# Aatrick/LightDiffusion

Measured on AMD Instinct MI355X. Metric: UNet denoise steps/sec at 512x512, higher is better.
Workload: dtype f16 (fp32 accumulate); 1 GPU; SD1.5 512x512 UNet CFG step, euler_ancestral / normal-30, batch 8/GPU (UNet batch 16), latent 64x64; global_batch=8, parallelism=dp1 (replicas, RCCL cond broadcast), hip_graph=True, setup_before_warmup=hipGraph capture + one untimed schedule pass per workload

## Files before the change

### lightdiffusion_amd/csrc/gemm.h

```cpp
#pragma once
#include "common.h"

struct GemmParams {
    const half_t* A = nullptr;
    const half_t* A2 = nullptr;
    int lda = 0;
    int conv = 0;
    int ksize = 3;
    int pad = -1;
    int Hs = 0, Ws = 0;
    int Hv = 0, Wv = 0;
    int Ho = 0, Wo = 0, stride = 1;
    int C1 = 0, C2 = 0;
    const half_t* S1 = nullptr;
    const half_t* S2 = nullptr;
    int SC1 = 0, SC2 = 0;
    const half_t* W = nullptr;
    int ldw = 0;
    int M = 0, N = 0, K = 0;
    int n_valid = 0;
    int batch = 1;
    long long sA = 0, sW = 0, sC = 0, sR = 0;
    float alpha = 1.0f;
    const half_t* bias_n = nullptr;
    const half_t* bias_m = nullptr;
    const half_t* rowvec = nullptr;
    int rows_per_vec = 1, ldrv = 0;
    const half_t* R = nullptr;
    int ldr = 0;
    int act = 0;
    half_t* C = nullptr;
    int ldc = 0;
    int bm = 0, bn = 0;
    int splitk = 0;
    int m_fastest = -1;
    int xcd_gm = 0;
    float* partial = nullptr;
    size_t partial_bytes = 0;
    float* stat_out = nullptr;
    int* stat_parts_out = nullptr;
    const float* ln_stat = nullptr;
    int ln_parts = 0;
    int ln_rows = 0;
    int ln_zrows = 0;
    float ln_inv_c = 0.f, ln_eps = 0.f;
    const float* ln_wsum = nullptr;
    int ln_swapped = 0;
    const float* gn_scale = nullptr;
    const float* gn_shift = nullptr;
    int gn_silu = 0;
    float* gn_part = nullptr;
    int gn_P = 0, gn_ppb = 0, gn_HW = 0;
    int* gn_part_done = nullptr;
    const half_t* W8 = nullptr;
    int* sync = nullptr;
    int c8_S = 0;
    int dbg = 0;
};

bool conv8_plan(const GemmParams& p, int* S_out);
int conv8_gn_chunks(const GemmParams& p);
int conv8_launch(const GemmParams& p, hipStream_t stream);
bool conv8_weight_eligible(int N, int Cin);
size_t conv8_weight_bytes(int N, int Cin);
int conv8_repack_launch(const half_t* w_okki, int N, int Cin, half_t* dst, hipStream_t stream);
#define LD_SYNC_INTS 1024

bool gemm_ln_fold_available();
const char* gemm_last_kernel_name();

static inline int gemm_pick_bn(int N) { return (N % 160 == 0) ? 160 : 128; }

int gemm_launch(const GemmParams& p, hipStream_t stream);
bool gemm_conv_fuses_groupnorm(const GemmParams& p);
bool gemm_conv_takes_skip_segment(const GemmParams& p);
bool gemm_conv_takes_halo_tile(const GemmParams& p);
```

### lightdiffusion_amd/csrc/gemm.hip

```cpp
#include <cstdlib>
#include <mutex>
#include <set>
#include <string>
#include <type_traits>

#include "gemm.h"

namespace {

constexpr int BK = 64;
constexpr int NT = 256;

__device__ __forceinline__ void epilogue_store8(const GemmParams& p, int z, int m, int n_out, int n_bias, float (&v)[8]) {
    const bool hb = p.bias_n != nullptr && p.act != 2, hv = p.rowvec != nullptr, hr = p.R != nullptr;
    const uint4 rb = hb ? ld16(p.bias_n + n_bias) : zero16();
    const uint4 rv = hv ? ld16(p.rowvec + (long long)(m / p.rows_per_vec) * p.ldrv + n_out) : zero16();
    const uint4 rr = hr ? ld16(p.R + (long long)z * p.sR + (long long)m * p.ldr + n_out) : zero16();
    const float bm = p.bias_m != nullptr ? (float)p.bias_m[m] : 0.f;
    float b[8], e[8], r[8];
    unpack8(rb, b);
    unpack8(rv, e);
    unpack8(rr, r);
#pragma unroll
    for (int j = 0; j < 8; ++j) v[j] = v[j] + b[j] + bm + e[j];
    if (p.act == 1) {
#pragma unroll
        for (int j = 0; j < 8; ++j) v[j] = silu_f(v[j]);
    } else if (p.act == 3) {
#pragma unroll
        for (int j = 0; j < 8; ++j) v[j] = quick_gelu_f(v[j]);
    }
#pragma unroll
    for (int j = 0; j < 8; ++j) v[j] += r[j];
    st16(p.C + (long long)z * p.sC + (long long)m * p.ldc + n_out, pack8(v));
}

template <int BM, int BN>
struct EpiPre {
    static constexpr int CPR = BN / 8, EIT = (BM * CPR + NT - 1) / NT, GRP = EIT > 5 ? (EIT + 1) / 2 : EIT;
    uint4 r[GRP];
    bool fast;
    bool bias_done;
};
template <int BM, int BN>
__device__ __forceinline__ EpiPre<BM, BN> epi_prefetch_residual(const GemmParams& p, int z, int m0, int n0, int tid, bool bias_done) {
    EpiPre<BM, BN> e;
    e.bias_done = bias_done;
    constexpr int CPR = EpiPre<BM, BN>::CPR, GRP = EpiPre<BM, BN>::GRP;
    e.fast = (BM * CPR) % NT == 0 && m0 + BM <= p.M && n0 + BN <= p.N && p.act == 0 && p.bias_m == nullptr && bias_done;
#pragma unroll
    for (int k = 0; k < GRP; ++k) e.r[k] = zero16();
    if (e.fast && p.R != nullptr) {
        const half_t* Rb = p.R + (long long)z * p.sR + (long long)m0 * p.ldr + n0;
#pragma unroll
        for (int k = 0; k < GRP; ++k) {
            const int q = tid + k * NT;
            const int row = q / CPR, cc = q - row * CPR;
            e.r[k] = ld16(Rb + (long long)row * p.ldr + cc * 8);
        }
    }
    return e;
}

template <int BM, int BN>
__device__ __forceinline__ void epilogue_tile(const GemmParams& p, const half_t* Cs, int z, int m0, int n0, int tid, float* lds_scratch, const half_t* bias_s,
                                              const EpiPre<BM, BN>& pre) {
    constexpr int CLD = BN + 8;
    if (p.act == 2) {
        constexpr int CPR = BN / 16;
        constexpr int EIT = (BM * CPR + NT - 1) / NT;
        if ((BM * CPR) % NT == 0 && m0 + BM <= p.M && n0 + BN <= p.N && pre.bias_done) {
            half_t* Cb = p.C + (long long)z * p.sC + (long long)m0 * p.ldc + n0 / 2;
            const bool hr = p.R != nullptr;
            const half_t* Rb = hr ? p.R + (long long)z * p.sR + (long long)m0 * p.ldr + n0 / 2 : nullptr;
            uint4 rres[EIT], ca[EIT], cg[EIT];
#pragma unroll
            for (int it = 0; it < EIT; ++it) {
                const int q = tid + it * NT;
                const int row = q / CPR, cc = q - row * CPR;
                rres[it] = hr ? ld16(Rb + (long long)row * p.ldr + cc * 8) : zero16();
                ca[it] = ld16(Cs + row * CLD + cc * 8);
                cg[it] = ld16(Cs + row * CLD + BN / 2 + cc * 8);
            }
#pragma unroll
            for (int it = 0; it < EIT; ++it) {
                const int q = tid + it * NT;
                const int row = q / CPR, cc = q - row * CPR;
                float g[8];
                unpack8(cg[it], g);
                const unsigned aw[4] = {ca[it].x, ca[it].y, ca[it].z, ca[it].w};
                const f32x2 gp[4] = {{g[0], g[1]}, {g[2], g[3]}, {g[4], g[5]}, {g[6], g[7]}};
                unsigned ow[4];
                geglu8_staged(aw, gp, ow);
                uint4 packed = make_uint4(ow[0], ow[1], ow[2], ow[3]);
                if (hr) packed = add8h(packed, rres[it]);
                st16(Cb + (long long)row * p.ldc + cc * 8, packed);
            }
            return;
        }
        uint4 rba[EIT], rbg[EIT], rres[EIT];
#pragma unroll
        for (int it = 0; it < EIT; ++it) {
            const int q = tid + it * NT;
            const int row = q / CPR, cc = q - row * CPR;
            const int m = m0 + row, nv = n0 + cc * 8, ng = nv + BN / 2;
            const bool ok = q < BM * CPR && m < p.M && ng < p.N;
            rba[it] = (ok && !pre.bias_done) ? ld16(p.bias_n + nv) : zero16();
            rbg[it] = (ok && !pre.bias_done) ? ld16(p.bias_n + ng) : zero16();
            rres[it] = (ok && p.R != nullptr) ? ld16(p.R + (long long)z * p.sR + (long long)m * p.ldr + n0 / 2 + cc * 8) : zero16();
        }
#pragma unroll
        for (int it = 0; it < EIT; ++it) {
            const int q = tid + it * NT;
            const int row = q / CPR, cc = q - row * CPR;
            const int m = m0 + row, ng = n0 + cc * 8 + BN / 2;
            if (q < BM * CPR && m < p.M && ng < p.N) {
                float a[8], g[8], ba[8], bg[8], r[8];
                unpack8(ld16(Cs + row * CLD + cc * 8), a);
                unpack8(ld16(Cs + row * CLD + BN / 2 + cc * 8), g);
                unpack8(rba[it], ba);
                unpack8(rbg[it], bg);
                unpack8(rres[it], r);
#pragma unroll
                for (int j = 0; j < 8; ++j) a[j] = (a[j] + ba[j]) * gelu_f(g[j] + bg[j]) + r[j];
                st16(p.C + (long long)z * p.sC + (long long)m * p.ldc + n0 / 2 + cc * 8, pack8(a));
            }
        }
    } else {
        constexpr int CPR = BN / 8;
        constexpr int EIT = (BM * CPR + NT - 1) / NT;
        constexpr int GRP = EIT > 5 ? (EIT + 1) / 2 : EIT;
        const bool hb = p.bias_n != nullptr && !pre.bias_done, hv = p.rowvec != nullptr, hr = p.R != nullptr;
        if (pre.fast) {
            static_assert(GRP == EpiPre<BM, BN>::GRP, "group size");
            half_t* Cb = p.C + (long long)z * p.sC + (long long)m0 * p.ldc + n0;
            const half_t* Rb = hr ? p.R + (long long)z * p.sR + (long long)m0 * p.ldr + n0 : nullptr;
            uint4 rnext[GRP];
#pragma unroll
            for (int k = 0; k < GRP; ++k) rnext[k] = pre.r[k];
#pragma unroll
            for (int g0 = 0; g0 < EIT; g0 += GRP) {
                uint4 rv[GRP], rres[GRP], cv[GRP];
#pragma unroll
                for (int k = 0; k < GRP; ++k) rres[k] = rnext[k];
#pragma unroll
                for (int k = 0; k < GRP; ++k) {
                    if (g0 + GRP + k >= EIT) continue;
                    const int q = tid + (g0 + GRP + k) * NT;
                    const int row = q / CPR, cc = q - row * CPR;
                    rnext[k] = hr ? ld16(Rb + (long long)row * p.ldr + cc * 8) : zero16();
                }
#pragma unroll
                for (int k = 0; k < GRP; ++k) {
                    if (g0 + k >= EIT) continue;
                    const int q = tid + (g0 + k) * NT;
                    const int row = q / CPR, cc = q - row * CPR;
                    rv[k] = hv ? ld16(p.rowvec + (long long)((m0 + row) / p.rows_per_vec) * p.ldrv + n0 + cc * 8) : zero16();
                    cv[k] = ld16(Cs + row * CLD + cc * 8);
                }
#pragma unroll
                for (int k = 0; k < GRP; ++k) {
                    if (g0 + k >= EIT) continue;
                    const int q = tid + (g0 + k) * NT;
                    const int row = q / CPR, cc = q - row * CPR;
                    uint4 packed = cv[k];
                    if (hv) packed = add8h(packed, rv[k]);
                    if (hr) packed = add8h(packed, rres[k]);
                    st16(Cb + (long long)row * p.ldc + cc * 8, packed);
                    if (lds_scratch != nullptr) {
                        const half2v one2 = {(half_t)1.f, (half_t)1.f};
                        const half2v h0 = __builtin_bit_cast(half2v, packed.x), h1 = __builtin_bit_cast(half2v, packed.y);
                        const half2v h2 = __builtin_bit_cast(half2v, packed.z), h3 = __builtin_bit_cast(half2v, packed.w);
                        float s1 = __builtin_amdgcn_fdot2(h1, one2, __builtin_amdgcn_fdot2(h0, one2, 0.f, false), false);
                        float s2 = __builtin_amdgcn_fdot2(h1, h1, __builtin_amdgcn_fdot2(h0, h0, 0.f, false), false);
                        s1 = __builtin_amdgcn_fdot2(h3, one2, __builtin_amdgcn_fdot2(h2, one2, s1, false), false);
                        s2 = __builtin_amdgcn_fdot2(h3, h3, __builtin_amdgcn_fdot2(h2, h2, s2, false), false);
                        *reinterpret_cast<float2*>(lds_scratch + q * 2) = make_float2(s1, s2);
                    }
                }
            }
            if (lds_scratch != nullptr) {
                __syncthreads();
                if (tid < BM) {
                    float s1 = 0.f, s2 = 0.f;
#pragma unroll 4
                    for (int c = 0; c < CPR; ++c) {
                        const float2 t = *reinterpret_cast<const float2*>(lds_scratch + (tid * CPR + c) * 2);
                        s1 += t.x;
                        s2 += t.y;
                    }
                    *reinterpret_cast<float2*>(p.stat_out + ((long long)(n0 / BN) * p.M + m0 + tid) * 2) = make_float2(s1, s2);
                }
            }
            return;
        }
#pragma unroll
        for (int g0 = 0; g0 < EIT; g0 += GRP) {
            uint4 rb[GRP], rv[GRP], rres[GRP];
#pragma unroll
            for (int k = 0; k < GRP; ++k) {
                const int q = tid + (g0 + k) * NT;
                const int row = q / CPR, cc = q - row * CPR;
                const int m = m0 + row, n = n0 + cc * 8;
                const bool ok = (g0 + k) < EIT && q < BM * CPR && m < p.M && n < p.N;
                rb[k] = (ok && hb) ? ld16(p.bias_n + n) : zero16();
                rv[k] = (ok && hv) ? ld16(p.rowvec + (long long)(m / p.rows_per_vec) * p.ldrv + n) : zero16();
                rres[k] = (ok && hr) ? ld16(p.R + (long long)z * p.sR + (long long)m * p.ldr + n) : zero16();
            }
#pragma unroll
            for (int k = 0; k < GRP; ++k) {
                const int q = tid + (g0 + k) * NT;
                const int row = q / CPR, cc = q - row * CPR;
                const int m = m0 + row, n = n0 + cc * 8;
                if ((g0 + k) < EIT && q < BM * CPR && m < p.M && n < p.N) {
                    float v[8], b[8], e[8], r[8];
                    unpack8(ld16(Cs + row * CLD + cc * 8), v);
                    unpack8(rb[k], b);
                    unpack8(rv[k], e);
                    unpack8(rres[k], r);
                    const float bm = p.bias_m != nullptr ? (float)p.bias_m[m] : 0.f;
#pragma unroll
                    for (int j = 0; j < 8; ++j) {
                        float t = v[j] + b[j] + bm + e[j];
                        if (p.act == 1) t = silu_f(t);
                        else if (p.act == 3) t = quick_gelu_f(t);
                        v[j] = t + r[j];
                    }
                    const uint4 packed = pack8(v);
                    st16(p.C + (long long)z * p.sC + (long long)m * p.ldc + n, packed);
                    if (lds_scratch != nullptr) {
                        float f[8];
                        unpack8(packed, f);
                        float s1 = 0.f, s2 = 0.f;
#pragma unroll
                        for (int j = 0; j < 8; ++j) {
                            s1 += f[j];
                            s2 += f[j] * f[j];
                        }
                        lds_scratch[q * 2] = s1;
                        lds_scratch[q * 2 + 1] = s2;
                    }
                } else if (lds_scratch != nullptr && (g0 + k) < EIT && q < BM * CPR) {
                    lds_scratch[q * 2] = 0.f;
                    lds_scratch[q * 2 + 1] = 0.f;
                }
            }
        }
        if (lds_scratch != nullptr) {
            __syncthreads();
            if (tid < BM && m0 + tid < p.M) {
                float s1 = 0.f, s2 = 0.f;
                for (int c = 0; c < CPR; ++c) {
                    s1 += lds_scratch[(tid * CPR + c) * 2];
                    s2 += lds_scratch[(tid * CPR + c) * 2 + 1];
                }
                float* o = p.stat_out + ((long long)(n0 / BN) * p.M + m0 + tid) * 2;
                o[0] = s1;
                o[1] = s2;
            }
        }
    }
}

__device__ __forceinline__ void ln_sum_parts(const float* q, long long stride, int parts, float& s1, float& s2) {
    int t = 0;
    for (; t + 4 <= parts; t += 4) {
        float2 v[4];
#pragma unroll
        for (int u = 0; u < 4; ++u) v[u] = *reinterpret_cast<const float2*>(q + (t + u) * stride);
#pragma unroll
        for (int u = 0; u < 4; ++u) {
            s1 += v[u].x;
            s2 += v[u].y;
        }
    }
    for (; t < parts; ++t) {
        const float2 v = *reinterpret_cast<const float2*>(q + t * stride);
        s1 += v.x;
        s2 += v.y;
    }
}

template <int BM, int BN>
__device__ __forceinline__ void ln_prepare(const GemmParams& p, float* ln_mu, float* ln_rs, int z, int m0, int n0, int tid) {
    const int cnt = p.ln_swapped ? BN : BM;
    if (tid >= cnt) return;
    const bool ok = p.ln_swapped ? (n0 + tid < p.n_valid) : (m0 + tid < p.M);
    const long long row = p.ln_swapped ? (long long)z * p.ln_zrows + n0 + tid : (long long)m0 + tid;
    float s1 = 0.f, s2 = 0.f;
    if (ok) ln_sum_parts(p.ln_stat + row * 2, (long long)p.ln_rows * 2, p.ln_parts, s1, s2);
    const float mu = s1 * p.ln_inv_c;
    ln_mu[tid] = mu;
    ln_rs[tid] = ok ? rsqrtf(fmaxf(s2 * p.ln_inv_c - mu * mu, 0.f) + p.ln_eps) : 0.f;
}

template <int TM, int TN>
__device__ __forceinline__ void ln_apply(const GemmParams& p, f32x4 (&acc)[TM][TN], const float* ln_mu, const float* ln_rs, int m0, int n0, int wm0,
                                         int wn0, int fr, int fq, const float* wsum_s, const half_t* bias_s, bool add_bias) {
    if (!p.ln_swapped) {
        f32x4 ws[TN], bj[TN];
        const float inv_alpha = 1.0f / p.alpha;
#pragma unroll
        for (int j = 0; j < TN; ++j) {
            ws[j] = *reinterpret_cast<const f32x4*>(wsum_s + wn0 + j * 16 + fq * 4);
            const half4 bh = *reinterpret_cast<const half4*>(bias_s + wn0 + j * 16 + fq * 4);
#pragma unroll
            for (int r = 0; r < 4; ++r) bj[j][r] = add_bias ? (float)bh[r] * inv_alpha : 0.f;
        }
#pragma unroll
        for (int i = 0; i < TM; ++i) {
            const float mu = ln_mu[wm0 + i * 16 + fr], rs = ln_rs[wm0 + i * 16 + fr];
#pragma unroll
            for (int j = 0; j < TN; ++j) acc[i][j] = (acc[i][j] - mu * ws[j]) * rs + bj[j];
        }
    } else {
#pragma unroll
        for (int i = 0; i < TM; ++i) {
            const int m = m0 + wm0 + i * 16 + fr;
            const float wsm = m < p.M ? p.ln_wsum[m] : 0.f;
#pragma unroll
            for (int j = 0; j < TN; ++j) {
                const f32x4 mu4 = *reinterpret_cast<const f32x4*>(ln_mu + wn0 + j * 16 + fq * 4);
                const f32x4 rs4 = *reinterpret_cast<const f32x4*>(ln_rs + wn0 + j * 16 + fq * 4);
                acc[i][j] = (acc[i][j] - mu4 * wsm) * rs4;
            }
        }
    }
}

__device__ uint4 g_zero_row[4096];

template <int BN>
__device__ __forceinline__ void epi_stage_load(const GemmParams& p, int n0, int t, f32x4& b, f32x4& w) {
    const char* zp = reinterpret_cast<const char*>(g_zero_row);
    const char* bp = (t < BN / 8 && p.bias_n != nullptr && n0 + t * 8 < p.N) ? reinterpret_cast<const char*>(p.bias_n + n0 + t * 8) : zp;
    const char* wp = (t < BN / 4 && p.ln_wsum != nullptr && !p.ln_swapped && n0 + t * 4 < p.N) ? reinterpret_cast<const char*>(p.ln_wsum + n0 + t * 4) : zp;
    asm volatile("global_load_dwordx4 %0, %1, off" : "=&v"(b) : "v"(bp) : "memory");
    asm volatile("global_load_dwordx4 %0, %1, off" : "=&v"(w) : "v"(wp) : "memory");
}
#define EPI_STAGE_WAIT(KEEP, b, w) asm volatile("s_waitcnt vmcnt(%2)" : "+v"(b), "+v"(w) : "n"(KEEP) : "memory")
template <int BN>
__device__ __forceinline__ void epi_stage_store(const f32x4& b, const f32x4& w, half_t* bias_s, float* wsum_s, int t) {
    if (t < BN / 8) *reinterpret_cast<f32x4*>(bias_s + t * 8) = b;
    if (t < BN / 4) *reinterpret_cast<f32x4*>(wsum_s + t * 4) = w;
}


__device__ __forceinline__ void glds16s(unsigned voff, const half_t* sbase, unsigned lds_base) {
    asm volatile(
        "s_mov_b32 m0, %2\n\t"
        "s_nop 0\n\t"
        "global_load_lds_dwordx4 %0, %1"
        :
        : "v"(voff), "s"(sbase), "s"(lds_base)
        : "memory");
}

template <int BM, int BN, bool CONV, int NST>
__global__ __launch_bounds__(NT, NST == 2 ? 2 : 1) void gemm3_kernel(const GemmParams p) {
    constexpr int BK3 = 64, PF = NST - 1;
    static_assert(NST == 2 || NST == 4, "ring depth");
    constexpr int WTM = BM / 2, WTN = BN / 2;
    constexpr int TM = WTM / 16, TN = WTN / 16;
    constexpr int A_CH = BM * 8, B_CH = BN * 8;
    constexpr int A_IT = A_CH / NT;
    constexpr int B_IT = B_CH / NT;
    static_assert(B_CH % NT == 0 && A_CH % NT == 0, "whole instructions per wave");
    constexpr int STAGE = (BM + BN) * BK3;
    constexpr int CLD = BN + 8;
    static_assert(BM * CLD <= NST * STAGE, "epilogue tile must fit in the ring");
    static_assert((BM * CLD * 2 + 15) / 16 * 16 + BM * (BN / 8) * 8 <= NST * STAGE * 2, "LN-fold row statistics must fit behind the epilogue tile");
    __shared__ __attribute__((aligned(16))) half_t smem[NST * STAGE];
    __shared__ __attribute__((aligned(16))) float ln_mu[BM > BN ? BM : BN], ln_rs[BM > BN ? BM : BN];
    __shared__ __attribute__((aligned(16))) half_t bias_s[BN];
    __shared__ __attribute__((aligned(16))) float wsum_s[BN];

    const int tid = threadIdx.x, lane = tid & 63;
    const int wid = __builtin_amdgcn_readfirstlane(tid >> 6);
    const int wm0 = (wid >> 1) * WTM, wn0 = (wid & 1) * WTN;
    const int z = blockIdx.z;
    const int tiles_m = (p.M + BM - 1) / BM, tiles_n = (p.N + BN - 1) / BN;
    const int tiles = tiles_m * tiles_n;
    const int splitk = p.splitk > 1 ? p.splitk : 1;
    int bid = xcd_remap(blockIdx.x, tiles * splitk);
    const int ks = bid / tiles;
    bid -= ks * tiles;
    const int tn_i = p.m_fastest ? bid / tiles_m : bid % tiles_n;
    const int tm_i = p.m_fastest ? bid % tiles_m : bid / tiles_n;
    const int m0 = tm_i * BM, n0 = tn_i * BN;
    const int KT = (p.K + BK3 - 1) / BK3;
    const int kt_begin = (int)((long long)ks * KT / splitk), kt_end = (int)((long long)(ks + 1) * KT / splitk);

    const half_t* Ab = p.A + (long long)z * p.sA;
    const half_t* Wb = p.W + (long long)z * p.sW;
    const half_t* zp = reinterpret_cast<const half_t*>(g_zero_row);
    const int Cin = p.C1 + p.C2;

    int a_lc[A_IT];
    bool a_ok[A_IT];
    int a_img[A_IT], a_iy0[A_IT], a_ix0[A_IT];
    const half_t* a_ptr[A_IT];
    unsigned a_off[A_IT];
#pragma unroll
    for (int i = 0; i < A_IT; ++i) {
        const int q = tid + i * NT;
        const int row = q >> 3;
        a_lc[i] = (q & 7) ^ (row & 7);
        const int m = m0 + row;
        a_ok[i] = m < p.M;
        a_img[i] = a_iy0[i] = a_ix0[i] = 0;
        a_ptr[i] = zp;
        a_off[i] = 0;
        if (CONV) {
            const int hw = p.Ho * p.Wo;
            const int mm = a_ok[i] ? m : 0;
            const int img = mm / hw, rem = mm - img * hw;
            const int oy = rem / p.Wo, ox = rem - oy * p.Wo;
            a_img[i] = img;
            a_iy0[i] = oy * p.stride - p.pad;
            a_ix0[i] = ox * p.stride - p.pad;
        } else {
            a_off[i] = (unsigned)(((long long)(a_ok[i] ? m : p.M - 1) * p.lda + a_lc[i] * 8) * 2);
        }
    }
    const half_t* a_base = Ab + (long long)kt_begin * BK3;
    int seg_left = 0;
    auto conv_seek = [&](int k0) {
        const int K9 = p.ksize * p.ksize * Cin;
        const bool skp = k0 >= K9 && p.SC1 > 0;
        const int tap = skp ? 0 : k0 / Cin;
        const int c0 = skp ? k0 - K9 : k0 - tap * Cin;
        const int ky = skp ? p.pad : tap / p.ksize, kx = skp ? p.pad : tap - (tap / p.ksize) * p.ksize;
        const int Ca = skp ? p.SC1 : p.C1, Cb = skp ? p.SC2 : p.C2;
        const bool second = c0 >= Ca;
        const half_t* src = skp ? (second ? p.S2 : p.S1) : (second ? p.A2 : Ab);
        const int Cs = second ? Cb : Ca;
        const int cl = second ? c0 - Ca : c0;
        seg_left = ((second ? Ca + Cb : Ca) - c0) / BK3;
#pragma unroll
        for (int i = 0; i < A_IT; ++i) {
            const int iy = a_iy0[i] + ky, ix = a_ix0[i] + kx;
            const bool ok = a_ok[i] && (unsigned)iy < (unsigned)p.Hv && (unsigned)ix < (unsigned)p.Wv && tap < p.ksize * p.ksize && c0 < Ca + Cb;
            int sy = iy, sx = ix;
            if (p.Hv == 2 * p.Hs && p.Wv == 2 * p.Ws) {
                sy = iy >> 1;
                sx = ix >> 1;
            } else if (p.Hv != p.Hs || p.Wv != p.Ws) {
                sy = (int)((long long)iy * p.Hs / p.Hv);
                sx = (int)((long long)ix * p.Ws / p.Wv);
            }
            a_ptr[i] = ok ? src + (((long long)a_img[i] * p.Hs + sy) * p.Ws + sx) * Cs + cl + a_lc[i] * 8 : zp + a_lc[i] * 8;
        }
    };
    unsigned b_off[B_IT];
    int b_lc[B_IT];
#pragma unroll
    for (int i = 0; i < B_IT; ++i) {
        const int q = tid + i * NT;
        const int row = q >> 3;
        b_lc[i] = (q & 7) ^ (row & 7);
        const int n = n0 + row < p.n_valid ? n0 + row : p.n_valid - 1;
        b_off[i] = (unsigned)(((long long)n * p.ldw + b_lc[i] * 8) * 2);
    }
    const half_t* b_base = Wb + (long long)kt_begin * BK3;

    const unsigned smem_base = __builtin_amdgcn_readfirstlane(lds_addr(smem));
    auto issue = [&](int kt, int st) {
        if (kt >= kt_end) return;
        const unsigned As = smem_base + (unsigned)(st * STAGE) * 2u + (unsigned)(wid * 64) * 16u;
        const unsigned Bs = As + (unsigned)(BM * BK3) * 2u;
        const int k0 = kt * BK3;
        if (k0 + BK3 <= p.K) {
#pragma unroll
            for (int i = 0; i < A_IT; ++i) {
                if (CONV) glds16(a_ptr[i], As + (unsigned)(i * NT) * 16u);
                else glds16s(a_off[i], a_base, As + (unsigned)(i * NT) * 16u);
            }
#pragma unroll
            for (int i = 0; i < B_IT; ++i) glds16s(b_off[i], b_base, Bs + (unsigned)(i * NT) * 16u);
        } else {
#pragma unroll
            for (int i = 0; i < A_IT; ++i) {
                const half_t* src = CONV ? a_ptr[i] : reinterpret_cast<const half_t*>(reinterpret_cast<const char*>(a_base) + a_off[i]);
                glds16(k0 + a_lc[i] * 8 < p.K ? src : zp, As + (unsigned)(i * NT) * 16u);
            }
#pragma unroll
            for (int i = 0; i < B_IT; ++i) {
                const half_t* src = reinterpret_cast<const half_t*>(reinterpret_cast<const char*>(b_base) + b_off[i]);
                glds16(k0 + b_lc[i] * 8 < p.K ? src : zp, Bs + (unsigned)(i * NT) * 16u);
            }
        }
        if (CONV) {
            if (--seg_left <= 0) {
                conv_seek(k0 + BK3);
            } else {
#pragma unroll
                for (int i = 0; i < A_IT; ++i) a_ptr[i] += BK3;
            }
        } else {
            a_base += BK3;
        }
        b_base += BK3;
    };
    if (CONV) conv_seek(kt_begin * BK3);

    const int fr = lane & 15, fq = lane >> 4;
    const half_t* rd0 = smem + (wm0 + fr) * BK3 + ((fq ^ (fr & 7)) << 3);
    const half_t* rd1 = smem + (wm0 + fr) * BK3 + (((4 + fq) ^ (fr & 7)) << 3);
    const int b_rel = (BM + wn0 - wm0) * BK3;

    f32x4 acc[TM][TN];
#pragma unroll
    for (int i = 0; i < TM; ++i)
#pragma unroll
        for (int j = 0; j < TN; ++j) acc[i][j] = (f32x4){0.f, 0.f, 0.f, 0.f};

    half8 fa0[TM], fb0[TN], fa1[TM], fb1[TN];
    auto read_frags = [&](const half_t* rd, half8 (&fa)[TM], half8 (&fb)[TN]) {
#pragma unroll
        for (int j = 0; j < TN; ++j) fb[j] = as_half8(ld16(rd + b_rel + j * 16 * BK3));
#pragma unroll
        for (int i = 0; i < TM; ++i) fa[i] = as_half8(ld16(rd + i * 16 * BK3));
    };
    auto mma = [&](const half8 (&fa)[TM], const half8 (&fb)[TN]) {
#pragma unroll
        for (int i = 0; i < TM; ++i)
#pragma unroll
            for (int j = 0; j < TN; ++j) acc[i][j] = __builtin_amdgcn_mfma_f32_16x16x32_f16(fb[j], fa[i], acc[i][j], 0, 0, 0);
    };

    constexpr int LPT = A_IT + B_IT;
    auto wait_slab = [&](int kt) {
        if (PF == 1) {
            wait_vmcnt<0>();
        } else {
            const int ahead = kt_end - 1 - kt;
            if (ahead >= PF - 1) wait_vmcnt<LPT*(PF - 1)>();
            else if (ahead == 1) wait_vmcnt<LPT>();
            else wait_vmcnt<0>();
        }
    };
    f32x4 est_b, est_w;
    epi_stage_load<BN>(p, n0, tid, est_b, est_w);
#pragma unroll
    for (int t = 0; t < PF; ++t) issue(kt_begin + t, t);
    if (p.ln_stat != nullptr) ln_prepare<BM, BN>(p, ln_mu, ln_rs, z, m0, n0, tid);
    if (kt_end - kt_begin >= PF) EPI_STAGE_WAIT(PF * (A_IT + B_IT), est_b, est_w);
    else EPI_STAGE_WAIT(0, est_b, est_w);
    epi_stage_store<BN>(est_b, est_w, bias_s, wsum_s, tid);
    wait_slab(kt_begin);
    __builtin_amdgcn_s_barrier();
    issue(kt_begin + PF, PF);
    const bool bias_acc = splitk == 1 && p.ln_stat == nullptr && (p.act == 0 || p.act == 2);
    const bool bias_done = bias_acc || (splitk == 1 && p.ln_stat != nullptr && !p.ln_swapped && (p.act == 0 || p.act == 2));
    if (bias_acc) {
        const float inv_alpha = 1.0f / p.alpha;
#pragma unroll
        for (int j = 0; j < TN; ++j) {
            const half4 bh = *reinterpret_cast<const half4*>(bias_s + wn0 + j * 16 + fq * 4);
            f32x4 bf;
#pragma unroll
            for (int r = 0; r < 4; ++r) bf[r] = (float)bh[r] * inv_alpha;
#pragma unroll
            for (int i = 0; i < TM; ++i) acc[i][j] = bf;
        }
    }
    read_frags(rd0, fa0, fb0);
    asm volatile("s_waitcnt lgkmcnt(0)" ::: "memory");
    int st = 0;
    for (int kt = kt_begin; kt < kt_end; ++kt) {
        read_frags(rd1, fa1, fb1);
        __builtin_amdgcn_sched_barrier(0);
        mma(fa0, fb0);
        __builtin_amdgcn_sched_barrier(0);
        asm volatile("s_waitcnt lgkmcnt(0)" ::: "memory");
        wait_slab(kt + 1);
        __builtin_amdgcn_s_barrier();
        issue(kt + NST, st);
        const int flip = (st == NST - 1) ? -(NST - 1) * STAGE : STAGE;
        rd0 += flip;
        rd1 += flip;
        st = (st + 1) & (NST - 1);
        read_frags(rd0, fa0, fb0);
        __builtin_amdgcn_sched_barrier(0);
        mma(fa1, fb1);
        __builtin_amdgcn_sched_barrier(0);
        asm volatile("s_waitcnt lgkmcnt(0)" ::: "memory");
    }
    wait_vmcnt<0>();
    __builtin_amdgcn_s_barrier();

    if (splitk > 1) {
        float* part = p.partial + (long long)ks * p.M * p.N;
#pragma unroll
        for (int i = 0; i < TM; ++i) {
            const int m = m0 + wm0 + i * 16 + fr;
#pragma unroll
            for (int j = 0; j < TN; ++j) {
                const int n = n0 + wn0 + j * 16 + fq * 4;
                if (m < p.M && n < p.N) {
                    f32x4 v = acc[i][j];
                    v *= p.alpha;
                    *reinterpret_cast<f32x4*>(part + (long long)m * p.N + n) = v;
                }
            }
        }
        return;
    }
    half_t* Cs = smem;
    const EpiPre<BM, BN> pre = epi_prefetch_residual<BM, BN>(p, z, m0, n0, tid, bias_done);
    if (p.ln_stat != nullptr) ln_apply<TM, TN>(p, acc, ln_mu, ln_rs, m0, n0, wm0, wn0, fr, fq, wsum_s, bias_s, bias_done);
#pragma unroll
    for (int i = 0; i < TM; ++i) {
        const int ml = wm0 + i * 16 + fr;
#pragma unroll
        for (int j = 0; j < TN; ++j) {
            const int nl = wn0 + j * 16 + fq * 4;
            const f32x4 v = acc[i][j] * p.alpha;
            *reinterpret_cast<uint2*>(Cs + ml * CLD + nl) = make_uint2(pk2h(v[0], v[1]), pk2h(v[2], v[3]));
        }
    }
    __syncthreads();
    float* scratch = p.stat_out != nullptr ? reinterpret_cast<float*>(reinterpret_cast<char*>(smem) + (BM * CLD * 2 + 15) / 16 * 16) : nullptr;
    epilogue_tile<BM, BN>(p, Cs, z, m0, n0, tid, scratch, bias_s, pre);
}

template <int LPT, int MAXA>
__device__ __forceinline__ void wait_slabs_ahead(int ahead) {
    if constexpr (MAXA == 0) {
        wait_vmcnt<0>();
    } else {
        if (ahead >= MAXA) wait_vmcnt<MAXA * LPT>();
        else wait_slabs_ahead<LPT, MAXA - 1>(ahead);
    }
}

template <int BM, int BN, bool CONV, int NST = 4, int WPS = 2>
__global__ __launch_bounds__(2 * NT, WPS) void gemm4_kernel(const GemmParams p) {
    constexpr int BK3 = 64;
    static_assert((NST & (NST - 1)) == 0 && NST >= 4, "ring depth");
    constexpr int WTM = BM / 2, WTN = BN / 2;
    constexpr int TM = WTM / 16, TN = WTN / 16;
    constexpr int A_IT = BM * 8 / NT, B_IT = BN * 8 / NT;
    static_assert((BM * 8) % NT == 0 && (BN * 8) % NT == 0, "whole instructions per wave");
    constexpr int LPT = A_IT + B_IT;
    constexpr int STAGE = (BM + BN) * BK3;
    constexpr int CLD = BN + 8;
    static_assert(BM * CLD <= NST * STAGE, "epilogue tile must fit in the ring");
    __shared__ __attribute__((aligned(16))) half_t smem[NST * STAGE];
    __shared__ __attribute__((aligned(16))) float ln_mu[BM > BN ? BM : BN], ln_rs[BM > BN ? BM : BN];
    __shared__ __attribute__((aligned(16))) half_t bias_s[BN];
    __shared__ __attribute__((aligned(16))) float wsum_s[BN];

    const int lane = threadIdx.x & 63;
    const int wid8 = __builtin_amdgcn_readfirstlane(threadIdx.x >> 6);
    const bool producer = wid8 >= 4;
    const int wid = wid8 & 3;
    const int tid = wid * 64 + lane;
    const int z = blockIdx.z;
    const int tiles_m = (p.M + BM - 1) / BM, tiles_n = (p.N + BN - 1) / BN;
    const int tiles = tiles_m * tiles_n;
    const int splitk = p.splitk > 1 ? p.splitk : 1;
    int bid = xcd_remap(blockIdx.x, tiles * splitk);
    const int ks = bid / tiles;
    bid -= ks * tiles;
    const int tn_i = p.m_fastest ? bid / tiles_m : bid % tiles_n;
    const int tm_i = p.m_fastest ? bid % tiles_m : bid / tiles_n;
    const int m0 = tm_i * BM, n0 = tn_i * BN;
    const int KT = (p.K + BK3 - 1) / BK3;
    const int kt_begin = (int)((long long)ks * KT / splitk), kt_end = (int)((long long)(ks + 1) * KT / splitk);

    if (producer) {
        const half_t* Ab = p.A + (long long)z * p.sA;
        const half_t* Wb = p.W + (long long)z * p.sW;
        const half_t* zp = reinterpret_cast<const half_t*>(g_zero_row);
        const int Cin = p.C1 + p.C2;
        int a_lc[A_IT];
        bool a_ok[A_IT];
        int a_img[A_IT], a_iy0[A_IT], a_ix0[A_IT];
        const half_t* a_ptr[A_IT];
        unsigned a_off[A_IT];
#pragma unroll
        for (int i = 0; i < A_IT; ++i) {
            const int q = tid + i * NT;
            const int row = q >> 3;
            a_lc[i] = (q & 7) ^ (row & 7);
            const int m = m0 + row;
            a_ok[i] = m < p.M;
            a_img[i] = a_iy0[i] = a_ix0[i] = 0;
            a_ptr[i] = zp;
            a_off[i] = 0;
            if (CONV) {
                const int hw = p.Ho * p.Wo;
                const int mm = a_ok[i] ? m : 0;
                const int img = mm / hw, rem = mm - img * hw;
                const int oy = rem / p.Wo, ox = rem - oy * p.Wo;
                a_img[i] = img;
                a_iy0[i] = oy * p.stride - p.pad;
                a_ix0[i] = ox * p.stride - p.pad;
            } else {
                a_off[i] = (unsigned)(((long long)(a_ok[i] ? m : p.M - 1) * p.lda + a_lc[i] * 8) * 2);
            }
        }
        const half_t* a_base = Ab + (long long)kt_begin * BK3;
        int seg_left = 0;
        auto conv_seek = [&](int k0) {
            const int K9 = p.ksize * p.ksize * Cin;
            const bool skp = k0 >= K9 && p.SC1 > 0;
            const int tap = skp ? 0 : k0 / Cin;
            const int c0 = skp ? k0 - K9 : k0 - tap * Cin;
            const int ky = skp ? p.pad : tap / p.ksize, kx = skp ? p.pad : tap - (tap / p.ksize) * p.ksize;
            const int Ca = skp ? p.SC1 : p.C1, Cb = skp ? p.SC2 : p.C2;
            const bool second = c0 >= Ca;
            const half_t* src = skp ? (second ? p.S2 : p.S1) : (second ? p.A2 : Ab);
            const int Cs = second ? Cb : Ca;
            const int cl = second ? c0 - Ca : c0;
            seg_left = ((second ? Ca + Cb : Ca) - c0) / BK3;
#pragma unroll
            for (int i = 0; i < A_IT; ++i) {
                const int iy = a_iy0[i] + ky, ix = a_ix0[i] + kx;
                const bool ok = a_ok[i] && (unsigned)iy < (unsigned)p.Hv && (unsigned)ix < (unsigned)p.Wv && tap < p.ksize * p.ksize && c0 < Ca + Cb;
                int sy = iy, sx = ix;
                if (p.Hv == 2 * p.Hs && p.Wv == 2 * p.Ws) {
                    sy = iy >> 1;
                    sx = ix >> 1;
                } else if (p.Hv != p.Hs || p.Wv != p.Ws) {
                    sy = (int)((long long)iy * p.Hs / p.Hv);
                    sx = (int)((long long)ix * p.Ws / p.Wv);
                }
                a_ptr[i] = ok ? src + (((long long)a_img[i] * p.Hs + sy) * p.Ws + sx) * Cs + cl + a_lc[i] * 8 : zp + a_lc[i] * 8;
            }
        };
        unsigned b_off[B_IT];
        int b_lc[B_IT];
#pragma unroll
        for (int i = 0; i < B_IT; ++i) {
            const int q = tid + i * NT;
            const int row = q >> 3;
            b_lc[i] = (q & 7) ^ (row & 7);
            const int n = n0 + row < p.n_valid ? n0 + row : p.n_valid - 1;
            b_off[i] = (unsigned)(((long long)n * p.ldw + b_lc[i] * 8) * 2);
        }
        const half_t* b_base = Wb + (long long)kt_begin * BK3;
        const unsigned smem_base = __builtin_amdgcn_readfirstlane(lds_addr(smem));
        auto issue = [&](int kt) {
            if (kt >= kt_end) return;
            const int st = (kt - kt_begin) & (NST - 1);
            const unsigned As = smem_base + (unsigned)(st * STAGE) * 2u + (unsigned)(wid * 64) * 16u;
            const unsigned Bs = As + (unsigned)(BM * BK3) * 2u;
            const int k0 = kt * BK3;
            if (k0 + BK3 <= p.K) {
#pragma unroll
                for (int i = 0; i < A_IT; ++i) {
                    if (CONV) glds16(a_ptr[i], As + (unsigned)(i * NT) * 16u);
                    else glds16s(a_off[i], a_base, As + (unsigned)(i * NT) * 16u);
                }
#pragma unroll
                for (int i = 0; i < B_IT; ++i) glds16s(b_off[i], b_base, Bs + (unsigned)(i * NT) * 16u);
            } else {
#pragma unroll
                for (int i = 0; i < A_IT; ++i) {
                    const half_t* src = CONV ? a_ptr[i] : reinterpret_cast<const half_t*>(reinterpret_cast<const char*>(a_base) + a_off[i]);
                    glds16(k0 + a_lc[i] * 8 < p.K ? src : zp, As + (unsigned)(i * NT) * 16u);
                }
#pragma unroll
                for (int i = 0; i < B_IT; ++i) {
                    const half_t* src = reinterpret_cast<const half_t*>(reinterpret_cast<const char*>(b_base) + b_off[i]);
                    glds16(k0 + b_lc[i] * 8 < p.K ? src : zp, Bs + (unsigned)(i * NT) * 16u);
                }
            }
            if (CONV) {
                if (--seg_left <= 0) {
                    conv_seek(k0 + BK3);
                } else {
#pragma unroll
                    for (int i = 0; i < A_IT; ++i) a_ptr[i] += BK3;
                }
            } else {
                a_base += BK3;
            }
            b_base += BK3;
        };
        auto wait_slab = [&](int kt, int issued_after) {
            int ahead = kt_end - 1 - kt;
            if (ahead > issued_after) ahead = issued_after;
            wait_slabs_ahead<LPT, NST - 1>(ahead);
        };
        if (CONV) conv_seek(kt_begin * BK3);
#pragma unroll
        for (int t = 0; t < NST; ++t) issue(kt_begin + t);
        wait_slab(kt_begin, NST - 1);
        __builtin_amdgcn_s_barrier();
        for (int kt = kt_begin; kt < kt_end; ++kt) {
            wait_slab(kt + 1, NST - 2);
            __builtin_amdgcn_s_barrier();
            issue(kt + NST);
        }
        wait_vmcnt<0>();
        __builtin_amdgcn_s_barrier();
        return;
    }

    {
        f32x4 est_b, est_w;
        epi_stage_load<BN>(p, n0, tid, est_b, est_w);
        EPI_STAGE_WAIT(0, est_b, est_w);
        epi_stage_store<BN>(est_b, est_w, bias_s, wsum_s, tid);
    }
    if (p.ln_stat != nullptr) ln_prepare<BM, BN>(p, ln_mu, ln_rs, z, m0, n0, tid);
    const int wm0 = (wid >> 1) * WTM, wn0 = (wid & 1) * WTN;
    const int fr = lane & 15, fq = lane >> 4;
    const half_t* rd0 = smem + (wm0 + fr) * BK3 + ((fq ^ (fr & 7)) << 3);
    const half_t* rd1 = smem + (wm0 + fr) * BK3 + (((4 + fq) ^ (fr & 7)) << 3);
    const int b_rel = (BM + wn0 - wm0) * BK3;

    f32x4 acc[TM][TN];
#pragma unroll
    for (int i = 0; i < TM; ++i)
#pragma unroll
        for (int j = 0; j < TN; ++j) acc[i][j] = (f32x4){0.f, 0.f, 0.f, 0.f};
    half8 fa0[TM], fb0[TN], fa1[TM], fb1[TN];
    auto read_frags = [&](const half_t* rd, half8 (&fa)[TM], half8 (&fb)[TN]) {
#pragma unroll
        for (int j = 0; j < TN; ++j) fb[j] = as_half8(ld16(rd + b_rel + j * 16 * BK3));
#pragma unroll
        for (int i = 0; i < TM; ++i) fa[i] = as_half8(ld16(rd + i * 16 * BK3));
    };
    auto mma = [&](const half8 (&fa)[TM], const half8 (&fb)[TN]) {
#pragma unroll
        for (int i = 0; i < TM; ++i)
#pragma unroll
            for (int j = 0; j < TN; ++j) acc[i][j] = __builtin_amdgcn_mfma_f32_16x16x32_f16(fb[j], fa[i], acc[i][j], 0, 0, 0);
    };
    __builtin_amdgcn_s_barrier();
    const bool bias_acc = splitk == 1 && p.ln_stat == nullptr && (p.act == 0 || p.act == 2);
    const bool bias_done = bias_acc || (splitk == 1 && p.ln_stat != nullptr && !p.ln_swapped && (p.act == 0 || p.act == 2));
    if (bias_acc) {
        const float inv_alpha = 1.0f / p.alpha;
#pragma unroll
        for (int j = 0; j < TN; ++j) {
            const half4 bh = *reinterpret_cast<const half4*>(bias_s + wn0 + j * 16 + fq * 4);
            f32x4 bf;
#pragma unroll
            for (int r = 0; r < 4; ++r) bf[r] = (float)bh[r] * inv_alpha;
#pragma unroll
            for (int i = 0; i < TM; ++i) acc[i][j] = bf;
        }
    }
    read_frags(rd0, fa0, fb0);
    asm volatile("s_waitcnt lgkmcnt(0)" ::: "memory");
    int st = 0;
    for (int kt = kt_begin; kt < kt_end; ++kt) {
        read_frags(rd1, fa1, fb1);
        __builtin_amdgcn_sched_barrier(0);
        mma(fa0, fb0);
        __builtin_amdgcn_sched_barrier(0);
        asm volatile("s_waitcnt lgkmcnt(0)" ::: "memory");
        __builtin_amdgcn_s_barrier();
        const int flip = (st == NST - 1) ? -(NST - 1) * STAGE : STAGE;
        rd0 += flip;
        rd1 += flip;
        st = (st + 1) & (NST - 1);
        read_frags(rd0, fa0, fb0);
        __builtin_amdgcn_sched_barrier(0);
        mma(fa1, fb1);
        __builtin_amdgcn_sched_barrier(0);
        asm volatile("s_waitcnt lgkmcnt(0)" ::: "memory");
    }
    __builtin_amdgcn_s_barrier();

    if (splitk > 1) {
        float* part = p.partial + (long long)ks * p.M * p.N;
#pragma unroll
        for (int i = 0; i < TM; ++i) {
            const int m = m0 + wm0 + i * 16 + fr;
#pragma unroll
            for (int j = 0; j < TN; ++j) {
                const int n = n0 + wn0 + j * 16 + fq * 4;
                if (m < p.M && n < p.N) {
                    f32x4 v = acc[i][j];
                    v *= p.alpha;
                    *reinterpret_cast<f32x4*>(part + (long long)m * p.N + n) = v;
                }
            }
        }
        return;
    }
    half_t* Cs = smem;
    const EpiPre<BM, BN> pre = epi_prefetch_residual<BM, BN>(p, z, m0, n0, tid, bias_done);
    if (p.ln_stat != nullptr) ln_apply<TM, TN>(p, acc, ln_mu, ln_rs, m0, n0, wm0, wn0, fr, fq, wsum_s, bias_s, bias_done);
#pragma unroll
    for (int i = 0; i < TM; ++i) {
        const int ml = wm0 + i * 16 + fr;
#pragma unroll
        for (int j = 0; j < TN; ++j) {
            const int nl = wn0 + j * 16 + fq * 4;
            const f32x4 v = acc[i][j] * p.alpha;
            *reinterpret_cast<uint2*>(Cs + ml * CLD + nl) = make_uint2(pk2h(v[0], v[1]), pk2h(v[2], v[3]));
        }
    }
    __syncthreads();
    float* scratch = p.stat_out != nullptr ? reinterpret_cast<float*>(reinterpret_cast<char*>(smem) + (BM * CLD * 2 + 15) / 16 * 16) : nullptr;
    epilogue_tile<BM, BN>(p, Cs, z, m0, n0, tid, scratch, bias_s, pre);
}

constexpr int V5_BM = 256, V5_BN = 320, V5_BK = 32, V5_NST = 4;
constexpr int V5_A_BYTES = V5_BM * 64, V5_STAGE_BYTES = (V5_BM + V5_BN) * 64;
constexpr int V5_EPI_LD = 164;
constexpr int V5_EPI_BYTES = 16 * V5_EPI_LD * 2;
constexpr int V5_SWZ = 0x78;

template <int EPI>
__device__ __forceinline__ void v5_epilogue_strip(const GemmParams& p, half_t* Cs, int z, int m_base, int n_base, int lane, int part, bool bias_done) {
    const bool rows_full = m_base + 16 <= p.M;
    if (EPI == 2) {
        if (rows_full) {
            half_t* Cb = p.C + (long long)z * p.sC + (long long)m_base * p.ldc + n_base / 2;
            const bool hr = p.R != nullptr;
            const half_t* Rb = hr ? p.R + (long long)z * p.sR + (long long)m_base * p.ldr + n_base / 2 : nullptr;
            uint4 rres[3], ca[3], cg[3];
#pragma unroll
            for (int it = 0; it < 3; ++it) {
                const int q0 = lane + it * 64;
                const int q = q0 < 160 ? q0 : 0;
                const int row = q / 10, cc = q - row * 10;
                rres[it] = hr ? ld16(Rb + (long long)row * p.ldr + cc * 8) : zero16();
                ca[it] = ld16(Cs + row * V5_EPI_LD + cc * 8);
                cg[it] = ld16(Cs + row * V5_EPI_LD + 80 + cc * 8);
            }
#pragma unroll
            for (int it = 0; it < 3; ++it) {
                const int q0 = lane + it * 64;
                const int q = q0 < 160 ? q0 : 0;
                const int row = q / 10, cc = q - row * 10;
                float g[8];
                unpack8(cg[it], g);
                const unsigned aw[4] = {ca[it].x, ca[it].y, ca[it].z, ca[it].w};
                const f32x2 gp[4] = {{g[0], g[1]}, {g[2], g[3]}, {g[4], g[5]}, {g[6], g[7]}};
                unsigned ow[4];
                geglu8_staged(aw, gp, ow);
                uint4 packed = make_uint4(ow[0], ow[1], ow[2], ow[3]);
                if (hr) packed = add8h(packed, rres[it]);
                if (q0 < 160) st16(Cb + (long long)row * p.ldc + cc * 8, packed);
            }
            return;
        }
        uint4 rba[3], rbg[3], rres[3];
#pragma unroll
        for (int it = 0; it < 3; ++it) {
            const int q = lane + it * 64;
            const int row = q / 10, cc = q - row * 10;
            const int m = m_base + row, nv = n_base + cc * 8;
            const bool ok = q < 160 && m < p.M;
            rba[it] = (ok && !bias_done) ? ld16(p.bias_n + nv) : zero16();
            rbg[it] = (ok && !bias_done) ? ld16(p.bias_n + nv + 80) : zero16();
            rres[it] = (ok && p.R != nullptr) ? ld16(p.R + (long long)z * p.sR + (long long)m * p.ldr + n_base / 2 + cc * 8) : zero16();
        }
#pragma unroll
        for (int it = 0; it < 3; ++it) {
            const int q = lane + it * 64;
            const int row = q / 10, cc = q - row * 10;
            const int m = m_base + row;
            if (q < 160 && m < p.M) {
                float a[8], g[8], ba[8], bg[8], r[8];
                unpack8(ld16(Cs + row * V5_EPI_LD + cc * 8), a);
                unpack8(ld16(Cs + row * V5_EPI_LD + 80 + cc * 8), g);
                unpack8(rba[it], ba);
                unpack8(rbg[it], bg);
                unpack8(rres[it], r);
#pragma unroll
                for (int j = 0; j < 8; ++j) a[j] = (a[j] + ba[j]) * gelu_f(g[j] + bg[j]) + r[j];
                st16(p.C + (long long)z * p.sC + (long long)m * p.ldc + n_base / 2 + cc * 8, pack8(a));
            }
        }
        return;
    }
    const bool hb = p.bias_n != nullptr && !bias_done, hv = p.rowvec != nullptr, hr = p.R != nullptr;
    if (rows_full && p.bias_m == nullptr && p.act == 0 && bias_done) {
        half_t* Cb = p.C + (long long)z * p.sC + (long long)m_base * p.ldc + n_base;
        const half_t* Rb = hr ? p.R + (long long)z * p.sR + (long long)m_base * p.ldr + n_base : nullptr;
        float s1[5], s2[5];
        uint4 rv[5], rres[5], cv[5];
#pragma unroll
        for (int k = 0; k < 5; ++k) {
            const int q = lane + k * 64;
            const int row = q / 20, cc = q - row * 20;
            rv[k] = hv ? ld16(p.rowvec + (long long)((m_base + row) / p.rows_per_vec) * p.ldrv + n_base + cc * 8) : zero16();
            rres[k] = hr ? ld16(Rb + (long long)row * p.ldr + cc * 8) : zero16();
            cv[k] = ld16(Cs + row * V5_EPI_LD + cc * 8);
        }
#pragma unroll
        for (int k = 0; k < 5; ++k) {
            const int q = lane + k * 64;
            const int row = q / 20, cc = q - row * 20;
            uint4 packed = cv[k];
            if (hv) packed = add8h(packed, rv[k]);
            if (hr) packed = add8h(packed, rres[k]);
            st16(Cb + (long long)row * p.ldc + cc * 8, packed);
            if (EPI == 1 && p.stat_out != nullptr) {
                const half2v one2 = {(half_t)1.f, (half_t)1.f};
                const half2v h0 = __builtin_bit_cast(half2v, packed.x), h1 = __builtin_bit_cast(half2v, packed.y);
                const half2v h2 = __builtin_bit_cast(half2v, packed.z), h3 = __builtin_bit_cast(half2v, packed.w);
                float a1 = __builtin_amdgcn_fdot2(h1, one2, __builtin_amdgcn_fdot2(h0, one2, 0.f, false), false);
                float a2 = __builtin_amdgcn_fdot2(h1, h1, __builtin_amdgcn_fdot2(h0, h0, 0.f, false), false);
                s1[k] = __builtin_amdgcn_fdot2(h3, one2, __builtin_amdgcn_fdot2(h2, one2, a1, false), false);
                s2[k] = __builtin_amdgcn_fdot2(h3, h3, __builtin_amdgcn_fdot2(h2, h2, a2, false), false);
            }
        }
        if (EPI == 1 && p.stat_out != nullptr) {
            float* sc = reinterpret_cast<float*>(Cs);
            asm volatile("s_waitcnt lgkmcnt(0)" ::: "memory");
#pragma unroll
            for (int it = 0; it < 5; ++it) *reinterpret_cast<float2*>(sc + (lane + it * 64) * 2) = make_float2(s1[it], s2[it]);
            asm volatile("s_waitcnt lgkmcnt(0)" ::: "memory");
            if (lane < 16) {
                float a = 0.f, b = 0.f;
#pragma unroll 4
                for (int c = 0; c < 20; ++c) {
                    const float2 t = *reinterpret_cast<const float2*>(sc + (lane * 20 + c) * 2);
                    a += t.x;
                    b += t.y;
                }
                *reinterpret_cast<float2*>(p.stat_out + ((long long)part * p.M + m_base + lane) * 2) = make_float2(a, b);
            }
            asm volatile("s_waitcnt lgkmcnt(0)" ::: "memory");
        }
        return;
    }
    uint4 rb[5], rv[5], rres[5];
#pragma unroll
    for (int it = 0; it < 5; ++it) {
        const int q = lane + it * 64;
        const int row = q / 20, cc = q - row * 20;
        const int m = m_base + row, n = n_base + cc * 8;
        const bool ok = m < p.M;
        rb[it] = (ok && hb) ? ld16(p.bias_n + n) : zero16();
        rv[it] = (ok && hv) ? ld16(p.rowvec + (long long)(m / p.rows_per_vec) * p.ldrv + n) : zero16();
        rres[it] = (ok && hr) ? ld16(p.R + (long long)z * p.sR + (long long)m * p.ldr + n) : zero16();
    }
    float s1[5], s2[5];
#pragma unroll
    for (int it = 0; it < 5; ++it) {
        const int q = lane + it * 64;
        const int row = q / 20, cc = q - row * 20;
        const int m = m_base + row, n = n_base + cc * 8;
        s1[it] = s2[it] = 0.f;
        if (m < p.M) {
            float v[8], b[8], e[8], r[8];
            unpack8(ld16(Cs + row * V5_EPI_LD + cc * 8), v);
            unpack8(rb[it], b);
// ... 974 lines not shown
        float v[8];
        if (p.act == 2) {
            const int half_bn = bn / 2;
            const int no = cc * 8;
            const int tile = no / half_bn, within = no - tile * half_bn;
            const int nv = tile * bn + within, ng = nv + half_bn;
            float a[8] = {0, 0, 0, 0, 0, 0, 0, 0}, g[8] = {0, 0, 0, 0, 0, 0, 0, 0};
            for (int s = 0; s < p.splitk; ++s) {
                const float* base = p.partial + ((long long)s * p.M + m) * p.N;
#pragma unroll
                for (int j = 0; j < 8; ++j) {
                    a[j] += base[nv + j];
                    g[j] += base[ng + j];
                }
            }
            float ba[8], bg[8];
            unpack8(ld16(p.bias_n + nv), ba);
            unpack8(ld16(p.bias_n + ng), bg);
#pragma unroll
            for (int j = 0; j < 8; ++j) v[j] = (a[j] + ba[j]) * gelu_f(g[j] + bg[j]);
            epilogue_store8(p, 0, m, no, 0, v);
        } else {
            const int n = cc * 8;
#pragma unroll
            for (int j = 0; j < 8; ++j) v[j] = 0.f;
            const float* base = p.partial + (long long)m * p.N + n;
            const long long slab = (long long)p.M * p.N;
            int s = 0;
            for (; s + 4 <= p.splitk; s += 4) {
                f32x4 x0[4], x1[4];
#pragma unroll
                for (int u = 0; u < 4; ++u) {
                    x0[u] = *reinterpret_cast<const f32x4*>(base + (s + u) * slab);
                    x1[u] = *reinterpret_cast<const f32x4*>(base + (s + u) * slab + 4);
                }
#pragma unroll
                for (int u = 0; u < 4; ++u)
#pragma unroll
                    for (int j = 0; j < 4; ++j) {
                        v[j] += x0[u][j];
                        v[4 + j] += x1[u][j];
                    }
            }
            for (; s < p.splitk; ++s) {
                const f32x4 x0 = *reinterpret_cast<const f32x4*>(base + s * slab), x1 = *reinterpret_cast<const f32x4*>(base + s * slab + 4);
#pragma unroll
                for (int j = 0; j < 4; ++j) {
                    v[j] += x0[j];
                    v[4 + j] += x1[j];
                }
            }
            epilogue_store8(p, 0, m, n, n, v);
        }
    }
}

__global__ __launch_bounds__(256) void splitk_reduce_gn_kernel(const GemmParams p) {
    __shared__ float csum[2048], csq[2048];
    const int C = p.N, cpg = C / 32;
    const int CS = C / 4, CHS = CS >> 3;
    const int n = blockIdx.y, pc = blockIdx.x, slab = blockIdx.z, tid = threadIdx.x;
    const int rows_par = 256 / CHS;
    const int cc = tid % CHS, prow = tid / CHS;
    const int c0 = slab * CS + cc * 8;
    const int p_begin = pc * p.gn_ppb, p_end = min(p.gn_HW, p_begin + p.gn_ppb);
    const long long slab_stride = (long long)p.M * p.N;
    if (prow < rows_par) {
        float s[8], ss[8];
#pragma unroll
        for (int j = 0; j < 8; ++j) s[j] = ss[j] = 0.f;
        for (int pix = p_begin + prow; pix < p_end; pix += rows_par) {
            const int m = n * p.gn_HW + pix;
            const float* base = p.partial + (long long)m * p.N + c0;
            float v[8];
#pragma unroll
            for (int j = 0; j < 8; ++j) v[j] = 0.f;
            int sp = 0;
            for (; sp + 4 <= p.splitk; sp += 4) {
                f32x4 x0[4], x1[4];
#pragma unroll
                for (int u = 0; u < 4; ++u) {
                    x0[u] = *reinterpret_cast<const f32x4*>(base + (sp + u) * slab_stride);
                    x1[u] = *reinterpret_cast<const f32x4*>(base + (sp + u) * slab_stride + 4);
                }
#pragma unroll
                for (int u = 0; u < 4; ++u)
#pragma unroll
                    for (int j = 0; j < 4; ++j) {
                        v[j] += x0[u][j];
                        v[4 + j] += x1[u][j];
                    }
            }
            for (; sp < p.splitk; ++sp) {
                const f32x4 x0 = *reinterpret_cast<const f32x4*>(base + sp * slab_stride), x1 = *reinterpret_cast<const f32x4*>(base + sp * slab_stride + 4);
#pragma unroll
                for (int j = 0; j < 4; ++j) {
                    v[j] += x0[j];
                    v[4 + j] += x1[j];
                }
            }
            epilogue_store8(p, 0, m, c0, c0, v);
            float f[8];
            unpack8(pack8(v), f);
#pragma unroll
            for (int j = 0; j < 8; ++j) {
                s[j] += f[j];
                ss[j] += f[j] * f[j];
            }
        }
#pragma unroll
        for (int j = 0; j < 8; ++j) {
            csum[prow * CS + cc * 8 + j] = s[j];
            csq[prow * CS + cc * 8 + j] = ss[j];
        }
    }
    __syncthreads();
    {
        const int g = tid >> 5, sub = tid & 31;
        const int cnt = rows_par * cpg;
        float a = 0.f, b = 0.f;
        for (int i = sub; i < cnt; i += 32) {
            const int pr = i / cpg, c = g * cpg + (i - pr * cpg);
            a += csum[pr * CS + c];
            b += csq[pr * CS + c];
        }
#pragma unroll
        for (int o = 1; o < 32; o <<= 1) {
            a += __shfl_xor(a, o, 64);
            b += __shfl_xor(b, o, 64);
        }
        if (sub == 0) {
            float* o = p.gn_part + (((long long)n * p.gn_P + pc) * 32 + slab * 8 + g) * 2;
            o[0] = a;
            o[1] = b;
        }
    }
}

constexpr int V4_MAX_BLOCKS = 256;

thread_local const char* t_last_kernel = "";
const char* intern_name(const std::string& s) {
    static std::mutex mu;
    static std::set<std::string> pool;
    std::lock_guard<std::mutex> lock(mu);
    return pool.insert(s).first->c_str();
}

template <int BM, int BN>
void launch_cfg(const GemmParams& p, hipStream_t s, bool deep = false, bool conv1_2wg = false) {
    const int tiles = ((p.M + BM - 1) / BM) * ((p.N + BN - 1) / BN);
    const int sk = p.splitk > 1 ? p.splitk : 1;
    dim3 grid(tiles * sk, 1, p.batch);
    if constexpr (BM == 64 && BN == 64) {
        const long long blocks = (long long)tiles * sk * p.batch;
        if (!p.conv && blocks > V4_MAX_BLOCKS && blocks <= 512 && p.K >= 640) {
            t_last_kernel = "gemm4_kernel<64,64,plain,2wg>";
            hipLaunchKernelGGL((gemm4_kernel<64, 64, false, 4, 4>), grid, dim3(2 * NT), 0, s, p);
            return;
        }
        if (conv1_2wg) {
            t_last_kernel = "gemm4_kernel<64,64,conv,2wg>";
            hipLaunchKernelGGL((gemm4_kernel<64, 64, true, 4, 4>), grid, dim3(2 * NT), 0, s, p);
            return;
        }
    }
    if (!p.conv && (long long)tiles * sk * p.batch <= V4_MAX_BLOCKS) {
        static const std::string name = "gemm4_kernel<" + std::to_string(BM) + "," + std::to_string(BN) + ",plain>";
        t_last_kernel = name.c_str();
        hipLaunchKernelGGL((gemm4_kernel<BM, BN, false>), grid, dim3(2 * NT), 0, s, p);
    } else if (p.conv) {
        static const std::string name = "gemm3_kernel<" + std::to_string(BM) + "," + std::to_string(BN) + ",conv>";
        t_last_kernel = name.c_str();
        if constexpr (BM == 64 && BN == 160) {
            if (deep) {
                t_last_kernel = "gemm3_kernel<64,160,conv,deep>";
                hipLaunchKernelGGL((gemm3_kernel<BM, BN, true, 4>), grid, dim3(NT), 0, s, p);
                return;
            }
        }
        hipLaunchKernelGGL((gemm3_kernel<BM, BN, true, 2>), grid, dim3(NT), 0, s, p);
    } else {
        static const std::string name = "gemm3_kernel<" + std::to_string(BM) + "," + std::to_string(BN) + ",plain>";
        t_last_kernel = name.c_str();
        hipLaunchKernelGGL((gemm3_kernel<BM, BN, false, 2>), grid, dim3(NT), 0, s, p);
    }
}

template <int W, bool GN, int BN, int BM, bool UP>
void launch_conv6_w(const GemmParams& p, dim3 grid, hipStream_t s) {
    static const std::string name = "conv6_kernel<W" + std::to_string(W) + ",halo" + (GN ? "+groupnorm" : "") +
                                    (BN == V5_BN ? "" : "," + std::to_string(BN) + (BM == V5_BM ? "" : "x" + std::to_string(BM))) + (UP ? ",up" : "") + ">";
    t_last_kernel = name.c_str();
    hipLaunchKernelGGL((conv6_kernel<W, GN, BN, BM, UP>), grid, dim3(512), 0, s, p);
}
template <bool GN, int BN = V5_BN, int BM = V5_BM, bool UP = false>
void launch_conv6(int wc, const GemmParams& p, dim3 grid, hipStream_t s) {
    if constexpr (BN == V5_BN) {
        if (wc == 16) return launch_conv6_w<16, GN, BN, BM, UP>(p, grid, s);
        if (wc == 32) return launch_conv6_w<32, GN, BN, BM, UP>(p, grid, s);
    }
    if constexpr (BN == V5_BN || (BN == 256 && !GN)) {
        if (wc == 64) return launch_conv6_w<64, GN, BN, BM, UP>(p, grid, s);
    }
    launch_conv6_w<128, GN, BN, BM, UP>(p, grid, s);
}

}

#ifdef LD_AB_BUILD
static int g_force_bm = 0, g_force_sk = 0;
static int g_shape_ovr[5] = {0, 0, 0, 0, 0};
extern "C" void ld_debug_gemm_shape_override(int M, int N, int K, int bm, int splitk) {
    g_shape_ovr[0] = M; g_shape_ovr[1] = N; g_shape_ovr[2] = K; g_shape_ovr[3] = bm; g_shape_ovr[4] = splitk;
}
extern "C" void ld_debug_gemm_override(int bm, int splitk) {
    g_force_bm = bm;
    g_force_sk = splitk;
}
#endif

static void launch_splitk_reduce(const GemmParams& p, int bn, hipStream_t stream) {
    const bool gn = p.gn_part != nullptr && p.act != 2 && p.batch == 1 && p.gn_P > 0 && p.gn_HW > 0 && p.M % p.gn_HW == 0 && p.N % 32 == 0 && p.N <= 8192 && p.N >= 256 &&
                    p.ldc == p.N && (p.N / 4) % 8 == 0 && p.N / 32 <= 256;
    if (gn) {
        hipLaunchKernelGGL(splitk_reduce_gn_kernel, dim3(p.gn_P, p.M / p.gn_HW, 4), dim3(256), 0, stream, p);
        if (p.gn_part_done != nullptr) *p.gn_part_done = p.gn_P;
        t_last_kernel = intern_name(std::string(t_last_kernel) + "+splitk_reduce_gn_kernel");
        return;
    }
    const int out_n = p.act == 2 ? p.N / 2 : p.N;
    const long long total = (long long)p.M * (out_n / 8);
    int blocks = (int)((total + 255) / 256);
    if (blocks > 2048) blocks = 2048;
    hipLaunchKernelGGL(splitk_reduce_kernel, dim3(blocks), dim3(256), 0, stream, p, bn);
    t_last_kernel = intern_name(std::string(t_last_kernel) + "+splitk_reduce_kernel");
}

bool gemm_ln_fold_available() { return true; }
const char* gemm_last_kernel_name() { return t_last_kernel; }

struct V6Plan {
    int sk = 1, bn = 0, bm = V5_BM, wc = 0;
    bool up = false;
};
static bool v6_plan(const GemmParams& p, V6Plan* out) {
    const bool same = p.Hv == p.Hs && p.Wv == p.Ws;
    const bool up = p.Hv == 2 * p.Hs && p.Wv == 2 * p.Ws;
    if (!(p.conv && p.ksize == 3 && p.stride == 1 && (p.pad < 0 || p.pad == 1) && (same || up) && p.Ho == p.Hv && p.Wo == p.Wv &&
          p.C1 % 32 == 0 && p.C2 % 32 == 0 && p.bm == 0 && p.bn == 0 && p.splitk == 0 && p.batch == 1 && p.act != 2))
        return false;
    if (up && (p.C2 != 0 || p.gn_scale != nullptr)) return false;
    if (p.SC1 > 0) return false;
    const int wc = (p.Wo == 16 || p.Wo == 32 || p.Wo == 64 || p.Wo == 128) ? p.Wo : (p.Wo > 128 && p.Wo % 128 == 0) ? 128 : 0;
    if (wc == 0) return false;
    int bn = 0, bm = V5_BM;
    if (p.N % V5_BN == 0) {
        bn = V5_BN;
    } else if (p.N % 256 == 0 && wc >= 64 && (p.gn_scale == nullptr || (p.N == 256 && wc == 128 && !up))) {
        bn = 256;
    } else if (p.N % 128 == 0 && wc == 128 && (p.gn_scale == nullptr || (p.N == 128 && !up))) {
        bn = 128;
        bm = 512;
    } else if (p.N == 32 && wc == 128 && p.gn_scale == nullptr && !up) {
        bn = 32;
        bm = 512;
    } else {
        return false;
    }
    if (p.Ho % (bm / wc) != 0 || p.M % bm != 0) return false;
    const long long tm = p.M / bm;
    const long long t6 = tm * (p.N / bn);
    const int NS = (p.C1 + p.C2) / 32;
    int sk6 = 1;
    if (t6 < 192 && p.partial != nullptr && p.K >= 8640) {
        sk6 = (int)((256 + t6 - 1) / t6);
        const int cap = p.K / 2560;
        if (sk6 > cap) sk6 = cap;
        if (sk6 > NS) sk6 = NS;
        while (sk6 > 1 && (size_t)sk6 * p.M * p.N * sizeof(float) > p.partial_bytes) --sk6;
    }
#ifdef LD_AB_BUILD
    if (p.partial != nullptr && bn == V5_BN) {
        static const char* names[4] = {"LD_V6_SK_W16", "LD_V6_SK_W32", "LD_V6_SK_W64", "LD_V6_SK_W128"};
        const char* e = getenv(names[wc == 16 ? 0 : wc == 32 ? 1 : wc == 64 ? 2 : 3]);
        if (e != nullptr) {
            int want = atoi(e);
            if (want < 1) want = 1;
            if (want > NS) want = NS;
            while (want > 1 && (size_t)want * p.M * p.N * sizeof(float) > p.partial_bytes) --want;
            sk6 = want;
        }
    }
#endif
    out->sk = sk6;
    out->bn = bn;
    out->bm = bm;
    out->wc = wc;
    out->up = up;
    return t6 * sk6 >= 192;
}

bool gemm_conv_takes_skip_segment(const GemmParams& p) {
    V6Plan pl;
    return p.conv && p.ksize == 3 && p.stride == 1 && p.Hv == p.Hs && p.Wv == p.Ws && p.SC1 == 0 && !conv8_plan(p, nullptr) && !v6_plan(p, &pl);
}

bool gemm_conv_takes_halo_tile(const GemmParams& pin) {
    GemmParams p = pin;
    V6Plan pl;
    return v6_plan(p, &pl);
}

bool gemm_conv_fuses_groupnorm(const GemmParams& p) {
    V6Plan pl;
    if (!v6_plan(p, &pl) || pl.up) return false;
    if (p.N == V5_BN && pl.bn == V5_BN) return true;
    return pl.wc == 128 && ((p.N == 256 && pl.bn == 256 && pl.bm == V5_BM) || (p.N == 128 && pl.bn == 128 && pl.bm == 512));
}

int gemm_launch(const GemmParams& pin, hipStream_t stream) {
    GemmParams p = pin;
    t_last_kernel = "";
#ifdef LD_AB_BUILD
    if (g_force_bm) p.bm = g_force_bm;
    if (g_force_sk) p.splitk = g_force_sk;
    if (g_shape_ovr[0] == p.M && g_shape_ovr[1] == p.N && g_shape_ovr[2] == p.K && p.batch == 1 && p.gn_scale == nullptr) {
        p.bm = g_shape_ovr[3];
        p.splitk = g_shape_ovr[4];
    }
#endif
    if (p.M <= 0 || p.N <= 0 || p.K <= 0 || p.A == nullptr || p.W == nullptr || p.C == nullptr) return LD_ERR_ARG;
    if ((p.N & 7) || (p.K & 7) || (p.ldw & 7) || (p.ldc & 7)) return LD_ERR_SHAPE;
    if (p.conv) {
        const int Cin = p.C1 + p.C2;
        if (p.ksize != 1 && p.ksize != 3) return LD_ERR_ARG;
        if (p.pad < 0) p.pad = p.ksize >> 1;
        if (p.SC1 < 0 || p.SC2 < 0 || (p.SC1 == 0 && p.SC2 != 0)) return LD_ERR_ARG;
        if (Cin <= 0 || (p.C1 % 64) || (p.C2 % 64) || (p.SC1 % 64) || (p.SC2 % 64) || p.K != p.ksize * p.ksize * Cin + p.SC1 + p.SC2) return LD_ERR_SHAPE;
        if (p.SC1 > 0) {
            if (p.S1 == nullptr || (p.SC2 > 0 && p.S2 == nullptr)) return LD_ERR_ARG;
            if (p.stride != 1 || p.Hv != p.Hs || p.Wv != p.Ws || p.Ho != p.Hv || p.Wo != p.Wv || p.pad != p.ksize / 2 || p.SC1 > 32768 || p.SC2 > 32768) return LD_ERR_SHAPE;
        }
        if (p.C1 > 32768 || p.C2 > 32768) return LD_ERR_SHAPE;
        if (p.C2 > 0 && p.A2 == nullptr) return LD_ERR_ARG;
        if (p.M % (p.Ho * p.Wo)) return LD_ERR_SHAPE;
        if (p.batch != 1) return LD_ERR_ARG;
    } else if (p.lda & 7) {
        return LD_ERR_SHAPE;
    }
    if (p.act == 2 && (p.bias_n == nullptr || (p.N & 15))) return LD_ERR_ARG;
    if (p.R != nullptr && (p.ldr & 7)) return LD_ERR_SHAPE;

    if (p.n_valid <= 0 || p.n_valid > p.N) p.n_valid = p.N;
    if (conv8_plan(p, nullptr)) {
        static const char* names[4][2] = {{"conv8_kernel<W8>", "conv8_kernel<W8,up>"}, {"conv8_kernel<W16>", "conv8_kernel<W16,up>"},
                                          {"conv8_kernel<W32>", "conv8_kernel<W32,up>"}, {"conv8_kernel<W64>", "conv8_kernel<W64,up>"}};
        t_last_kernel = names[p.Wo == 8 ? 0 : p.Wo == 16 ? 1 : p.Wo == 32 ? 2 : 3][p.Hv == 2 * p.Hs ? 1 : 0];
        if (p.gn_part != nullptr && p.gn_part_done != nullptr) *p.gn_part_done = conv8_gn_chunks(p);
        return conv8_launch(p, stream);
    }
    V6Plan pl;
    if (v6_plan(p, &pl)) {
        const int sk6 = pl.sk, bn6 = pl.bn, wc = pl.wc;
        const long long t6 = (long long)(p.M / pl.bm) * (p.N / bn6);
        p.splitk = sk6;
        p.pad = 1;
        if (bn6 != 32) p.n_valid = p.N;
        dim3 grid((unsigned)(t6 * sk6), 1, 1);
        if (sk6 == 1 && p.gn_part != nullptr) {
            const int cpg = p.N / 32, tiles_img = (p.Ho / (pl.bm / wc)) * (p.Wo / wc);
            const bool ok = (bn6 == 256 || bn6 == 128) && p.N % 32 == 0 && (p.N == 128 || cpg % 8 == 0) && bn6 % cpg == 0 && p.n_valid == p.N && p.act == 0;
            if (ok) {
                p.gn_P = tiles_img;
                if (p.gn_part_done != nullptr) *p.gn_part_done = tiles_img;
            } else {
                p.gn_part = nullptr;
            }
        }
        if (p.gn_scale != nullptr) {
            if (p.gn_shift == nullptr || pl.up) return LD_ERR_ARG;
            if (bn6 != V5_BN && (wc != 128 || p.N != bn6 || !((bn6 == 256 && pl.bm == V5_BM) || (bn6 == 128 && pl.bm == 512)))) return LD_ERR_ARG;
            if (bn6 == 256) launch_conv6<true, 256>(wc, p, grid, stream);
            else if (bn6 == 128) launch_conv6<true, 128, 512>(wc, p, grid, stream);
            else launch_conv6<true>(wc, p, grid, stream);
        } else if (bn6 == 128) {
            launch_conv6<false, 128, 512>(wc, p, grid, stream);
        } else if (bn6 == 32) {
            launch_conv6<false, 32, 512>(wc, p, grid, stream);
        } else if (bn6 == 256) {
            if (pl.up) launch_conv6<false, 256, V5_BM, true>(wc, p, grid, stream);
            else launch_conv6<false, 256>(wc, p, grid, stream);
        } else {
            if (pl.up) launch_conv6<false, V5_BN, V5_BM, true>(wc, p, grid, stream);
            else launch_conv6<false>(wc, p, grid, stream);
        }
        if (sk6 > 1) launch_splitk_reduce(p, 160, stream);
        return hipGetLastError() == hipSuccess ? LD_OK : LD_ERR_HIP;
    }
    if (p.gn_scale != nullptr) return LD_ERR_ARG;
    if (!p.conv && p.K == V7_K && p.batch == 1 && !p.ln_swapped && p.bias_m == nullptr && p.rowvec == nullptr && p.bm == 0 && (p.bn == 0 || p.bn == 160) &&
        p.splitk == 0 && (p.n_valid <= 0 || p.n_valid >= p.N) && p.N % (p.act == 2 ? 160 : V7_NB) == 0 && (p.M + V7_BM - 1) / V7_BM >= 192 &&
        (p.act == 0 || (p.act == 2 && p.bias_n != nullptr && p.stat_out == nullptr && p.R == nullptr))) {
        if (p.stat_parts_out != nullptr) *p.stat_parts_out = p.N / V7_NB;
        dim3 grid((unsigned)((p.M + V7_BM - 1) / V7_BM), 1, 1);
        const bool ln = p.ln_stat != nullptr;
        if (p.act == 2) {
            t_last_kernel = ln ? "gemm7_kernel<256,K320,geglu,ln>" : "gemm7_kernel<256,K320,geglu>";
            if (ln) hipLaunchKernelGGL((gemm7_kernel<true, true>), grid, dim3(512), 0, stream, p);
            else hipLaunchKernelGGL((gemm7_kernel<true, false>), grid, dim3(512), 0, stream, p);
        } else {
            t_last_kernel = ln ? "gemm7_kernel<256,K320,plain,ln>" : "gemm7_kernel<256,K320,plain>";
            if (ln) hipLaunchKernelGGL((gemm7_kernel<false, true>), grid, dim3(512), 0, stream, p);
            else hipLaunchKernelGGL((gemm7_kernel<false, false>), grid, dim3(512), 0, stream, p);
        }
        return hipGetLastError() == hipSuccess ? LD_OK : LD_ERR_HIP;
    }
    {
        const bool conv3 = p.conv && p.ksize == 3;
        const bool shape_ok = !p.ln_swapped && p.bm == 0 && (p.bn == 0 || p.bn == 160) && p.N % V5_BN == 0 && p.K % V5_BK == 0 &&
                              p.K >= (p.act == 2 ? 1280 : conv3 ? 640 : 2560) && (p.n_valid == p.N || p.n_valid <= 0 || p.n_valid > p.N) &&
                              p.splitk == 0 && p.M >= 1024;
        if (shape_ok) {
            const long long t5 = (long long)((p.M + V5_BM - 1) / V5_BM) * (p.N / V5_BN) * p.batch;
            if (t5 >= 192 && !(p.act == 2 && p.stat_out != nullptr)) {
                if (p.stat_parts_out != nullptr) *p.stat_parts_out = 2 * (p.N / V5_BN);
                p.splitk = 1;
                p.bn = 160;
                if (p.n_valid <= 0 || p.n_valid > p.N) p.n_valid = p.N;
                dim3 grid((unsigned)t5, 1, 1);
                grid.x = (unsigned)(((p.M + V5_BM - 1) / V5_BM) * (p.N / V5_BN));
                grid.z = (unsigned)p.batch;
                const bool ln = p.ln_stat != nullptr || p.stat_out != nullptr;
                if (p.conv) {
                    if (ln || p.act == 2) return LD_ERR_ARG;
                    t_last_kernel = "gemm5_kernel<256,320,conv>";
                    hipLaunchKernelGGL((gemm5_kernel<true, 0>), grid, dim3(512), 0, stream, p);
                } else {
                    t_last_kernel = p.act == 2 ? "gemm5_kernel<256,320,geglu>" : ln ? "gemm5_kernel<256,320,lnfold>" : "gemm5_kernel<256,320,plain>";
                    {
                        const int tm5 = (p.M + V5_BM - 1) / V5_BM, tn5 = p.N / V5_BN;
                        p.xcd_gm = 0;
                        if (p.batch == 1 && (tm5 * tn5) % 8 == 0 && p.M % V5_BM == 0) {
                            double best = 0;
                            for (int gm = 1; gm <= 8; gm <<= 1) {
                                const int gn = 8 / gm;
                                if (tm5 % gm || tn5 % gn) continue;
                                const double cost = (double)p.M * gn + (double)p.N * gm;
                                if (p.xcd_gm == 0 || cost < best) {
                                    best = cost;
                                    p.xcd_gm = gm;
                                }
                            }
                        }
                    }
                    if (p.act == 2) hipLaunchKernelGGL((gemm5_kernel<false, 2>), grid, dim3(512), 0, stream, p);
                    else if (ln) hipLaunchKernelGGL((gemm5_kernel<false, 1>), grid, dim3(512), 0, stream, p);
                    else hipLaunchKernelGGL((gemm5_kernel<false, 0>), grid, dim3(512), 0, stream, p);
                }
                return hipGetLastError() == hipSuccess ? LD_OK : LD_ERR_HIP;
            }
        }
    }
    int bn = p.bn ? p.bn : gemm_pick_bn(p.N);
    constexpr int skinny_max = 256;
    const bool skinny_ok = !p.conv && p.act != 2 && p.bn == 0 && p.bm == 0 && (p.N % 64) == 0;
    if (skinny_ok) {
        const long long t160 = (long long)((p.M + 63) / 64) * ((p.N + bn - 1) / bn) * p.batch;
        if (t160 <= skinny_max && (p.N + bn - 1) / bn <= 8) bn = 64;
    }
    bool skinny_conv1 = false;
    if (p.conv && p.ksize == 1 && p.act == 0 && p.bn == 0 && p.bm == 0 && p.splitk == 0 && p.batch == 1 && (p.N % 64) == 0 && p.SC1 == 0) {
        const long long t64 = (long long)((p.M + 63) / 64) * (p.N / 64);
        if (t64 > 128 && t64 <= 512 && p.K >= 1280 && p.K <= 3200) {
            bn = 64;
            skinny_conv1 = true;
        }

    }
    if (bn != 128 && bn != 160 && bn != 64) return LD_ERR_ARG;
    if (p.act == 2 && (p.N % bn)) return LD_ERR_SHAPE;
    const int tiles_n = (p.N + bn - 1) / bn;
    const int KT = (p.K + BK - 1) / BK;
    const int tiles128 = ((p.M + 127) / 128) * tiles_n * p.batch;
    const bool can_split = p.batch == 1 && p.partial != nullptr;
    const int sk_cap = p.K / 640 < 1 ? 1 : (p.K / 640 > 16 ? 16 : p.K / 640);
    int bm = p.bm, sk = p.splitk;
    if (bm == 0) {
        if (tiles128 >= 512) bm = 128;
        else if (p.K >= 4096 && can_split && (tiles128 >= 128 || (p.K >= 8192 && tiles128 >= 64))) bm = 128;
        else if (!p.conv && tiles128 >= 256) bm = 128;
        else bm = 64;
    }
    if (bn == 64) bm = 64;
    if (skinny_conv1) sk = 1;
    if (bm != 64 && bm != 128) return LD_ERR_ARG;
    const int tiles = ((p.M + bm - 1) / bm) * tiles_n;
    const bool deep = p.conv && bm == 64 && bn == 160 && p.batch == 1 && p.splitk == 0 && (tiles <= 32 || (tiles >= 256 && tiles < 512));
    if (sk == 0) {
        sk = 1;
        if (can_split && tiles * p.batch < 512) {
            sk = ((deep ? 256 : 512) + tiles - 1) / tiles;
            if (sk > sk_cap) sk = sk_cap;
        }
// ... 29 lines not shown
```

### lightdiffusion_amd/csrc/kernels.h

```cpp
#pragma once
#include <cstdlib>
#include "common.h"
#include "gemm.h"

static inline int gn_num_chunks(int n_img, int HW) {
    const long long px = (long long)(n_img < 1 ? 1 : n_img) * HW;
    const int target = px <= 8192 ? 512 : (px <= 131072 ? 1024 : 2048);
    int p = target / (4 * (n_img < 1 ? 1 : n_img));
    if (p > HW / 8) p = HW / 8;
    if (p > 256) p = 256;
    return p < 1 ? 1 : p;
}
size_t groupnorm_workspace_bytes(int n_img, int HW);
int groupnorm_launch(const half_t* x1, int C1, const half_t* x2, int C2, int n_img, int HW, const half_t* gamma,
                     const half_t* beta, float eps, int silu, half_t* y, float* partial, hipStream_t stream, int stats_ready = 0);
int groupnorm_stats_launch(const half_t* x1, int C1, const half_t* x2, int C2, int n_img, int HW, float* partial, hipStream_t stream);
int groupnorm_scale_shift_launch(const half_t* x1, int C1, const half_t* x2, int C2, int n_img, int HW, const half_t* gamma, const half_t* beta,
                                 float eps, float* partial, float* scale, float* shift, hipStream_t stream, int stats_ready = 0);
int layernorm_launch(const half_t* x, const half_t* gamma, const half_t* beta, half_t* y, int rows, int C, float eps,
                     hipStream_t stream);
int softmax_rows_launch(half_t* s, int rows, int cols, long long ld, hipStream_t stream, int valid = 0);

struct AttnParams {
    const half_t* Q = nullptr;
    const half_t* K = nullptr;
    const half_t* Vt = nullptr;
    const half_t* V = nullptr;
    int ldv = 0;
    half_t* O = nullptr;
    int ldq = 0, ldk = 0, ldvt = 0, ldo = 0;
    long long sQ = 0, sK = 0, sV = 0, sO = 0;
    int B = 0, H = 0, Lq = 0, Lk = 0, d = 0;
    float scale = 1.0f;
    int causal = 0;
};
int attention_launch(const AttnParams& p, hipStream_t stream);
const char* attention_last_kernel_name();

int ln_fold_launch(const half_t* W, int N, int K, const half_t* gamma, const half_t* beta, const half_t* bias, half_t* Wout, half_t* bout,
                   float* wsum, hipStream_t stream);
int mlp_out_fold_launch(const half_t* Wpo, const half_t* W2, const half_t* b2, const half_t* bpo, int C, half_t* Wout, half_t* bout, hipStream_t stream);
int skip_fold_launch(const half_t* W2, const half_t* Wsk, const half_t* b2, const half_t* bsk, int N, int K9, int SC, half_t* Wout, half_t* bout,
                     hipStream_t stream);
struct SmallConvInArgs {
    const float* x = nullptr;
    const float* scale_sigma = nullptr;
    const half_t* pre_w = nullptr;
    const half_t* pre_b = nullptr;
    const half_t* w = nullptr;
    const half_t* b = nullptr;
    half_t* y = nullptr;
    int N = 0, Cin = 0, H = 0, W = 0, Cout = 0;
    long long dup_off = 0;
};
int small_conv_in_launch(const SmallConvInArgs& a, hipStream_t stream);

struct SmallConvOutArgs {
    const half_t* x = nullptr;
    const half_t* w = nullptr;
    const half_t* b = nullptr;
    int N = 0, H = 0, W = 0, Cin = 0, Cout = 0;
    int mode = 0;
    const float* x_in = nullptr;
    const float* sigma = nullptr;
    float* out = nullptr;
    int in_mod = 0;
};
int small_conv_out_launch(const SmallConvOutArgs& a, hipStream_t stream);

int vae_out_finish_launch(const half_t* t8, float* out, long long npix, int cout, hipStream_t stream);

int small_pointwise_launch(const half_t* x, const half_t* w, const half_t* b, float* out, int N, int HW, int C, hipStream_t stream);

int timestep_embed_launch(const float* sigma, const float* log_sigmas, int n_sig, int N, int dim, half_t* out, float* t_out,
                          hipStream_t stream, int sigma_mod = 0);

struct DupArgs {
    char* base[3] = {nullptr, nullptr, nullptr};
    unsigned long long bytes[3] = {0, 0, 0};
    int count = 0;
};
int dup_halves_launch(const DupArgs& a, hipStream_t stream);

int repack_conv3x3_launch(const void* src, int src_is_f32, int O, int I, half_t* dst, hipStream_t stream);
int repack_rows_launch(const void* src, int src_is_f32, int rows, int cols, half_t* dst, int geglu_bn, hipStream_t stream);
int ctx_pad_launch(const void* src, int src_is_f32, int n, int T, int Tp, int D, half_t* dst, hipStream_t stream);
int fill_half_launch(half_t* dst, size_t n, float v, hipStream_t stream);

int cfg_combine_launch(const float* den2, float* out, float cfg, size_t n_half, hipStream_t stream);
int axpby_launch(float* x, float a, const float* y, float b, const float* z, float c, size_t n, hipStream_t stream);
int hook_check_launch(const void* a, const void* b, size_t words_ab, const void* x, size_t half_words_x, const void* sigma, int half_sigma,
                      int* flags, int epoch, hipStream_t stream);
int bislerp_launch(const float* x, float* tmp, float* y, int n, int c, int h, int w, int h_new, int w_new, hipStream_t stream);
```

### lightdiffusion_amd/csrc/misc.hip

```cpp
#include "kernels.h"

namespace {

template <int CIN>
__global__ __launch_bounds__(256) void small_conv_in_kernel(const SmallConvInArgs a) {
    extern __shared__ __attribute__((aligned(16))) char smem_raw[];
    half_t* wl = reinterpret_cast<half_t*>(smem_raw);
    constexpr int KK = 9 * CIN;
    if ((KK & 3) == 0) {
        for (int i = threadIdx.x; i < a.Cout * KK / 4; i += blockDim.x) {
            const int o = (i * 4) / KK, k = i * 4 - o * KK;
            const half4 v = *reinterpret_cast<const half4*>(a.w + (long long)i * 4);
#pragma unroll
            for (int e = 0; e < 4; ++e) wl[(k + e) * a.Cout + o] = v[e];
        }
    } else {
        for (int i = threadIdx.x; i < a.Cout * KK; i += blockDim.x) {
            const int o = i / KK, k = i - o * KK;
            wl[k * a.Cout + o] = a.w[i];
        }
    }
    float pw[CIN][CIN], pb[CIN];
    if (a.pre_w != nullptr) {
#pragma unroll
// ... 417 lines not shown

int axpby_launch(float* x, float a, const float* y, float b, const float* z, float c, size_t n, hipStream_t stream) {
    if (x == nullptr) return LD_ERR_ARG;
    hipLaunchKernelGGL(axpby_kernel, dim3(grid_for((long long)n, 256)), dim3(256), 0, stream, x, a, y, b, z, c, n);
    return hipGetLastError() == hipSuccess ? LD_OK : LD_ERR_HIP;
}

namespace {
__global__ __launch_bounds__(256) void ln_fold_kernel(const half_t* __restrict__ W, int K, const half_t* __restrict__ gamma,
                                                      const half_t* __restrict__ beta, const half_t* __restrict__ bias, half_t* __restrict__ Wout,
                                                      half_t* __restrict__ bout, float* __restrict__ wsum) {
    __shared__ float red[2][256];
    const int n = blockIdx.x, tid = threadIdx.x;
    float s = 0.f, sb = 0.f;
    for (int k = tid; k < K; k += 256) {
        const float w = (float)W[(long long)n * K + k];
        const half_t wf = (half_t)(w * (float)gamma[k]);
        Wout[(long long)n * K + k] = wf;
        s += (float)wf;
        sb += w * (float)beta[k];
    }
    red[0][tid] = s;
    red[1][tid] = sb;
    __syncthreads();
    for (int o = 128; o > 0; o >>= 1) {
        if (tid < o) {
            red[0][tid] += red[0][tid + o];
            red[1][tid] += red[1][tid + o];
        }
        __syncthreads();
    }
    if (tid == 0) {
        wsum[n] = red[0][0];
        bout[n] = (half_t)((bias != nullptr ? (float)bias[n] : 0.f) + red[1][0]);
    }
}
}

int ln_fold_launch(const half_t* W, int N, int K, const half_t* gamma, const half_t* beta, const half_t* bias, half_t* Wout, half_t* bout,
                   float* wsum, hipStream_t stream) {
    if (W == nullptr || gamma == nullptr || beta == nullptr || Wout == nullptr || bout == nullptr || wsum == nullptr || N <= 0 || K <= 0)
        return LD_ERR_ARG;
    hipLaunchKernelGGL(ln_fold_kernel, dim3(N), dim3(256), 0, stream, W, K, gamma, beta, bias, Wout, bout, wsum);
    return hipGetLastError() == hipSuccess ? LD_OK : LD_ERR_HIP;
}

namespace {
__global__ __launch_bounds__(256) void bislerp_axis_kernel(const float* __restrict__ x, float* __restrict__ y, int n, int c, int h,
                                                           int w, int len_new, int axis_w) {
    const int ho = axis_w ? h : len_new, wo = axis_w ? len_new : w;
    const long long total = (long long)n * ho * wo;
    for (long long idx = (long long)blockIdx.x * blockDim.x + threadIdx.x; idx < total; idx += (long long)gridDim.x * blockDim.x) {
    const int xo = (int)(idx % wo), yo = (int)((idx / wo) % ho), b = (int)(idx / ((long long)wo * ho));
    const int len_old = axis_w ? w : h, o = axis_w ? xo : yo;
    float pos = ((float)o + 0.5f) * ((float)len_old / (float)len_new) - 0.5f;
    pos = fmaxf(pos, 0.f);
    int lo = (int)floorf(pos);
    if (lo > len_old - 1) lo = len_old - 1;
    const int hi = lo + 1 < len_old ? lo + 1 : len_old - 1;
    const float r = lo >= len_old - 1 ? 0.f : pos - (float)lo;
    const long long plane = (long long)h * w;
    const float* pa = x + (long long)b * c * plane + (axis_w ? (long long)yo * w + lo : (long long)lo * w + xo);
    const float* pb = x + (long long)b * c * plane + (axis_w ? (long long)yo * w + hi : (long long)hi * w + xo);
    float na = 0.f, nb = 0.f, dot = 0.f;
    for (int ch = 0; ch < c; ++ch) {
        const float a = pa[ch * plane], bb = pb[ch * plane];
        na += a * a;
        nb += bb * bb;
        dot += a * bb;
    }
    na = sqrtf(na);
    nb = sqrtf(nb);
    const float ia = na > 0.f ? 1.f / na : 0.f, ib = nb > 0.f ? 1.f / nb : 0.f;
    dot *= ia * ib;
    const float om = acosf(dot), so = sinf(om);
    const float wa = sinf((1.f - r) * om) / so * ia, wb = sinf(r * om) / so * ib;
    const float mag = na * (1.f - r) + nb * r;
    const long long oplane = (long long)ho * wo;
    float* py = y + (long long)b * c * oplane + (long long)yo * wo + xo;
    for (int ch = 0; ch < c; ++ch) {
        const float a = pa[ch * plane], bb = pb[ch * plane];
        float v = (wa * a + wb * bb) * mag;
        if (dot > 1.f - 1e-5f) v = a;
        if (dot < 1e-5f - 1.f) v = a * (1.f - r) + bb * r;
        py[ch * oplane] = v;
    }
    }
}
}

int bislerp_launch(const float* x, float* tmp, float* y, int n, int c, int h, int w, int h_new, int w_new, hipStream_t stream) {
    if (x == nullptr || tmp == nullptr || y == nullptr || n <= 0 || c <= 0 || h <= 0 || w <= 0 || h_new <= 0 || w_new <= 0) return LD_ERR_ARG;
    hipLaunchKernelGGL(bislerp_axis_kernel, dim3(grid_for((long long)n * h * w_new, 256)), dim3(256), 0, stream, x, tmp, n, c, h, w, w_new, 1);
    hipLaunchKernelGGL(bislerp_axis_kernel, dim3(grid_for((long long)n * h_new * w_new, 256)), dim3(256), 0, stream, tmp, y, n, c, h, w_new,
                       h_new, 0);
    return hipGetLastError() == hipSuccess ? LD_OK : LD_ERR_HIP;
}

namespace {
__global__ __launch_bounds__(256) void mlp_out_fold_kernel(const half_t* __restrict__ Wpo, const half_t* __restrict__ W2, const half_t* __restrict__ b2,
                                                           const half_t* __restrict__ bpo, int C, half_t* __restrict__ Wout, half_t* __restrict__ bout) {
    extern __shared__ float wrow[];
    const int n = blockIdx.x, tid = threadIdx.x;
    const int H = 4 * C, K = 5 * C;
    for (int c = tid; c < C; c += 256) wrow[c] = (float)Wpo[(long long)n * C + c];
    __syncthreads();
    for (int k = tid; k < H; k += 256) {
        float s = 0.f;
        for (int c = 0; c < C; ++c) s += wrow[c] * (float)W2[(long long)c * H + k];
        Wout[(long long)n * K + k] = (half_t)s;
    }
    for (int c = tid; c < C; c += 256) Wout[(long long)n * K + H + c] = Wpo[(long long)n * C + c];
    if (tid == 0) {
        float s = (float)bpo[n];
        for (int c = 0; c < C; ++c) s += wrow[c] * (float)b2[c];
        bout[n] = (half_t)s;
    }
}
}

int mlp_out_fold_launch(const half_t* Wpo, const half_t* W2, const half_t* b2, const half_t* bpo, int C, half_t* Wout, half_t* bout, hipStream_t stream) {
    if (Wpo == nullptr || W2 == nullptr || b2 == nullptr || bpo == nullptr || Wout == nullptr || bout == nullptr || C <= 0) return LD_ERR_ARG;
    hipLaunchKernelGGL(mlp_out_fold_kernel, dim3(C), dim3(256), (size_t)C * sizeof(float), stream, Wpo, W2, b2, bpo, C, Wout, bout);
    return hipGetLastError() == hipSuccess ? LD_OK : LD_ERR_HIP;
}

namespace {
__global__ __launch_bounds__(256) void skip_fold_kernel(const uint4* __restrict__ W2, const uint4* __restrict__ Wsk, const half_t* __restrict__ b2,
                                                        const half_t* __restrict__ bsk, int N, int K9c, int SCc, uint4* __restrict__ Wout, half_t* __restrict__ bout) {
    const int Kc = K9c + SCc;
    const long long total = (long long)N * Kc;
    for (long long q = (long long)blockIdx.x * blockDim.x + threadIdx.x; q < total; q += (long long)gridDim.x * blockDim.x) {
        const int n = (int)(q / Kc), c = (int)(q - (long long)n * Kc);
        Wout[q] = c < K9c ? W2[(long long)n * K9c + c] : Wsk[(long long)n * SCc + (c - K9c)];
    }
    const int t = blockIdx.x * blockDim.x + threadIdx.x;
    if (t < N) bout[t] = (half_t)((float)b2[t] + (float)bsk[t]);
}
}

int skip_fold_launch(const half_t* W2, const half_t* Wsk, const half_t* b2, const half_t* bsk, int N, int K9, int SC, half_t* Wout, half_t* bout,
                     hipStream_t stream) {
    if (W2 == nullptr || Wsk == nullptr || b2 == nullptr || bsk == nullptr || Wout == nullptr || bout == nullptr || N <= 0 || K9 <= 0 || SC <= 0 ||
        (K9 & 7) || (SC & 7))
        return LD_ERR_ARG;
    const long long total = (long long)N * ((K9 + SC) / 8);
    int blocks = (int)((total + 255) / 256);
    if (blocks > 4096) blocks = 4096;
    if (blocks * 256 < N) blocks = (N + 255) / 256;
    hipLaunchKernelGGL(skip_fold_kernel, dim3(blocks), dim3(256), 0, stream, reinterpret_cast<const uint4*>(W2), reinterpret_cast<const uint4*>(Wsk), b2, bsk, N,
                       K9 / 8, SC / 8, reinterpret_cast<uint4*>(Wout), bout);
    return hipGetLastError() == hipSuccess ? LD_OK : LD_ERR_HIP;
}
```

### lightdiffusion_amd/csrc/unet.hip

```cpp
#include <cstring>

#include "runtime.h"
#include "../../include/ld_mi355x.h"

namespace {

struct ResW {
    std::string prefix;
    int cin = 0, cout = 0, emb_off = 0;
    int gn1_g, gn1_b, c1_w, c1_b, emb_w, emb_b, gn2_g, gn2_b, c2_w, c2_b, sk_w = -1, sk_b = -1;
    size_t f_c2_w = 0, f_c2_b = 0;
};
struct StW {
    int c = 0, bn = 0, ctx_slot = 0;
    size_t f_qk_w = 0, f_q2_w = 0, f_ff1_w = 0, f_qk_b = 0, f_q2_b = 0, f_ff1_b = 0, f_qk_s = 0, f_q2_s = 0,
           f_ff1_s = 0;
    size_t f_mo_w = 0, f_mo_b = 0;
    int gn_g, gn_b, pin_w, pin_b, ln1_g, ln1_b, q1_w, k1_w, v1_w, o1_w, o1_b, ln2_g, ln2_b, q2_w, k2_w, v2_w, o2_w, o2_b, ln3_g,
        ln3_b, ff1_w, ff1_b, ff2_w, ff2_b, pout_w, pout_b;
};
struct ConvW {
    int cin = 0, cout = 0, w = -1, b = -1;
};
enum LayerKind { L_CONV_IN, L_RES, L_ST, L_DOWN, L_UP };
struct Layer {
    int kind, idx;
};
struct Feat {
    half_t* p;
    int C, H, W;
    float* gn = nullptr;
    int gnP = 0;
};

}

struct ld_unet {
    ld_unet_config cfg;
    ParamTable pt;
    std::vector<ResW> res;
    std::vector<StW> st;
    std::vector<ConvW> convs;
    std::vector<std::vector<Layer>> in_blocks, out_blocks;
    std::vector<Layer> mid_block;
    int te0_w, te0_b, te2_w, te2_b, outn_g, outn_b, outc_w, outc_b;
    int emb_total = 0, ted = 0;
    Arena arena;
    char* ws_base = nullptr;
    size_t ws_bytes = 0;
    float* splitk_ws = nullptr;
    size_t splitk_bytes = 0;
    float* log_sigmas = nullptr;
    int max_n = 0, max_h = 0, max_w = 0, max_tok = 0;
    half_t* ctx16 = nullptr;
    std::vector<half_t*> ctx_k, ctx_vt;
    int ctx_n = 0, ctx_tok = 0, ctx_tpad = 0;
    int plan_n = 0, plan_h = 0, plan_w = 0, plan_pair = 0;
    int last_launches = 0;
    double last_flops = 0.0;
    int* sync_ws = nullptr;
    struct W8 { int slot, N, Cin; size_t off; };
    std::vector<W8> w8_list;
    std::vector<long long> w8_of_slot;
    char* w8_base = nullptr;
    size_t w8_bytes = 0;
    const half_t* w8(int slot) const {
        return (w8_base != nullptr && slot >= 0 && slot < (int)w8_of_slot.size() && w8_of_slot[slot] >= 0) ? reinterpret_cast<const half_t*>(w8_base + w8_of_slot[slot]) : nullptr;
    }
    void want_w8(int slot, int N, int Cin) {
        if (!conv8_weight_eligible(N, Cin)) return;
        w8_list.push_back({slot, N, Cin, w8_bytes});
        w8_bytes += (conv8_weight_bytes(N, Cin) + 255) / 256 * 256;
    }
    Timing timing;
    bool want_timing = false;
    char* fold_base = nullptr;
    size_t fold_bytes = 0;
    bool fold_dirty = true;
    bool ln_fold = false;
};

namespace {

std::string S(const char* fmt, int a = 0, int b = 0) {
    char buf[160];
    snprintf(buf, sizeof buf, fmt, a, b);
    return buf;
}

int add_res(ld_unet* u, const std::string& p, int cin, int cout) {
    ParamTable& t = u->pt;
    ResW r;
    r.prefix = p;
    r.cin = cin;
    r.cout = cout;
    r.gn1_g = t.add(p + ".in_layers.0.weight", PK_VEC, {cin});
    r.gn1_b = t.add(p + ".in_layers.0.bias", PK_VEC, {cin});
    r.c1_w = t.add(p + ".in_layers.2.weight", PK_CONV3, {cout, cin, 3, 3});
    r.c1_b = t.add(p + ".in_layers.2.bias", PK_VEC, {cout});
    u->want_w8(r.c1_w, cout, cin);
    r.gn2_g = t.add(p + ".out_layers.0.weight", PK_VEC, {cout});
    r.gn2_b = t.add(p + ".out_layers.0.bias", PK_VEC, {cout});
    r.c2_w = t.add(p + ".out_layers.3.weight", PK_CONV3, {cout, cout, 3, 3});
    r.c2_b = t.add(p + ".out_layers.3.bias", PK_VEC, {cout});
    u->want_w8(r.c2_w, cout, cout);
    if (cin != cout) {
        r.sk_w = t.add(p + ".skip_connection.weight", PK_MAT, {cout, cin, 1, 1});
        r.sk_b = t.add(p + ".skip_connection.bias", PK_VEC, {cout});
        size_t& fb = u->fold_bytes;
        r.f_c2_w = fb;
        fb += ((size_t)cout * (9 * cout + cin) * sizeof(half_t) + 255) / 256 * 256;
        r.f_c2_b = fb;
        fb += ((size_t)cout * sizeof(half_t) + 255) / 256 * 256;
    }
    r.emb_off = u->emb_total;
    u->emb_total += cout;
    u->res.push_back(r);
    return (int)u->res.size() - 1;
}

int add_st(ld_unet* u, const std::string& p, int c) {
    ParamTable& t = u->pt;
    const int ctx = u->cfg.context_dim;
    StW s;
    s.c = c;
    s.bn = gemm_pick_bn(8 * c);
    s.ctx_slot = (int)u->st.size();
    s.gn_g = t.add(p + ".norm.weight", PK_VEC, {c});
    s.gn_b = t.add(p + ".norm.bias", PK_VEC, {c});
    s.pin_w = t.add(p + ".proj_in.weight", PK_MAT, {c, c, 1, 1});
    s.pin_b = t.add(p + ".proj_in.bias", PK_VEC, {c});
    const std::string b = p + ".transformer_blocks.0";
    s.ln1_g = t.add(b + ".norm1.weight", PK_VEC, {c});
    s.ln1_b = t.add(b + ".norm1.bias", PK_VEC, {c});
    s.q1_w = t.add(b + ".attn1.to_q.weight", PK_MAT, {c, c});
    s.k1_w = t.add(b + ".attn1.to_k.weight", PK_MAT, {c, c}, 16);
    s.v1_w = t.add(b + ".attn1.to_v.weight", PK_MAT, {c, c}, 16);
    s.o1_w = t.add(b + ".attn1.to_out.0.weight", PK_MAT, {c, c});
    s.o1_b = t.add(b + ".attn1.to_out.0.bias", PK_VEC, {c});
    s.ln2_g = t.add(b + ".norm2.weight", PK_VEC, {c});
    s.ln2_b = t.add(b + ".norm2.bias", PK_VEC, {c});
    s.q2_w = t.add(b + ".attn2.to_q.weight", PK_MAT, {c, c});
    s.k2_w = t.add(b + ".attn2.to_k.weight", PK_MAT, {c, ctx});
    s.v2_w = t.add(b + ".attn2.to_v.weight", PK_MAT, {c, ctx});
    s.o2_w = t.add(b + ".attn2.to_out.0.weight", PK_MAT, {c, c});
    s.o2_b = t.add(b + ".attn2.to_out.0.bias", PK_VEC, {c});
    s.ln3_g = t.add(b + ".norm3.weight", PK_VEC, {c});
    s.ln3_b = t.add(b + ".norm3.bias", PK_VEC, {c});
    s.ff1_w = t.add(b + ".ff.net.0.proj.weight", PK_GEGLU_W, {8 * c, c}, 256, s.bn);
    s.ff1_b = t.add(b + ".ff.net.0.proj.bias", PK_GEGLU_B, {8 * c}, 256, s.bn);
    s.ff2_w = t.add(b + ".ff.net.2.weight", PK_MAT, {c, 4 * c});
    s.ff2_b = t.add(b + ".ff.net.2.bias", PK_VEC, {c});
    s.pout_w = t.add(p + ".proj_out.weight", PK_MAT, {c, c, 1, 1});
    s.pout_b = t.add(p + ".proj_out.bias", PK_VEC, {c});
    {
        size_t& fb = u->fold_bytes;
        auto take = [&](size_t bytes) {
            const size_t o = fb;
            fb += (bytes + 255) / 256 * 256;
            return o;
        };
        const size_t C = (size_t)c;
        s.f_qk_w = take(3 * C * C * sizeof(half_t));
        s.f_q2_w = take(C * C * sizeof(half_t));
        s.f_ff1_w = take(8 * C * C * sizeof(half_t));
        s.f_qk_b = take(3 * C * sizeof(half_t));
        s.f_q2_b = take(C * sizeof(half_t));
        s.f_ff1_b = take(8 * C * sizeof(half_t));
        s.f_qk_s = take(3 * C * sizeof(float));
        s.f_q2_s = take(C * sizeof(float));
        s.f_ff1_s = take(8 * C * sizeof(float));
        s.f_mo_w = take(5 * C * C * sizeof(half_t));
        s.f_mo_b = take(C * sizeof(half_t));
    }
    u->st.push_back(s);
    return (int)u->st.size() - 1;
}

int add_conv(ld_unet* u, const std::string& p, int cin, int cout) {
    ConvW c;
    c.cin = cin;
    c.cout = cout;
    c.w = u->pt.add(p + ".weight", PK_CONV3, {cout, cin, 3, 3});
    c.b = u->pt.add(p + ".bias", PK_VEC, {cout});
    u->convs.push_back(c);
    return (int)u->convs.size() - 1;
}

int build(ld_unet* u) {
    const ld_unet_config& c = u->cfg;
    if (c.num_levels < 1 || c.num_levels > 8 || c.model_channels % 32 || c.num_heads < 1) return LD_ERR_ARG;
    const int mc = c.model_channels;
    u->ted = mc * 4;
    ParamTable& t = u->pt;
    u->te0_w = t.add("time_embed.0.weight", PK_MAT, {u->ted, mc});
    u->te0_b = t.add("time_embed.0.bias", PK_VEC, {u->ted});
    u->te2_w = t.add("time_embed.2.weight", PK_MAT, {u->ted, u->ted});
    u->te2_b = t.add("time_embed.2.bias", PK_VEC, {u->ted});
    u->in_blocks.push_back({{L_CONV_IN, add_conv(u, "input_blocks.0.0", c.in_channels, mc)}});
    int ch = mc, idx = 1, td = 0;
    std::vector<int> chans{mc};
    for (int lvl = 0; lvl < c.num_levels; ++lvl) {
        for (int r = 0; r < c.num_res_blocks[lvl]; ++r) {
            std::vector<Layer> L;
            L.push_back({L_RES, add_res(u, S("input_blocks.%d.0", idx), ch, c.channel_mult[lvl] * mc)});
            ch = c.channel_mult[lvl] * mc;
            if (c.transformer_depth[td++] > 0) L.push_back({L_ST, add_st(u, S("input_blocks.%d.1", idx), ch)});
            u->in_blocks.push_back(L);
            chans.push_back(ch);
            ++idx;
        }
        if (lvl != c.num_levels - 1) {
            u->in_blocks.push_back({{L_DOWN, add_conv(u, S("input_blocks.%d.0.op", idx), ch, ch)}});
            chans.push_back(ch);
            ++idx;
        }
    }
    u->mid_block.push_back({L_RES, add_res(u, "middle_block.0", ch, ch)});
    if (c.transformer_depth_middle > 0) u->mid_block.push_back({L_ST, add_st(u, "middle_block.1", ch)});
    u->mid_block.push_back({L_RES, add_res(u, "middle_block.2", ch, ch)});
    int n_out = 0;
    for (int lvl = 0; lvl < c.num_levels; ++lvl) n_out += c.num_res_blocks[lvl] + 1;
    int tdo = n_out;
    idx = 0;
    for (int lvl = c.num_levels - 1; lvl >= 0; --lvl) {
        for (int i = 0; i <= c.num_res_blocks[lvl]; ++i) {
            const int ich = chans.back();
            chans.pop_back();
            std::vector<Layer> L;
            L.push_back({L_RES, add_res(u, S("output_blocks.%d.0", idx), ch + ich, mc * c.channel_mult[lvl])});
            ch = mc * c.channel_mult[lvl];
            int j = 1;
            if (c.transformer_depth_output[--tdo] > 0) {
                L.push_back({L_ST, add_st(u, S("output_blocks.%d.%d", idx, j), ch)});
                ++j;
            }
            if (lvl && i == c.num_res_blocks[lvl]) {
                L.push_back({L_UP, add_conv(u, S("output_blocks.%d.%d.conv", idx, j), ch, ch)});
                u->want_w8(u->convs.back().w, ch, ch);
            }
            u->out_blocks.push_back(L);
            ++idx;
        }
    }
    u->outn_g = t.add("out.0.weight", PK_VEC, {ch});
    u->outn_b = t.add("out.0.bias", PK_VEC, {ch});
    u->outc_w = t.add("out.2.weight", PK_CONV3, {c.out_channels, mc, 3, 3});
    u->outc_b = t.add("out.2.bias", PK_VEC, {c.out_channels});
    for (size_t i = 0; i < u->res.size(); ++i)
        u->res[i].emb_w = t.add(u->res[i].prefix + ".emb_layers.1.weight", PK_MAT, {u->res[i].cout, u->ted}, i == 0 ? 256 : 16);
    for (size_t i = 0; i < u->res.size(); ++i)
        u->res[i].emb_b = t.add(u->res[i].prefix + ".emb_layers.1.bias", PK_VEC, {u->res[i].cout}, i == 0 ? 256 : 16);
    return t.finalize();
}

struct Run {
    ld_unet* u;
    Exec ex;
    int n;
    int n_alloc = 0;
    bool pair_pending = false;
    const half_t* emb_all;
    half_t* P(int slot) const { return u->pt.ptr(slot); }
    int na() const { return n_alloc > 0 ? n_alloc : n; }
    void dup(void* base, size_t half_bytes) {
        ex.launches += 1;
        ex.t_begin(KC_MISC, 0.0, 1, "dup", (long long)half_bytes, 0, 0, 1);
        if (!ex.dry && ex.status == LD_OK &&
            hipMemcpyAsync(static_cast<char*>(base) + half_bytes, base, half_bytes, hipMemcpyDeviceToDevice, ex.stream) != hipSuccess)
            ex.note(LD_ERR_HIP);
        ex.t_end("hipMemcpyAsync(pair)");
    }

    void want_stats(GemmParams& p, float* buf, int HW, int* done) {
        p.gn_part = buf;
        p.gn_P = gn_num_chunks(n, HW);
        p.gn_HW = HW;
        p.gn_ppb = (HW + p.gn_P - 1) / p.gn_P;
        p.gn_part_done = done;
    }

    half_t* conv3(const half_t* x1, int C1, const half_t* x2, int C2, int Hs, int Ws, int Hv, int Wv, int stride, int wslot, int bslot,
                  int cout, const half_t* rowvec, int ldrv, const half_t* R, half_t* out, int* Ho_, int* Wo_, int ksize = 3, float* stats = nullptr,
                  int* stats_done = nullptr) {
        const int Ho = ksize == 3 ? (Hv - 1) / stride + 1 : Hv, Wo = ksize == 3 ? (Wv - 1) / stride + 1 : Wv;
        GemmParams p;
        p.conv = 1;
        p.ksize = ksize;
        p.A = x1; p.A2 = x2; p.C1 = C1; p.C2 = C2;
        p.Hs = Hs; p.Ws = Ws; p.Hv = Hv; p.Wv = Wv; p.Ho = Ho; p.Wo = Wo; p.stride = stride;
        p.W = P(wslot); p.ldw = ksize * ksize * (C1 + C2);
        p.W8 = ksize == 3 ? u->w8(wslot) : nullptr;
        p.M = n * Ho * Wo; p.N = cout; p.K = ksize * ksize * (C1 + C2);
        p.bias_n = P(bslot);
        p.rowvec = rowvec; p.rows_per_vec = Ho * Wo; p.ldrv = ldrv;
        p.R = R; p.ldr = cout;
        p.C = out; p.ldc = cout;
        if (stats != nullptr) want_stats(p, stats, Ho * Wo, stats_done);
        ex.gemm(p);
        if (Ho_) *Ho_ = Ho;
        if (Wo_) *Wo_ = Wo;
        return out;
    }

    void linear(const half_t* x, int lda, int wslot, int bslot, const half_t* R, half_t* y, int M, int N, int K, int act = 0, int bn = 0) {
        GemmParams p;
        p.A = x; p.lda = lda;
        p.W = P(wslot); p.ldw = K;
        p.M = M; p.N = N; p.K = K;
        p.bias_n = bslot >= 0 ? P(bslot) : nullptr;
        p.R = R; p.ldr = (act == 2 ? N / 2 : N);
        p.act = act; p.bn = bn;
        p.C = y; p.ldc = (act == 2 ? N / 2 : N);
        ex.gemm(p);
    }

    Feat resblock(const ResW& r, const half_t* x1, int C1, const half_t* x2, int C2, int H, int W, float* in_stats = nullptr, int in_P = 0) {
        Arena& ar = *ex.arena;
        const size_t M = (size_t)na() * H * W;
        half_t* out = ar.halfs(M * r.cout);
        float* gno = reinterpret_cast<float*>(ar.alloc(groupnorm_workspace_bytes(na(), H * W)));
        int gno_done = 0;
        if (C2 != 0) in_stats = nullptr;
        const size_t mk = ar.mark();
        auto conv_params = [&](const half_t* a1, int c1, const half_t* a2, int c2, int wslot, int bslot, const half_t* rowvec, int ldrv, const half_t* R,
                               half_t* dst) {
            GemmParams p;
            p.conv = 1; p.ksize = 3;
            p.A = a1; p.A2 = a2; p.C1 = c1; p.C2 = c2;
            p.Hs = H; p.Ws = W; p.Hv = H; p.Wv = W; p.Ho = H; p.Wo = W; p.stride = 1;
            p.W = P(wslot); p.ldw = 9 * (c1 + c2);
            p.W8 = u->w8(wslot);
            p.M = n * H * W; p.N = r.cout; p.K = 9 * (c1 + c2);
            p.bias_n = P(bslot);
            p.rowvec = rowvec; p.rows_per_vec = H * W; p.ldrv = ldrv;
            p.R = R; p.ldr = r.cout;
            p.C = dst; p.ldc = r.cout;
            return p;
        };
        half_t* g1 = ar.halfs(M * r.cin);
        half_t* h1 = ar.halfs(M * r.cout);
        const half_t* skip = x1;
        bool fold_skip = false;
        if (r.sk_w >= 0) {
            GemmParams probe = conv_params(h1, r.cout, nullptr, 0, r.c2_w, r.c2_b, nullptr, 0, nullptr, out);
            fold_skip = u->ln_fold && u->fold_base != nullptr && ex.conv_takes_skip_segment(probe);
            half_t* sk = (!fold_skip || ex.dry) ? ar.halfs(M * r.cout) : nullptr;
            if (!fold_skip) {
                conv3(x1, C1, x2, C2, H, W, H, W, 1, r.sk_w, r.sk_b, r.cout, nullptr, 0, nullptr, sk, nullptr, nullptr, 1);
                skip = sk;
            }
        }
        float* gnp = reinterpret_cast<float*>(ar.alloc(groupnorm_workspace_bytes(na(), H * W)));
        int gnp_done = 0;
        {
            GemmParams c1 = conv_params(x1, C1, x2, C2, r.c1_w, r.c1_b, emb_all + r.emb_off, u->emb_total, nullptr, h1);
            want_stats(c1, gnp, H * W, &gnp_done);
            ex.gn_silu_conv(c1, n, H * W, P(r.gn1_g), P(r.gn1_b), 1e-5f, g1, in_stats, in_P);
        }
        half_t* g2 = g1;
        if (r.cout > r.cin) g2 = ar.halfs(M * r.cout);
        {
            GemmParams c2 = conv_params(h1, r.cout, nullptr, 0, r.c2_w, r.c2_b, nullptr, 0, skip, out);
            if (fold_skip) {
                c2.S1 = x1; c2.SC1 = C1; c2.S2 = x2; c2.SC2 = C2;
                c2.W = reinterpret_cast<const half_t*>(u->fold_base + r.f_c2_w);
                c2.K = 9 * r.cout + r.cin; c2.ldw = c2.K;
                c2.bias_n = reinterpret_cast<const half_t*>(u->fold_base + r.f_c2_b);
                c2.R = nullptr;
                c2.W8 = nullptr;
            }
            want_stats(c2, gno, H * W, &gno_done);
            ex.gn_silu_conv(c2, n, H * W, P(r.gn2_g), P(r.gn2_b), 1e-5f, g2, gnp_done ? gnp : nullptr, gnp_done);
        }
        ar.release(mk);
        return {out, r.cout, H, W, gno_done ? gno : nullptr, gno_done};
    }

    Feat transformer(const StW& s, const half_t* x, int H, int W, float* in_stats = nullptr, int in_P = 0) {
        Arena& ar = *ex.arena;
        const int C = s.c, L = H * W, heads = u->cfg.num_heads, d = C / heads;
        int M = n * L;
        const size_t Ma = (size_t)na() * L;
        half_t* out = ar.halfs(Ma * C);
        float* gno = reinterpret_cast<float*>(ar.alloc(groupnorm_workspace_bytes(na(), L)));
        int gno_done = 0;
        const size_t mk = ar.mark();
        half_t* g = ar.halfs(Ma * C);
        ex.groupnorm(x, C, nullptr, 0, n, L, P(s.gn_g), P(s.gn_b), 1e-6f, 0, g, in_stats, in_P);
        half_t* t = ar.halfs(Ma * C);
        half_t* nrm = g;
        half_t* qkv = ar.halfs(Ma * 3 * C);
        half_t* ao = ar.halfs(Ma * C);
        half_t* ff = nullptr;
        const bool fold = u->ln_fold;
        float* stat = fold ? reinterpret_cast<float*>(ar.alloc((size_t)((C + 63) / 64) * Ma * 2 * sizeof(float))) : nullptr;
        int parts = 0;
        char* fb = u->fold_base;
        auto producer = [&](const half_t* x_, int lda, int wslot, int bslot, const half_t* R, int K) {
            GemmParams p;
            p.A = x_; p.lda = lda;
            p.W = P(wslot); p.ldw = K;
            p.M = M; p.N = C; p.K = K;
            p.bias_n = P(bslot);
            p.R = R; p.ldr = C;
            p.C = t; p.ldc = C;
            if (fold) {
                p.stat_out = stat;
                p.stat_parts_out = &parts;
            }
            ex.gemm(p);
        };
        auto ln_args = [&](GemmParams& p, size_t wsum_off) {
            p.ln_stat = stat; p.ln_parts = parts; p.ln_rows = M;
            p.ln_inv_c = 1.0f / (float)C; p.ln_eps = 1e-5f;
            p.ln_wsum = reinterpret_cast<const float*>(fb + wsum_off);
        };
        producer(g, C, s.pin_w, s.pin_b, nullptr, C);
        if (!fold) ex.layernorm(t, P(s.ln1_g), P(s.ln1_b), nrm, M, C);
        {
            GemmParams p;
            p.A = fold ? t : nrm; p.lda = C;
            p.W = fold ? reinterpret_cast<const half_t*>(fb + s.f_qk_w) : P(s.q1_w); p.ldw = C;
            p.M = M; p.N = 3 * C; p.K = C;
            p.C = qkv; p.ldc = 3 * C;
            if (fold) {
                p.bias_n = reinterpret_cast<const half_t*>(fb + s.f_qk_b);
                ln_args(p, s.f_qk_s);
            }
            ex.gemm(p);
        }
        {
            AttnParams a;
            a.Q = qkv; a.ldq = 3 * C; a.sQ = (long long)L * 3 * C;
            a.K = qkv + C; a.ldk = 3 * C; a.sK = (long long)L * 3 * C;
            a.V = qkv + 2 * C; a.ldv = 3 * C; a.sV = (long long)L * 3 * C;
            a.O = ao; a.ldo = C; a.sO = (long long)L * C;
            a.B = n; a.H = heads; a.Lq = L; a.Lk = L; a.d = d;
            a.scale = 1.0f / sqrtf((float)d);
            ex.attention(a);
        }
        const bool split_here = pair_pending;
        producer(ao, C, s.o1_w, s.o1_b, t, C);
        if (!fold) ex.layernorm(t, P(s.ln2_g), P(s.ln2_b), nrm, M, C);
        half_t* q2 = qkv;
        {
            GemmParams p;
            p.A = fold ? t : nrm; p.lda = C;
            p.W = fold ? reinterpret_cast<const half_t*>(fb + s.f_q2_w) : P(s.q2_w); p.ldw = C;
            p.M = M; p.N = C; p.K = C;
            p.C = q2; p.ldc = C;
            if (fold) {
                p.bias_n = reinterpret_cast<const half_t*>(fb + s.f_q2_b);
                ln_args(p, s.f_q2_s);
            }
            ex.gemm(p);
        }
        if (split_here) {
            const size_t hb = (size_t)M * C * sizeof(half_t);
            DupArgs da;
            da.count = 3;
            da.base[0] = reinterpret_cast<char*>(t); da.base[1] = reinterpret_cast<char*>(q2); da.base[2] = reinterpret_cast<char*>(const_cast<half_t*>(x));
            da.bytes[0] = da.bytes[1] = da.bytes[2] = hb;
            ex.launches += 1;
            ex.t_begin(KC_MISC, 0.0, 1, "dup3", (long long)hb, 0, 0, 1);
            if (!ex.dry && ex.status == LD_OK) ex.note(dup_halves_launch(da, ex.stream));
            ex.t_end("dup_halves_kernel");
            pair_pending = false;
            n = n_alloc;
            M = n * L;
        }
        {
            const int Tp = u->ctx_tpad;
            AttnParams a;
            a.Q = q2; a.ldq = C; a.sQ = (long long)L * C;
            a.K = u->ctx_k[s.ctx_slot]; a.ldk = C; a.sK = (long long)Tp * C;
            a.Vt = u->ctx_vt[s.ctx_slot]; a.ldvt = Tp; a.sV = (long long)C * Tp;
            a.O = ao; a.ldo = C; a.sO = (long long)L * C;
            a.B = n; a.H = heads; a.Lq = L; a.Lk = u->ctx_tok; a.d = d;
            a.scale = 1.0f / sqrtf((float)d);
            ex.attention(a);
        }
        producer(ao, C, s.o2_w, s.o2_b, t, C);
        if (!fold) ex.layernorm(t, P(s.ln3_g), P(s.ln3_b), nrm, M, C);
        ff = ar.halfs(Ma * 4 * C);
        {
            GemmParams p;
            p.A = fold ? t : nrm; p.lda = C;
            p.W = fold ? reinterpret_cast<const half_t*>(fb + s.f_ff1_w) : P(s.ff1_w); p.ldw = C;
            p.M = M; p.N = 8 * C; p.K = C;
            p.bias_n = fold ? reinterpret_cast<const half_t*>(fb + s.f_ff1_b) : P(s.ff1_b);
            p.act = 2; p.bn = s.bn;
            p.C = ff; p.ldc = 4 * C; p.ldr = 4 * C;
            if (fold) ln_args(p, s.f_ff1_s);
            ex.gemm(p);
        }
        if (fold) {
            GemmParams p;
            p.conv = 1; p.ksize = 1;
            p.A = ff; p.A2 = t; p.C1 = 4 * C; p.C2 = C;
            p.Hs = p.Hv = p.Ho = H; p.Ws = p.Wv = p.Wo = W; p.stride = 1;
            p.W = reinterpret_cast<const half_t*>(fb + s.f_mo_w); p.ldw = 5 * C;
            p.M = M; p.N = C; p.K = 5 * C;
            p.bias_n = reinterpret_cast<const half_t*>(fb + s.f_mo_b);
            p.R = x; p.ldr = C;
            p.C = out; p.ldc = C;
            want_stats(p, gno, L, &gno_done);
            ex.gemm(p);
        } else {
            linear(ff, 4 * C, s.ff2_w, s.ff2_b, t, t, M, C, 4 * C);
            linear(t, C, s.pout_w, s.pout_b, x, out, M, C, C);
        }
        ar.release(mk);
        return {out, C, H, W, gno_done ? gno : nullptr, gno_done};
    }
};

int fold_layernorms(ld_unet* u, hipStream_t stream) {
    for (const StW& s : u->st) {
        const int C = s.c;
        char* fb = u->fold_base;
        auto H = [&](size_t off) { return reinterpret_cast<half_t*>(fb + off); };
        auto F = [&](size_t off) { return reinterpret_cast<float*>(fb + off); };
        const half_t* P_q1 = u->pt.ptr(s.q1_w);
        int st = ln_fold_launch(P_q1, 3 * C, C, u->pt.ptr(s.ln1_g), u->pt.ptr(s.ln1_b), nullptr, H(s.f_qk_w), H(s.f_qk_b), F(s.f_qk_s), stream);
        if (st == LD_OK) st = ln_fold_launch(u->pt.ptr(s.q2_w), C, C, u->pt.ptr(s.ln2_g), u->pt.ptr(s.ln2_b), nullptr, H(s.f_q2_w), H(s.f_q2_b), F(s.f_q2_s), stream);
        if (st == LD_OK) st = ln_fold_launch(u->pt.ptr(s.ff1_w), 8 * C, C, u->pt.ptr(s.ln3_g), u->pt.ptr(s.ln3_b), u->pt.ptr(s.ff1_b), H(s.f_ff1_w), H(s.f_ff1_b), F(s.f_ff1_s), stream);
        if (st == LD_OK) st = mlp_out_fold_launch(u->pt.ptr(s.pout_w), u->pt.ptr(s.ff2_w), u->pt.ptr(s.ff2_b), u->pt.ptr(s.pout_b), C, H(s.f_mo_w), H(s.f_mo_b), stream);
        if (st != LD_OK) return st;
    }
    for (const ResW& r : u->res) {
        if (r.sk_w < 0) continue;
        const int st = skip_fold_launch(u->pt.ptr(r.c2_w), u->pt.ptr(r.sk_w), u->pt.ptr(r.c2_b), u->pt.ptr(r.sk_b), r.cout, 9 * r.cout, r.cin,
                                        reinterpret_cast<half_t*>(u->fold_base + r.f_c2_w), reinterpret_cast<half_t*>(u->fold_base + r.f_c2_b), stream);
        if (st != LD_OK) return st;
    }
    u->fold_dirty = false;
    return LD_OK;
}

int derive_conv8_weights(ld_unet* u, hipStream_t stream) {
    for (const ld_unet::W8& w : u->w8_list) {
        const int st = conv8_repack_launch(u->pt.ptr(w.slot), w.N, w.Cin, reinterpret_cast<half_t*>(u->w8_base + w.off), stream);
        if (st != LD_OK) return st;
    }
    return LD_OK;
}

int run_forward(ld_unet* u, bool dry, const float* x, const float* sigma, float* out, int n, int h, int w, int eps_only, hipStream_t stream,
                size_t* dry_peak = nullptr, bool pair = false) {
    if (!dry && u->fold_dirty) {
        if (u->w8_base != nullptr) {
            const int st = derive_conv8_weights(u, stream);
            if (st != LD_OK) return st;
        }
        if (u->ln_fold) {
            const int st = fold_layernorms(u, stream);
            if (st != LD_OK) return st;
        }
        u->fold_dirty = false;
    }
    if (pair && (n & 1)) return LD_ERR_SHAPE;
    Run R;
    R.u = u;
    R.n = n;
    R.n_alloc = n;
    Exec& ex = R.ex;
    ex.stream = stream;
    ex.dry = dry;
    Arena plan;
    ex.arena = dry ? &plan : &u->arena;
    ex.splitk_ws = u->splitk_ws;
    ex.splitk_bytes = u->splitk_bytes;
    ex.sync_ws = u->sync_ws;
    if (u->want_timing && !dry) {
        u->timing.reset();
        ex.timing = &u->timing;
    }
    Arena& ar = *ex.arena;
    ar.release(0);
    const ld_unet_config& c = u->cfg;
    const int mc = c.model_channels, ted = u->ted;
    const int in_mod = pair ? n / 2 : 0;
    if (pair) R.pair_pending = true;

    half_t* temb = ar.halfs((size_t)n * mc);
    ex.launches += 1;
    ex.t_begin(KC_MISC, 0.0, 1);
    if (!dry) ex.note(timestep_embed_launch(sigma, u->log_sigmas, 1000, n, mc, temb, nullptr, stream, in_mod));
    ex.t_end("timestep_embed_kernel");
    half_t* e1 = ar.halfs((size_t)n * ted);
    R.linear(temb, mc, u->te0_w, u->te0_b, nullptr, e1, n, ted, mc, 1);
    half_t* semb = ar.halfs((size_t)n * ted);
    R.linear(e1, ted, u->te2_w, u->te2_b, nullptr, semb, n, ted, ted, 1);
    half_t* emb_all = ar.halfs((size_t)n * u->emb_total);
    R.linear(semb, ted, u->res[0].emb_w, u->res[0].emb_b, nullptr, emb_all, n, u->emb_total, ted);
    R.emb_all = emb_all;

    auto run_layers = [&](const std::vector<Layer>& layers, Feat f, const half_t* x2, int C2, int outH, int outW) -> Feat {
        for (const Layer& L : layers) {
            switch (L.kind) {
                case L_RES: {
                    f = R.resblock(u->res[L.idx], f.p, f.C, x2, C2, f.H, f.W, f.gn, f.gnP);
                    x2 = nullptr;
                    C2 = 0;
                    break;
                }
                case L_ST: f = R.transformer(u->st[L.idx], f.p, f.H, f.W, f.gn, f.gnP); break;
                case L_DOWN: {
                    const ConvW& cw = u->convs[L.idx];
                    const int Ho = (f.H - 1) / 2 + 1, Wo = (f.W - 1) / 2 + 1;
                    if (R.pair_pending) {
                        R.dup(const_cast<half_t*>(f.p), (size_t)R.n * f.H * f.W * f.C * sizeof(half_t));
                        R.pair_pending = false;
                        R.n = n;
                    }
                    half_t* o = ar.halfs((size_t)n * Ho * Wo * cw.cout);
                    float* gno = reinterpret_cast<float*>(ar.alloc(groupnorm_workspace_bytes(n, Ho * Wo)));
                    int gno_done = 0;
                    R.conv3(f.p, f.C, nullptr, 0, f.H, f.W, f.H, f.W, 2, cw.w, cw.b, cw.cout, nullptr, 0, nullptr, o, nullptr, nullptr, 3, gno, &gno_done);
                    f = {o, cw.cout, Ho, Wo, gno_done ? gno : nullptr, gno_done};
                    break;
                }
                case L_UP: {
                    const ConvW& cw = u->convs[L.idx];
                    const int Hv = outH > 0 ? outH : f.H * 2, Wv = outW > 0 ? outW : f.W * 2;
                    half_t* o = ar.halfs((size_t)n * Hv * Wv * cw.cout);
                    R.conv3(f.p, f.C, nullptr, 0, f.H, f.W, Hv, Wv, 1, cw.w, cw.b, cw.cout, nullptr, 0, nullptr, o, nullptr, nullptr);
                    f = {o, cw.cout, Hv, Wv};
                    break;
                }
                default: break;
            }
        }
        return f;
    };

    std::vector<Feat> hs;
    Feat f{nullptr, 0, h, w};
    {
        const ConvW& cw = u->convs[u->in_blocks[0][0].idx];
        half_t* o = ar.halfs((size_t)n * h * w * mc);
        if (R.pair_pending) R.n = n / 2;
        SmallConvInArgs a;
        a.x = x; a.scale_sigma = sigma; a.w = u->pt.ptr(cw.w); a.b = u->pt.ptr(cw.b); a.y = o;
        a.N = R.n; a.Cin = c.in_channels; a.H = h; a.W = w; a.Cout = mc;
        if (R.pair_pending) a.dup_off = (long long)R.n * h * w * mc;
        ex.launches += 1;
        ex.flops += 2.0 * R.n * h * w * mc * 9.0 * c.in_channels;
        ex.t_begin(KC_MISC, 2.0 * R.n * h * w * mc * 9.0 * c.in_channels, 1);
        if (!dry) ex.note(small_conv_in_launch(a, stream));
        ex.t_end("small_conv_in_kernel");
        f = {o, mc, h, w};
        hs.push_back(f);
    }
    for (size_t b = 1; b < u->in_blocks.size(); ++b) {
        f = run_layers(u->in_blocks[b], f, nullptr, 0, 0, 0);
        if (R.pair_pending && b == 1) {
            R.dup(const_cast<half_t*>(f.p), (size_t)R.n * f.H * f.W * f.C * sizeof(half_t));
            R.pair_pending = false;
            R.n = n;
            f.gn = nullptr;
            f.gnP = 0;
        }
        hs.push_back(f);
    }
    if (R.pair_pending) {
        R.pair_pending = false;
        R.n = n;
    }
    f = run_layers(u->mid_block, f, nullptr, 0, 0, 0);
    for (size_t b = 0; b < u->out_blocks.size(); ++b) {
        const Feat skip = hs.back();
        hs.pop_back();
        if (skip.H != f.H || skip.W != f.W) ex.note(LD_ERR_SHAPE);
        const int oh = hs.empty() ? 0 : hs.back().H, ow = hs.empty() ? 0 : hs.back().W;
        f = run_layers(u->out_blocks[b], f, skip.p, skip.C, oh, ow);
    }
    {
        half_t* g = ar.halfs((size_t)n * f.H * f.W * f.C);
        ex.groupnorm(f.p, f.C, nullptr, 0, n, f.H * f.W, u->pt.ptr(u->outn_g), u->pt.ptr(u->outn_b), 1e-5f, 1, g, f.gn, f.gnP);
        SmallConvOutArgs a;
        a.x = g; a.w = u->pt.ptr(u->outc_w); a.b = u->pt.ptr(u->outc_b);
        a.N = n; a.H = f.H; a.W = f.W; a.Cin = f.C; a.Cout = c.out_channels;
        a.mode = eps_only ? 2 : 0;
        a.x_in = x; a.sigma = sigma; a.out = out; a.in_mod = in_mod;
        ex.launches += 1;
        ex.flops += 2.0 * n * f.H * f.W * f.C * 9.0 * c.out_channels;
        ex.t_begin(KC_MISC, 2.0 * n * f.H * f.W * f.C * 9.0 * c.out_channels, 1);
        if (!dry) ex.note(small_conv_out_launch(a, stream));
        ex.t_end("small_conv_out_kernel");
    }
    u->last_launches = ex.launches;
    u->last_flops = ex.flops;
    if (dry_peak) *dry_peak = ar.peak;
    return ex.status;
}

}

extern "C" {

int ld_unet_create(const ld_unet_config* cfg, ld_unet** out) {
    if (cfg == nullptr || out == nullptr) return LD_ERR_ARG;
    ld_unet* u = new ld_unet();
    u->cfg = *cfg;
    const int st = build(u);
    if (st != LD_OK) {
        u->pt.destroy();
        delete u;
        return st;
    }
    std::vector<float> ls(1000);
    {
        const double b0 = sqrt(0.00085), b1 = sqrt(0.012);
        double ac = 1.0;
        for (int i = 0; i < 1000; ++i) {
            const double sb = b0 + (b1 - b0) * (double)i / 999.0;
            ac *= 1.0 - sb * sb;
            ls[i] = (float)log(sqrt((1.0 - ac) / ac));
        }
    }
    u->w8_of_slot.assign(u->pt.slots.size(), -1);
    for (const ld_unet::W8& w : u->w8_list) u->w8_of_slot[w.slot] = (long long)w.off;
    if (u->w8_bytes > 0 && hipMalloc((void**)&u->w8_base, u->w8_bytes) != hipSuccess) u->w8_base = nullptr;
    u->ln_fold = gemm_ln_fold_available();
    if (u->ln_fold && u->fold_bytes > 0 && hipMalloc((void**)&u->fold_base, u->fold_bytes) != hipSuccess) {
        u->pt.destroy();
        delete u;
        return LD_ERR_HIP;
    }
    if (hipMalloc((void**)&u->sync_ws, LD_SYNC_INTS * sizeof(int)) != hipSuccess || hipMemset(u->sync_ws, 0, LD_SYNC_INTS * sizeof(int)) != hipSuccess ||
        hipMalloc((void**)&u->log_sigmas, 1000 * sizeof(float)) != hipSuccess ||
        hipMemcpy(u->log_sigmas, ls.data(), 1000 * sizeof(float), hipMemcpyHostToDevice) != hipSuccess) {
        u->pt.destroy();
        delete u;
        return LD_ERR_HIP;
    }
    *out = u;
    return LD_OK;
}

void ld_unet_destroy(ld_unet* u) {
    if (u == nullptr) return;
    u->pt.destroy();
    u->timing.destroy();
    if (u->ws_base) (void)hipFree(u->ws_base);
    if (u->log_sigmas) (void)hipFree(u->log_sigmas);
    if (u->sync_ws) (void)hipFree(u->sync_ws);
    if (u->w8_base) (void)hipFree(u->w8_base);
    if (u->fold_base) (void)hipFree(u->fold_base);
    delete u;
}

int ld_unet_param_count(const ld_unet* u) { return u ? (int)u->pt.slots.size() : 0; }

int ld_unet_param_info(const ld_unet* u, int i, const char** name, int* ndim, int64_t shape[4]) {
    if (u == nullptr || i < 0 || i >= (int)u->pt.slots.size()) return LD_ERR_ARG;
    const ParamSlot& s = u->pt.slots[i];
    if (name) *name = s.name.c_str();
    if (ndim) *ndim = s.ndim;
    if (shape)
        for (int k = 0; k < 4; ++k) shape[k] = s.shape[k];
    return LD_OK;
}

int ld_unet_load_param(ld_unet* u, const char* name, const void* src, int dtype, void* stream) {
    if (u == nullptr || name == nullptr) return LD_ERR_ARG;
    u->fold_dirty = true;
    return u->pt.load(name, src, dtype, (hipStream_t)stream);
}

size_t ld_unet_workspace_bytes(const ld_unet* u) { return u ? u->ws_bytes : 0; }
size_t ld_unet_weight_bytes(const ld_unet* u) { return u ? u->pt.bytes + (u->fold_base ? u->fold_bytes : 0) + (u->w8_base ? u->w8_bytes : 0) : 0; }

int ld_unet_reserve(ld_unet* u, int max_n, int max_h, int max_w, int max_tok) {
    if (u == nullptr || max_n < 1 || max_h < 1 || max_w < 1 || max_tok < 1) return LD_ERR_ARG;
    if (u->ws_base) {
        (void)hipFree(u->ws_base);
        u->ws_base = nullptr;
    }
    u->arena = Arena();
    u->plan_n = u->plan_h = u->plan_w = u->plan_pair = 0;
    u->ctx_tok = max_tok;
    u->ctx_tpad = (max_tok + 7) & ~7;
    u->ctx_k.assign(u->st.size(), nullptr);
    u->ctx_vt.assign(u->st.size(), nullptr);
    size_t peak = 0;
    int st = run_forward(u, true, nullptr, nullptr, nullptr, max_n, max_h, max_w, 0, nullptr, &peak);
    if (st != LD_OK) return st;
    if (!(max_n & 1)) {
        size_t peak2 = 0;
        st = run_forward(u, true, nullptr, nullptr, nullptr, max_n, max_h, max_w, 0, nullptr, &peak2, true);
        if (st != LD_OK) return st;
        if (peak2 > peak) peak = peak2;
    }
    const size_t act = (peak + 4095) / 4096 * 4096;
    const size_t tpad = (size_t)u->ctx_tpad;
    size_t ctxb = ((size_t)max_n * tpad * u->cfg.context_dim * sizeof(half_t) + 255) / 256 * 256;
    for (const StW& s : u->st) ctxb += 2 * (((size_t)max_n * tpad * s.c * sizeof(half_t) + 255) / 256 * 256);
    u->splitk_bytes = (size_t)96 << 20;
    u->ws_bytes = act + ctxb + u->splitk_bytes + 4096;
    if (hipMalloc((void**)&u->ws_base, u->ws_bytes) != hipSuccess) {
        u->ws_base = nullptr;
        return LD_ERR_HIP;
    }
    char* p = u->ws_base;
    u->arena.base = p;
    u->arena.cap = act;
    u->arena.off = u->arena.peak = 0;
    p += act;
    u->splitk_ws = reinterpret_cast<float*>(p);
    p += u->splitk_bytes;
    u->ctx16 = reinterpret_cast<half_t*>(p);
    p += ((size_t)max_n * tpad * u->cfg.context_dim * sizeof(half_t) + 255) / 256 * 256;
    for (size_t i = 0; i < u->st.size(); ++i) {
        const size_t b = ((size_t)max_n * tpad * u->st[i].c * sizeof(half_t) + 255) / 256 * 256;
        u->ctx_k[i] = reinterpret_cast<half_t*>(p);
        p += b;
        u->ctx_vt[i] = reinterpret_cast<half_t*>(p);
        p += b;
    }
    if (getenv("LD_PROFILE_DUMP") != nullptr)
        fprintf(stderr, "[ld_reserve] workspace %p (%zu MiB)  weights %p  folds %p  conv8 weights %p\n", (void*)u->ws_base, u->ws_bytes >> 20, (void*)u->pt.base,
                (void*)u->fold_base, (void*)u->w8_base);
    u->max_n = max_n;
    u->max_h = max_h;
    u->max_w = max_w;
    u->max_tok = max_tok;
    u->ctx_n = 0;
    return LD_OK;
}

int ld_unet_set_context(ld_unet* u, const void* ctx, int dtype, int n, int tokens, void* stream_) {
    if (u == nullptr || ctx == nullptr) return LD_ERR_ARG;
    if (u->ws_base == nullptr || !u->pt.all_loaded()) return LD_ERR_STATE;
    if (n < 1 || n > u->max_n || tokens < 1 || tokens > u->max_tok) return LD_ERR_SHAPE;
    hipStream_t stream = (hipStream_t)stream_;
    const int D = u->cfg.context_dim, Tp = (tokens + 7) & ~7;
    int st = ctx_pad_launch(ctx, dtype == LD_F32, n, tokens, Tp, D, u->ctx16, stream);
    if (st != LD_OK) return st;
    for (size_t i = 0; i < u->st.size(); ++i) {
        const StW& s = u->st[i];
        GemmParams k;
        k.A = u->ctx16; k.lda = D;
        k.W = u->pt.ptr(s.k2_w); k.ldw = D;
        k.M = n * Tp; k.N = s.c; k.K = D;
        k.C = u->ctx_k[i]; k.ldc = s.c;
        st = gemm_launch(k, stream);
        if (st != LD_OK) return st;
        GemmParams v;
        v.A = u->pt.ptr(s.v2_w); v.lda = D; v.sA = 0;
        v.W = u->ctx16; v.ldw = D; v.sW = (long long)Tp * D;
        v.M = s.c; v.N = Tp; v.K = D; v.batch = n;
        v.C = u->ctx_vt[i]; v.ldc = Tp; v.sC = (long long)s.c * Tp;
        st = gemm_launch(v, stream);
        if (st != LD_OK) return st;
    }
    u->ctx_n = n;
    u->ctx_tok = tokens;
    u->ctx_tpad = Tp;
    return LD_OK;
}

static int forward_checked(ld_unet* u, const float* x, const float* sigma, float* out, int n, int h, int w, int eps_only, void* stream, bool pair) {
    if (u == nullptr || x == nullptr || sigma == nullptr || out == nullptr) return LD_ERR_ARG;
    if (u->ws_base == nullptr || !u->pt.all_loaded() || u->ctx_n == 0) return LD_ERR_STATE;
    if (n != u->ctx_n) return LD_ERR_SHAPE;
    if (n > u->max_n || h < 1 || w < 1) return LD_ERR_SHAPE;
    int st = LD_OK;
    if (n != u->plan_n || h != u->plan_h || w != u->plan_w || (int)pair != u->plan_pair) {
        size_t peak = 0;
        st = run_forward(u, true, nullptr, nullptr, nullptr, n, h, w, eps_only, nullptr, &peak, pair);
        if (st != LD_OK) return st;
        if (peak > u->arena.cap) return LD_ERR_SHAPE;
        u->plan_n = n;
        u->plan_h = h;
        u->plan_w = w;
        u->plan_pair = (int)pair;
    }
    return run_forward(u, false, x, sigma, out, n, h, w, eps_only, (hipStream_t)stream, nullptr, pair);
}

int ld_unet_forward(ld_unet* u, const float* x, const float* sigma, float* out, int n, int h, int w, int eps_only, void* stream) {
    return forward_checked(u, x, sigma, out, n, h, w, eps_only, stream, false);
}

int ld_unet_forward_pair(ld_unet* u, const float* x, const float* sigma, float* out, int nb, int h, int w, void* stream) {
    if (nb < 1) return LD_ERR_SHAPE;
    return forward_checked(u, x, sigma, out, 2 * nb, h, w, 0, stream, true);
}

static int profile_any(ld_unet* u, const float* x, const float* sigma, float* out, int n, int h, int w, void* stream, double ms[6], double flops[6],
                       int launches[6], bool pair);

int ld_unet_profile(ld_unet* u, const float* x, const float* sigma, float* out, int n, int h, int w, void* stream, double ms[6],
                    double flops[6], int launches[6]) {
    return profile_any(u, x, sigma, out, n, h, w, stream, ms, flops, launches, false);
}

int ld_unet_profile_pair(ld_unet* u, const float* x, const float* sigma, float* out, int nb, int h, int w, void* stream, double ms[6],
                         double flops[6], int launches[6]) {
    return profile_any(u, x, sigma, out, 2 * nb, h, w, stream, ms, flops, launches, true);
}

static int profile_any(ld_unet* u, const float* x, const float* sigma, float* out, int n, int h, int w, void* stream, double ms[6], double flops[6],
                       int launches[6], bool pair) {
    if (u == nullptr || ms == nullptr || flops == nullptr || launches == nullptr) return LD_ERR_ARG;
    u->want_timing = true;
    int st = forward_checked(u, x, sigma, out, n, h, w, 0, stream, pair);
    u->want_timing = false;
    if (st != LD_OK) return st;
    if (hipStreamSynchronize((hipStream_t)stream) != hipSuccess) return LD_ERR_HIP;
    u->timing.collect();
    for (int i = 0; i < KC_COUNT; ++i) {
        ms[i] = u->timing.ms[i];
        flops[i] = u->timing.flops[i];
        launches[i] = u->timing.launches[i];
    }
    return LD_OK;
}

int ld_unet_profile_kernels(const ld_unet* u, char* buf, size_t buf_bytes) {
    if (u == nullptr || buf == nullptr || buf_bytes == 0) return LD_ERR_ARG;
    size_t off = 0;
    buf[0] = 0;
    for (const auto& kv : u->timing.per_kernel) {
        const int w = snprintf(buf + off, buf_bytes - off, "%s\t%d\t%.6f\t%.0f\n", kv.first.c_str(), kv.second.launches, kv.second.ms, kv.second.flops);
        if (w < 0 || (size_t)w >= buf_bytes - off) return LD_ERR_ARG;
        off += (size_t)w;
    }
    return LD_OK;
}

int ld_unet_profile_launches(const ld_unet* u, char* buf, size_t buf_bytes) {
    if (u == nullptr) return LD_ERR_ARG;
    return u->timing.format_launches(buf, buf_bytes);
}

int ld_unet_last_launches(const ld_unet* u) { return u ? u->last_launches : 0; }
double ld_unet_last_flops(const ld_unet* u) { return u ? u->last_flops : 0.0; }

}
```

### lightdiffusion_amd/ops.py

```python
from __future__ import annotations

import math
from typing import Optional

import torch

from ._lib import F16, F32, check, lib


def _stream() -> int:
    return torch.cuda.current_stream().cuda_stream


def _p(t: Optional[torch.Tensor]) -> Optional[int]:
    if t is None:
        return None
    assert t.is_cuda and t.is_contiguous(), "device-resident contiguous tensors only"
    return t.data_ptr()


def last_kernel() -> str:
    return lib().ld_op_last_kernel().decode()


_WS = {}


def _ws(nbytes: int, device) -> torch.Tensor:
    d = torch.device(device)
    idx = d.index if d.index is not None else torch.cuda.current_device()
    n = max(nbytes, 256)
    if torch.cuda.is_current_stream_capturing():
        return torch.empty(n, dtype=torch.uint8, device=device)
    key = (idx, torch.cuda.current_stream(idx).cuda_stream)
    buf = _WS.get(key)
    if buf is None or buf.numel() < n:
        buf = torch.empty(n, dtype=torch.uint8, device=device)
        _WS[key] = buf
    return buf[:n]


def linear(x: torch.Tensor, weight: torch.Tensor, bias: Optional[torch.Tensor] = None, residual: Optional[torch.Tensor] = None,
           act: str = "none", alpha: float = 1.0) -> torch.Tensor:
    code = {"none": 0, "silu": 1, "geglu": 2, "quick_gelu": 3}[act]
    K = x.shape[-1]
    N = weight.shape[0]
    M = x.numel() // K
    y = torch.empty(*x.shape[:-1], N // 2 if code == 2 else N, dtype=torch.float16, device=x.device)
    ws = _ws(64 << 20, x.device)
    check(lib().ld_op_linear(_p(x), _p(weight), _p(bias), _p(residual), _p(y), M, N, K, alpha, code, _p(ws), ws.numel(), _stream()),
          "ld_op_linear")
    return y


def linear_ln(x: torch.Tensor, w_prod: torch.Tensor, b_prod: Optional[torch.Tensor], gamma: torch.Tensor, beta: torch.Tensor,
              weight: torch.Tensor, bias: Optional[torch.Tensor], eps: float = 1e-5):
    M, C = x.shape
    N = weight.shape[0]
    t = torch.empty(M, C, dtype=torch.float16, device=x.device)
    y = torch.empty(M, N, dtype=torch.float16, device=x.device)
    ws = _ws(2 * N * C + 8 * N + 8 * ((C + 63) // 64) * M + 4096, x.device)
    check(lib().ld_op_linear_ln(_p(x), _p(w_prod), _p(b_prod), _p(gamma), _p(beta), _p(weight), _p(bias), _p(t), _p(y), M, C, N, eps,
                                _p(ws), ws.numel(), _stream()), "ld_op_linear_ln")
    return t, y


def linear_ln_geglu(x: torch.Tensor, w_prod: torch.Tensor, b_prod: Optional[torch.Tensor], gamma: torch.Tensor, beta: torch.Tensor,
                    weight: torch.Tensor, bias: torch.Tensor, eps: float = 1e-5):
    M, C = x.shape
    N = weight.shape[0]
    t = torch.empty(M, C, dtype=torch.float16, device=x.device)
    y = torch.empty(M, N // 2, dtype=torch.float16, device=x.device)
    ws = _ws(4 * N * C + 12 * N + 8 * ((C + 63) // 64) * M + 4096, x.device)
    check(lib().ld_op_linear_ln_geglu(_p(x), _p(w_prod), _p(b_prod), _p(gamma), _p(beta), _p(weight), _p(bias), _p(t), _p(y), M, C, N, eps,
                                      _p(ws), ws.numel(), _stream()), "ld_op_linear_ln_geglu")
    return t, y


def repack_conv_weight(w_oihw: torch.Tensor) -> torch.Tensor:
    O, I, kh, kw = w_oihw.shape
    w_oihw = w_oihw.contiguous()
    out = torch.empty(O, kh * kw * I, dtype=torch.float16, device=w_oihw.device)
    if kh == 3:
        check(lib().ld_op_repack_conv(_p(w_oihw), F32 if w_oihw.dtype == torch.float32 else F16, O, I, _p(out), _stream()),
              "ld_op_repack_conv")
    else:
        out.copy_(w_oihw.reshape(O, I))
    return out


def conv2d(x: torch.Tensor, w_packed: torch.Tensor, bias: Optional[torch.Tensor], ksize: int = 3, stride: int = 1,
           x2: Optional[torch.Tensor] = None, out_hw: Optional[tuple] = None, rowvec: Optional[torch.Tensor] = None,
           residual: Optional[torch.Tensor] = None) -> torch.Tensor:
    n, h, w, c1 = x.shape
    c2 = 0 if x2 is None else x2.shape[-1]
    hv, wv = (h, w) if out_hw is None else out_hw
    cout = w_packed.shape[0]
    ho = (hv - 1) // stride + 1 if ksize == 3 else hv
    wo = (wv - 1) // stride + 1 if ksize == 3 else wv
    y = torch.empty(n, ho, wo, cout, dtype=torch.float16, device=x.device)
    ws = _ws(192 << 20, x.device)
    check(lib().ld_op_conv(_p(x), c1, _p(x2), c2, n, h, w, hv, wv, stride, ksize, _p(w_packed), _p(bias), _p(rowvec), _p(residual),
                           _p(y), cout, _p(ws), ws.numel(), _stream()), "ld_op_conv")
    return y


def conv2d_skip(x: torch.Tensor, w_packed: torch.Tensor, bias: torch.Tensor, s1: torch.Tensor, s2: Optional[torch.Tensor], w_skip: torch.Tensor,
                b_skip: torch.Tensor, rowvec: Optional[torch.Tensor] = None) -> torch.Tensor:
    n, h, w, c = x.shape
    sc1 = s1.shape[-1]
    sc2 = 0 if s2 is None else s2.shape[-1]
    cout = w_packed.shape[0]
    y = torch.empty(n, h, w, cout, dtype=torch.float16, device=x.device)
    ws = _ws(lib().ld_op_conv_skip_ws_bytes(c, sc1, sc2, cout), x.device)
    check(lib().ld_op_conv_skip(_p(x), c, n, h, w, _p(w_packed), _p(bias), _p(s1), sc1, _p(s2), sc2, _p(w_skip), _p(b_skip), _p(rowvec), _p(y), cout,
                                _p(ws), ws.numel(), _stream()), "ld_op_conv_skip")
    return y


def conv2d_gn_partials(x: torch.Tensor, w_packed: torch.Tensor, bias: Optional[torch.Tensor], out_hw: Optional[tuple] = None,
                       residual: Optional[torch.Tensor] = None):
    import ctypes
    n, h, w, c = x.shape
    hv, wv = (h, w) if out_hw is None else out_hw
    cout = w_packed.shape[0]
    y = torch.empty(n, hv, wv, cout, dtype=torch.float16, device=x.device)
    part = torch.zeros(lib().ld_op_conv_gn_partials_floats(n, hv * wv), dtype=torch.float32, device=x.device)
    chunks = ctypes.c_int(0)
    ws = _ws(192 << 20, x.device)
    check(lib().ld_op_conv_gn_partials(_p(x), c, n, h, w, hv, wv, _p(w_packed), _p(bias), _p(residual), _p(y), cout, _p(part), ctypes.byref(chunks),
                                       _p(ws), ws.numel(), _stream()), "ld_op_conv_gn_partials")
    if chunks.value == 0:
        return y, None
    return y, part[: n * chunks.value * 64].view(n, chunks.value, 32, 2)


def group_norm_silu_conv2d(x: torch.Tensor, gamma: torch.Tensor, beta: torch.Tensor, eps: float, w_packed: torch.Tensor,
                           bias: Optional[torch.Tensor], x2: Optional[torch.Tensor] = None, rowvec: Optional[torch.Tensor] = None,
                           residual: Optional[torch.Tensor] = None) -> torch.Tensor:
    n, h, w, c1 = x.shape
    c2 = 0 if x2 is None else x2.shape[-1]
    cout = w_packed.shape[0]
    y = torch.empty(n, h, w, cout, dtype=torch.float16, device=x.device)
    ws = _ws(lib().ld_op_groupnorm_conv_ws_bytes(c1, c2, n, h, w, cout), x.device)
    check(lib().ld_op_groupnorm_conv(_p(x), c1, _p(x2), c2, n, h, w, _p(gamma), _p(beta), eps, _p(w_packed), _p(bias), _p(rowvec), _p(residual),
                                     _p(y), cout, _p(ws), ws.numel(), _stream()), "ld_op_groupnorm_conv")
    return y


def group_norm(x: torch.Tensor, gamma: torch.Tensor, beta: torch.Tensor, eps: float, silu: bool = False,
               x2: Optional[torch.Tensor] = None) -> torch.Tensor:
    n, c1 = x.shape[0], x.shape[-1]
    hw = x.numel() // (n * c1)
    c2 = 0 if x2 is None else x2.shape[-1]
    y = torch.empty(*x.shape[:-1], c1 + c2, dtype=torch.float16, device=x.device)
    ws = _ws(lib().ld_op_groupnorm_ws_bytes(n, hw), x.device)
    check(lib().ld_op_groupnorm(_p(x), c1, _p(x2), c2, n, hw, _p(gamma), _p(beta), eps, int(silu), _p(y), _p(ws), _stream()),
          "ld_op_groupnorm")
    return y


def layer_norm(x: torch.Tensor, gamma: torch.Tensor, beta: torch.Tensor, eps: float = 1e-5) -> torch.Tensor:
    c = x.shape[-1]
    y = torch.empty_like(x)
    check(lib().ld_op_layernorm(_p(x), _p(gamma), _p(beta), _p(y), x.numel() // c, c, eps, _stream()), "ld_op_layernorm")
    return y


def attention(q: torch.Tensor, k: torch.Tensor, v: torch.Tensor, heads: int, causal: bool = False) -> torch.Tensor:
    b, lq, c = q.shape
    lk = k.shape[1]
    d = c // heads
    lkp = (lk + 7) // 8 * 8
    vt = torch.zeros(b, c, lkp, dtype=torch.float16, device=q.device)
    vt[:, :, :lk] = v.transpose(1, 2)
    o = torch.empty_like(q)
    check(lib().ld_op_attention(_p(q), c, _p(k.contiguous()), c, _p(vt), lkp, _p(o), c, b, heads, lq, lk, d, 1.0 / math.sqrt(d), int(causal), _stream()),
          "ld_op_attention")
    return o


def attention_qkv(qkv: torch.Tensor, heads: int, causal: bool = False) -> torch.Tensor:
    b, l, c3 = qkv.shape
    c = c3 // 3
    d = c // heads
    o = torch.empty(b, l, c, dtype=torch.float16, device=qkv.device)
    base = qkv.data_ptr()
    check(lib().ld_op_attention_rowv(base, c3, base + 2 * c, c3, base + 4 * c, c3, _p(o), c, b, heads, l, l, d, 1.0 / math.sqrt(d), int(causal),
                                     _stream()), "ld_op_attention_rowv")
    return o


def attention_rowv(q: torch.Tensor, k: torch.Tensor, v: torch.Tensor, heads: int, causal: bool = False) -> torch.Tensor:
    b, lq, c = q.shape
    lk = k.shape[1]
    d = c // heads
    o = torch.empty_like(q)
# ... 143 lines not shown
```

Before: 60.15 steps/s.

## Fold cross-attention Q/K/V/O projections into per-context GEMMs with fused group softmax

For cross-attention with at most 80 context tokens, the query projection is folded into the keys (G = K·Wq per head) and the values into the output projection (Z), once per conditioning update. Each denoise step then runs the cross-attention as a GEMM with a fused per-80-column softmax epilogue (new act code 4) followed by a second GEMM, in place of the separate q2 projection, attention kernel and output projection. LayerNorm stats, bias and wsum are now indexed per batch so the LN fold works with batched folded weights. The cost is extra workspace and fold kernels run whenever the context changes, and K grows to heads*80 for the folded GEMMs.

```diff
diff --git a/lightdiffusion_amd/csrc/gemm.h b/lightdiffusion_amd/csrc/gemm.h
--- a/lightdiffusion_amd/csrc/gemm.h
+++ b/lightdiffusion_amd/csrc/gemm.h
@@ -29,6 +29,7 @@
     const half_t* R = nullptr;
     int ldr = 0;
     int act = 0;
+    long long sBias = 0, sWsum = 0;
     half_t* C = nullptr;
     int ldc = 0;
     int bm = 0, bn = 0;
@@ -46,6 +47,7 @@
     float ln_inv_c = 0.f, ln_eps = 0.f;
     const float* ln_wsum = nullptr;
     int ln_swapped = 0;
+    int ln_zmod = 0;
     const float* gn_scale = nullptr;
     const float* gn_shift = nullptr;
     int gn_silu = 0;
diff --git a/lightdiffusion_amd/csrc/gemm.hip b/lightdiffusion_amd/csrc/gemm.hip
--- a/lightdiffusion_amd/csrc/gemm.hip
+++ b/lightdiffusion_amd/csrc/gemm.hip
@@ -47,7 +47,7 @@
     EpiPre<BM, BN> e;
     e.bias_done = bias_done;
     constexpr int CPR = EpiPre<BM, BN>::CPR, GRP = EpiPre<BM, BN>::GRP;
-    e.fast = (BM * CPR) % NT == 0 && m0 + BM <= p.M && n0 + BN <= p.N && p.act == 0 && p.bias_m == nullptr && bias_done;
+    e.fast = (BM * CPR) % NT == 0 && m0 + BM <= p.M && n0 + BN <= p.N && (p.act == 0 || p.act == 4) && p.bias_m == nullptr && bias_done;
 #pragma unroll
     for (int k = 0; k < GRP; ++k) e.r[k] = zero16();
     if (e.fast && p.R != nullptr) {
@@ -189,7 +189,7 @@
                         s1 += t.x;
                         s2 += t.y;
                     }
-                    *reinterpret_cast<float2*>(p.stat_out + ((long long)(n0 / BN) * p.M + m0 + tid) * 2) = make_float2(s1, s2);
+                    *reinterpret_cast<float2*>(p.stat_out + (((long long)(n0 / BN) * p.batch + z) * p.M + m0 + tid) * 2) = make_float2(s1, s2);
                 }
             }
             return;
@@ -254,7 +254,7 @@
                     s1 += lds_scratch[(tid * CPR + c) * 2];
                     s2 += lds_scratch[(tid * CPR + c) * 2 + 1];
                 }
-                float* o = p.stat_out + ((long long)(n0 / BN) * p.M + m0 + tid) * 2;
+                float* o = p.stat_out + (((long long)(n0 / BN) * p.batch + z) * p.M + m0 + tid) * 2;
                 o[0] = s1;
                 o[1] = s2;
             }
@@ -286,7 +286,7 @@
     const int cnt = p.ln_swapped ? BN : BM;
     if (tid >= cnt) return;
     const bool ok = p.ln_swapped ? (n0 + tid < p.n_valid) : (m0 + tid < p.M);
-    const long long row = p.ln_swapped ? (long long)z * p.ln_zrows + n0 + tid : (long long)m0 + tid;
+    const long long row = p.ln_swapped ? (long long)z * p.ln_zrows + n0 + tid : (long long)(p.ln_zmod > 0 ? z % p.ln_zmod : z) * p.M + m0 + tid;
     float s1 = 0.f, s2 = 0.f;
     if (ok) ln_sum_parts(p.ln_stat + row * 2, (long long)p.ln_rows * 2, p.ln_parts, s1, s2);
     const float mu = s1 * p.ln_inv_c;
@@ -331,10 +331,10 @@
 __device__ uint4 g_zero_row[4096];
 
 template <int BN>
-__device__ __forceinline__ void epi_stage_load(const GemmParams& p, int n0, int t, f32x4& b, f32x4& w) {
+__device__ __forceinline__ void epi_stage_load(const GemmParams& p, int z, int n0, int t, f32x4& b, f32x4& w) {
     const char* zp = reinterpret_cast<const char*>(g_zero_row);
-    const char* bp = (t < BN / 8 && p.bias_n != nullptr && n0 + t * 8 < p.N) ? reinterpret_cast<const char*>(p.bias_n + n0 + t * 8) : zp;
-    const char* wp = (t < BN / 4 && p.ln_wsum != nullptr && !p.ln_swapped && n0 + t * 4 < p.N) ? reinterpret_cast<const char*>(p.ln_wsum + n0 + t * 4) : zp;
+    const char* bp = (t < BN / 8 && p.bias_n != nullptr && n0 + t * 8 < p.N) ? reinterpret_cast<const char*>(p.bias_n + (long long)z * p.sBias + n0 + t * 8) : zp;
+    const char* wp = (t < BN / 4 && p.ln_wsum != nullptr && !p.ln_swapped && n0 + t * 4 < p.N) ? reinterpret_cast<const char*>(p.ln_wsum + (long long)z * p.sWsum + n0 + t * 4) : zp;
     asm volatile("global_load_dwordx4 %0, %1, off" : "=&v"(b) : "v"(bp) : "memory");
     asm volatile("global_load_dwordx4 %0, %1, off" : "=&v"(w) : "v"(wp) : "memory");
 }
@@ -356,8 +356,39 @@
         : "memory");
 }
 
-template <int BM, int BN, bool CONV, int NST>
+template <int TM, int TN>
+__device__ __forceinline__ void softmax80_rows(f32x4 (&acc)[TM][TN], float alpha) {
+    static_assert(TN == 5, "one 80-column group per wave");
+#pragma unroll
+    for (int i = 0; i < TM; ++i) {
+        float mx = -INFINITY;
+#pragma unroll
+        for (int j = 0; j < TN; ++j) {
+            acc[i][j] *= alpha;
+            mx = fmaxf(mx, fmaxf(fmaxf(acc[i][j][0], acc[i][j][1]), fmaxf(acc[i][j][2], acc[i][j][3])));
+        }
+        mx = fmaxf(mx, __shfl_xor(mx, 16));
+        mx = fmaxf(mx, __shfl_xor(mx, 32));
+        float sum = 0.f;
+#pragma unroll
+        for (int j = 0; j < TN; ++j) {
+#pragma unroll
+            for (int r = 0; r < 4; ++r) {
+                acc[i][j][r] = __builtin_amdgcn_exp2f(acc[i][j][r] - mx);
+                sum += acc[i][j][r];
+            }
+        }
+        sum += __shfl_xor(sum, 16);
+        sum += __shfl_xor(sum, 32);
+        const float inv = 1.0f / sum;
+#pragma unroll
+        for (int j = 0; j < TN; ++j) acc[i][j] *= inv;
+    }
+}
+
+template <int BM, int BN, bool CONV, int NST, bool SMX = false>
 __global__ __launch_bounds__(NT, NST == 2 ? 2 : 1) void gemm3_kernel(const GemmParams p) {
+    static_assert(!SMX || (BN == 160 && !CONV), "group softmax: two 80-column groups per tile");
     constexpr int BK3 = 64, PF = NST - 1;
     static_assert(NST == 2 || NST == 4, "ring depth");
     constexpr int WTM = BM / 2, WTN = BN / 2;
@@ -541,7 +572,7 @@
         }
     };
     f32x4 est_b, est_w;
-    epi_stage_load<BN>(p, n0, tid, est_b, est_w);
+    epi_stage_load<BN>(p, z, n0, tid, est_b, est_w);
 #pragma unroll
     for (int t = 0; t < PF; ++t) issue(kt_begin + t, t);
     if (p.ln_stat != nullptr) ln_prepare<BM, BN>(p, ln_mu, ln_rs, z, m0, n0, tid);
@@ -551,8 +582,8 @@
     wait_slab(kt_begin);
     __builtin_amdgcn_s_barrier();
     issue(kt_begin + PF, PF);
-    const bool bias_acc = splitk == 1 && p.ln_stat == nullptr && (p.act == 0 || p.act == 2);
-    const bool bias_done = bias_acc || (splitk == 1 && p.ln_stat != nullptr && !p.ln_swapped && (p.act == 0 || p.act == 2));
+    const bool bias_acc = splitk == 1 && p.ln_stat == nullptr && (p.act == 0 || p.act == 2 || SMX);
+    const bool bias_done = bias_acc || (splitk == 1 && p.ln_stat != nullptr && !p.ln_swapped && (p.act == 0 || p.act == 2 || SMX));
     if (bias_acc) {
         const float inv_alpha = 1.0f / p.alpha;
 #pragma unroll
@@ -610,13 +641,14 @@
     half_t* Cs = smem;
     const EpiPre<BM, BN> pre = epi_prefetch_residual<BM, BN>(p, z, m0, n0, tid, bias_done);
     if (p.ln_stat != nullptr) ln_apply<TM, TN>(p, acc, ln_mu, ln_rs, m0, n0, wm0, wn0, fr, fq, wsum_s, bias_s, bias_done);
+    if constexpr (SMX) softmax80_rows<TM, TN>(acc, p.alpha);
 #pragma unroll
     for (int i = 0; i < TM; ++i) {
         const int ml = wm0 + i * 16 + fr;
 #pragma unroll
         for (int j = 0; j < TN; ++j) {
             const int nl = wn0 + j * 16 + fq * 4;
-            const f32x4 v = acc[i][j] * p.alpha;
+            const f32x4 v = SMX ? acc[i][j] : acc[i][j] * p.alpha;
             *reinterpret_cast<uint2*>(Cs + ml * CLD + nl) = make_uint2(pk2h(v[0], v[1]), pk2h(v[2], v[3]));
         }
     }
@@ -635,8 +667,9 @@
     }
 }
 
-template <int BM, int BN, bool CONV, int NST = 4, int WPS = 2>
+template <int BM, int BN, bool CONV, int NST = 4, int WPS = 2, bool SMX = false>
 __global__ __launch_bounds__(2 * NT, WPS) void gemm4_kernel(const GemmParams p) {
+    static_assert(!SMX || (BN == 160 && !CONV), "group softmax: two 80-column groups per tile");
     constexpr int BK3 = 64;
     static_assert((NST & (NST - 1)) == 0 && NST >= 4, "ring depth");
     constexpr int WTM = BM / 2, WTN = BN / 2;
@@ -803,7 +836,7 @@
 
     {
         f32x4 est_b, est_w;
-        epi_stage_load<BN>(p, n0, tid, est_b, est_w);
+        epi_stage_load<BN>(p, z, n0, tid, est_b, est_w);
         EPI_STAGE_WAIT(0, est_b, est_w);
         epi_stage_store<BN>(est_b, est_w, bias_s, wsum_s, tid);
     }
@@ -833,8 +866,8 @@
             for (int j = 0; j < TN; ++j) acc[i][j] = __builtin_amdgcn_mfma_f32_16x16x32_f16(fb[j], fa[i], acc[i][j], 0, 0, 0);
     };
     __builtin_amdgcn_s_barrier();
-    const bool bias_acc = splitk == 1 && p.ln_stat == nullptr && (p.act == 0 || p.act == 2);
-    const bool bias_done = bias_acc || (splitk == 1 && p.ln_stat != nullptr && !p.ln_swapped && (p.act == 0 || p.act == 2));
+    const bool bias_acc = splitk == 1 && p.ln_stat == nullptr && (p.act == 0 || p.act == 2 || SMX);
+    const bool bias_done = bias_acc || (splitk == 1 && p.ln_stat != nullptr && !p.ln_swapped && (p.act == 0 || p.act == 2 || SMX));
     if (bias_acc) {
         const float inv_alpha = 1.0f / p.alpha;
 #pragma unroll
@@ -889,13 +922,14 @@
     half_t* Cs = smem;
     const EpiPre<BM, BN> pre = epi_prefetch_residual<BM, BN>(p, z, m0, n0, tid, bias_done);
     if (p.ln_stat != nullptr) ln_apply<TM, TN>(p, acc, ln_mu, ln_rs, m0, n0, wm0, wn0, fr, fq, wsum_s, bias_s, bias_done);
+    if constexpr (SMX) softmax80_rows<TM, TN>(acc, p.alpha);
 #pragma unroll
     for (int i = 0; i < TM; ++i) {
         const int ml = wm0 + i * 16 + fr;
 #pragma unroll
         for (int j = 0; j < TN; ++j) {
             const int nl = wn0 + j * 16 + fq * 4;
-            const f32x4 v = acc[i][j] * p.alpha;
+            const f32x4 v = SMX ? acc[i][j] : acc[i][j] * p.alpha;
             *reinterpret_cast<uint2*>(Cs + ml * CLD + nl) = make_uint2(pk2h(v[0], v[1]), pk2h(v[2], v[3]));
         }
     }
@@ -2176,6 +2210,20 @@
     const int tiles = ((p.M + BM - 1) / BM) * ((p.N + BN - 1) / BN);
     const int sk = p.splitk > 1 ? p.splitk : 1;
     dim3 grid(tiles * sk, 1, p.batch);
+    if constexpr (BN == 160) {
+        if (p.act == 4) {
+            if ((long long)tiles * p.batch <= V4_MAX_BLOCKS) {
+                static const std::string name = "xattn_gemm4_kernel<" + std::to_string(BM) + ",160,softmax80>";
+                t_last_kernel = name.c_str();
+                hipLaunchKernelGGL((gemm4_kernel<BM, BN, false, 4, 2, true>), grid, dim3(2 * NT), 0, s, p);
+            } else {
+                static const std::string name = "xattn_gemm3_kernel<" + std::to_string(BM) + ",160,softmax80>";
+                t_last_kernel = name.c_str();
+                hipLaunchKernelGGL((gemm3_kernel<BM, BN, false, 2, true>), grid, dim3(NT), 0, s, p);
+            }
+            return;
+        }
+    }
     if constexpr (BM == 64 && BN == 64) {
         const long long blocks = (long long)tiles * sk * p.batch;
         if (!p.conv && blocks > V4_MAX_BLOCKS && blocks <= 512 && p.K >= 640) {
@@ -2374,6 +2422,14 @@
         return LD_ERR_SHAPE;
     }
     if (p.act == 2 && (p.bias_n == nullptr || (p.N & 15))) return LD_ERR_ARG;
+    if (p.act == 4) {
+        if (p.conv || (p.N % 160) || p.ln_swapped || p.bias_m != nullptr || p.splitk > 1 || (p.bn != 0 && p.bn != 160) || (p.n_valid > 0 && p.n_valid < p.N)) return LD_ERR_ARG;
+        p.bn = 160;
+        p.splitk = 1;
+    } else if (p.sBias != 0 || p.sWsum != 0) {
+        return LD_ERR_ARG;
+    }
+    if (p.ln_zmod != 0 && (p.act != 4 || p.ln_stat == nullptr || p.ln_zmod < 0)) return LD_ERR_ARG;
     if (p.R != nullptr && (p.ldr & 7)) return LD_ERR_SHAPE;
 
     if (p.n_valid <= 0 || p.n_valid > p.N) p.n_valid = p.N;
diff --git a/lightdiffusion_amd/csrc/kernels.h b/lightdiffusion_amd/csrc/kernels.h
--- a/lightdiffusion_amd/csrc/kernels.h
+++ b/lightdiffusion_amd/csrc/kernels.h
@@ -42,6 +42,20 @@
 int mlp_out_fold_launch(const half_t* Wpo, const half_t* W2, const half_t* b2, const half_t* bpo, int C, half_t* Wout, half_t* bout, hipStream_t stream);
 int skip_fold_launch(const half_t* W2, const half_t* Wsk, const half_t* b2, const half_t* bsk, int N, int K9, int SC, half_t* Wout, half_t* bout,
                      hipStream_t stream);
+struct XattnFoldArgs {
+    const half_t* K2 = nullptr;
+    const half_t* V2 = nullptr;
+    const half_t* WqT = nullptr;
+    const half_t* bq = nullptr;
+    const half_t* Wo = nullptr;
+    int n = 0, heads = 0, C = 0, Tp = 0, tokens = 0;
+    half_t* G = nullptr;
+    half_t* gbias = nullptr;
+    float* gwsum = nullptr;
+    half_t* Z = nullptr;
+};
+int xattn_fold_launch(const XattnFoldArgs& a, hipStream_t stream);
+int transpose_half_launch(const half_t* src, int rows, int cols, half_t* dst, hipStream_t stream);
 struct SmallConvInArgs {
     const float* x = nullptr;
     const float* scale_sigma = nullptr;
diff --git a/lightdiffusion_amd/csrc/misc.hip b/lightdiffusion_amd/csrc/misc.hip
--- a/lightdiffusion_amd/csrc/misc.hip
+++ b/lightdiffusion_amd/csrc/misc.hip
@@ -593,3 +593,129 @@
                        K9 / 8, SC / 8, reinterpret_cast<uint4*>(Wout), bout);
     return hipGetLastError() == hipSuccess ? LD_OK : LD_ERR_HIP;
 }
+
+namespace {
+struct XFoldArgs {
+    const half_t* A; int lda; long long sA; int M, m_valid;
+    const half_t* B; int ldb; long long sB; int N, n_valid;
+    half_t* O; int ldo; long long sO, hO;
+    int d; float alpha;
+};
+template <int TM, int TN, bool SPLIT_M>
+__global__ __launch_bounds__(256) void xattn_fold_kernel(const XFoldArgs a) {
+    const int lane = threadIdx.x & 63, wid = threadIdx.x >> 6;
+    const int fr = lane & 15, fq = lane >> 4;
+    const int h = blockIdx.y, s = blockIdx.z;
+    const int m_base = SPLIT_M ? (blockIdx.x * 4 + wid) * TM * 16 : 0;
+    const int n_base = SPLIT_M ? 0 : (blockIdx.x * 4 + wid) * TN * 16;
+    if (m_base >= a.M || n_base >= a.N) return;
+    const half_t* Ab = a.A + (long long)s * a.sA + (long long)h * a.d;
+    const half_t* Bb = a.B + (long long)s * a.sB + (long long)h * a.d;
+    f32x4 acc[TM][TN];
+#pragma unroll
+    for (int i = 0; i < TM; ++i)
+#pragma unroll
+        for (int j = 0; j < TN; ++j) acc[i][j] = (f32x4){0.f, 0.f, 0.f, 0.f};
+    for (int k0 = 0; k0 < a.d; k0 += 32) {
+        const int k = k0 + fq * 8;
+        half8 fa[TM], fb[TN];
+#pragma unroll
+        for (int i = 0; i < TM; ++i) {
+            const int m = m_base + i * 16 + fr;
+            fa[i] = as_half8((m < a.m_valid && k < a.d) ? ld16(Ab + (long long)m * a.lda + k) : zero16());
+        }
+#pragma unroll
+        for (int j = 0; j < TN; ++j) {
+            const int n = n_base + j * 16 + fr;
+            fb[j] = as_half8((n < a.n_valid && k < a.d) ? ld16(Bb + (long long)n * a.ldb + k) : zero16());
+        }
+#pragma unroll
+        for (int i = 0; i < TM; ++i)
+#pragma unroll
+            for (int j = 0; j < TN; ++j) acc[i][j] = __builtin_amdgcn_mfma_f32_16x16x32_f16(fb[j], fa[i], acc[i][j], 0, 0, 0);
+    }
+    half_t* Ob = a.O + (long long)s * a.sO + (long long)h * a.hO;
+#pragma unroll
+    for (int i = 0; i < TM; ++i) {
+        const int m = m_base + i * 16 + fr;
+#pragma unroll
+        for (int j = 0; j < TN; ++j) {
+            const int n = n_base + j * 16 + fq * 4;
+            if (m < a.M && n < a.N) {
+                const f32x4 v = acc[i][j] * a.alpha;
+                *reinterpret_cast<uint2*>(Ob + (long long)m * a.ldo + n) = make_uint2(pk2h(v[0], v[1]), pk2h(v[2], v[3]));
+            }
+        }
+    }
+}
+
+__global__ __launch_bounds__(256) void xattn_fold_rows_kernel(const half_t* __restrict__ G, const half_t* __restrict__ K2, const half_t* __restrict__ bq, int n, int heads, int C,
+                                                              int Tp, int tokens, float alpha, half_t* __restrict__ gbias, float* __restrict__ gwsum) {
+    const int lane = threadIdx.x & 63;
+    const long long row = (long long)blockIdx.x * 4 + (threadIdx.x >> 6);
+    if (row >= (long long)n * heads * 80) return;
+    const int t = (int)(row % 80), h = (int)((row / 80) % heads), s = (int)(row / (80 * heads));
+    const int d = C / heads;
+    float ws = 0.f, bs = 0.f;
+    const half_t* g = G + row * C;
+    for (int c = lane * 8; c < C; c += 512) {
+        float f[8];
+        unpack8(ld16(g + c), f);
+#pragma unroll
+        for (int j = 0; j < 8; ++j) ws += f[j];
+    }
+    if (t < tokens)
+        for (int k = lane; k < d; k += 64) bs += (float)K2[((long long)s * Tp + t) * C + h * d + k] * (float)bq[h * d + k];
+#pragma unroll
+    for (int o = 32; o > 0; o >>= 1) {
+        ws += __shfl_xor(ws, o);
+        bs += __shfl_xor(bs, o);
+    }
+    if (lane == 0) {
+        gwsum[row] = t < tokens ? ws : 0.f;
+        gbias[row] = (half_t)(t < tokens ? alpha * bs : -60000.f);
+    }
+}
+
+__global__ __launch_bounds__(256) void transpose_half_kernel(const half_t* __restrict__ src, int rows, int cols, half_t* __restrict__ dst) {
+    __shared__ half_t tile[32][33];
+    const int tx = threadIdx.x & 31, ty = threadIdx.x >> 5;
+    const int c0 = blockIdx.x * 32, r0 = blockIdx.y * 32;
+    for (int i = ty; i < 32; i += 8)
+        if (r0 + i < rows && c0 + tx < cols) tile[i][tx] = src[(long long)(r0 + i) * cols + c0 + tx];
+    __syncthreads();
+    for (int i = ty; i < 32; i += 8)
+        if (c0 + i < cols && r0 + tx < rows) dst[(long long)(c0 + i) * rows + r0 + tx] = tile[tx][i];
+}
+}
+
+int transpose_half_launch(const half_t* src, int rows, int cols, half_t* dst, hipStream_t stream) {
+    if (src == nullptr || dst == nullptr || rows <= 0 || cols <= 0) return LD_ERR_ARG;
+    hipLaunchKernelGGL(transpose_half_kernel, dim3((cols + 31) / 32, (rows + 31) / 32), dim3(256), 0, stream, src, rows, cols, dst);
+    return hipGetLastError() == hipSuccess ? LD_OK : LD_ERR_HIP;
+}
+
+int xattn_fold_launch(const XattnFoldArgs& a, hipStream_t stream) {
+    if (a.K2 == nullptr || a.V2 == nullptr || a.WqT == nullptr || a.bq == nullptr || a.Wo == nullptr || a.G == nullptr || a.gbias == nullptr || a.gwsum == nullptr ||
+        a.Z == nullptr)
+        return LD_ERR_ARG;
+    if (a.n < 1 || a.heads < 1 || a.C % a.heads || ((a.C / a.heads) & 7) || (a.C & 7) || a.tokens < 1 || a.tokens > a.Tp || a.Tp > 80) return LD_ERR_SHAPE;
+    const int C = a.C, d = C / a.heads, HN = a.heads * 80;
+    const float alpha = 1.4426950408889634f / sqrtf((float)d);
+    XFoldArgs g;
+    g.A = a.K2; g.lda = C; g.sA = (long long)a.Tp * C; g.M = 80; g.m_valid = a.tokens;
+    g.B = a.WqT; g.ldb = C; g.sB = 0; g.N = C; g.n_valid = C;
+    g.O = a.G; g.ldo = C; g.sO = (long long)HN * C; g.hO = (long long)80 * C;
+    g.d = d; g.alpha = alpha;
+    hipLaunchKernelGGL((xattn_fold_kernel<5, 4, false>), dim3((C + 255) / 256, a.heads, a.n), dim3(256), 0, stream, g);
+    XFoldArgs z;
+    z.A = a.Wo; z.lda = C; z.sA = 0; z.M = C; z.m_valid = C;
+    z.B = a.V2; z.ldb = C; z.sB = (long long)a.Tp * C; z.N = 80; z.n_valid = a.tokens;
+    z.O = a.Z; z.ldo = HN; z.sO = (long long)C * HN; z.hO = 80;
+    z.d = d; z.alpha = 1.0f;
+    hipLaunchKernelGGL((xattn_fold_kernel<4, 5, true>), dim3((C + 255) / 256, a.heads, a.n), dim3(256), 0, stream, z);
+    const long long rows = (long long)a.n * HN;
+    hipLaunchKernelGGL(xattn_fold_rows_kernel, dim3((unsigned)((rows + 3) / 4)), dim3(256), 0, stream, a.G, a.K2, a.bq, a.n, a.heads, C, a.Tp, a.tokens, alpha, a.gbias,
+                       a.gwsum);
+    return hipGetLastError() == hipSuccess ? LD_OK : LD_ERR_HIP;
+}
diff --git a/lightdiffusion_amd/csrc/unet.hip b/lightdiffusion_amd/csrc/unet.hip
--- a/lightdiffusion_amd/csrc/unet.hip
+++ b/lightdiffusion_amd/csrc/unet.hip
@@ -16,6 +16,7 @@
     size_t f_qk_w = 0, f_q2_w = 0, f_ff1_w = 0, f_qk_b = 0, f_q2_b = 0, f_ff1_b = 0, f_qk_s = 0, f_q2_s = 0,
            f_ff1_s = 0;
     size_t f_mo_w = 0, f_mo_b = 0;
+    size_t f_q2_wt = 0;
     int gn_g, gn_b, pin_w, pin_b, ln1_g, ln1_b, q1_w, k1_w, v1_w, o1_w, o1_b, ln2_g, ln2_b, q2_w, k2_w, v2_w, o2_w, o2_b, ln3_g,
         ln3_b, ff1_w, ff1_b, ff2_w, ff2_b, pout_w, pout_b;
 };
@@ -54,6 +55,10 @@
     int max_n = 0, max_h = 0, max_w = 0, max_tok = 0;
     half_t* ctx16 = nullptr;
     std::vector<half_t*> ctx_k, ctx_vt;
+    std::vector<half_t*> ctx_v, xf_g, xf_z, xf_gb;
+    std::vector<float*> xf_gs;
+    bool xf_reserved = false;
+    bool xf_live = false;
     int ctx_n = 0, ctx_tok = 0, ctx_tpad = 0;
     int plan_n = 0, plan_h = 0, plan_w = 0, plan_pair = 0;
     int last_launches = 0;
@@ -172,6 +177,7 @@
         s.f_ff1_s = take(8 * C * sizeof(float));
         s.f_mo_w = take(5 * C * C * sizeof(half_t));
         s.f_mo_b = take(C * sizeof(half_t));
+        s.f_q2_wt = take(C * C * sizeof(half_t));
     }
     u->st.push_back(s);
     return (int)u->st.size() - 1;
@@ -252,6 +258,10 @@
     for (size_t i = 0; i < u->res.size(); ++i)
         u->res[i].emb_b = t.add(u->res[i].prefix + ".emb_layers.1.bias", PK_VEC, {u->res[i].cout}, i == 0 ? 256 : 16);
     return t.finalize();
+}
+
+bool xattn_fold_gate(int C, int L) {
+    return C >= 640 || L <= 256;
 }
 
 struct Run {
@@ -442,46 +452,90 @@
         }
         const bool split_here = pair_pending;
         producer(ao, C, s.o1_w, s.o1_b, t, C);
-        if (!fold) ex.layernorm(t, P(s.ln2_g), P(s.ln2_b), nrm, M, C);
-        half_t* q2 = qkv;
-        {
-            GemmParams p;
-            p.A = fold ? t : nrm; p.lda = C;
-            p.W = fold ? reinterpret_cast<const half_t*>(fb + s.f_q2_w) : P(s.q2_w); p.ldw = C;
-            p.M = M; p.N = C; p.K = C;
-            p.C = q2; p.ldc = C;
-            if (fold) {
-                p.bias_n = reinterpret_cast<const half_t*>(fb + s.f_q2_b);
-                ln_args(p, s.f_q2_s);
-            }
-            ex.gemm(p);
-        }
-        if (split_here) {
-            const size_t hb = (size_t)M * C * sizeof(half_t);
-            DupArgs da;
-            da.count = 3;
-            da.base[0] = reinterpret_cast<char*>(t); da.base[1] = reinterpret_cast<char*>(q2); da.base[2] = reinterpret_cast<char*>(const_cast<half_t*>(x));
-            da.bytes[0] = da.bytes[1] = da.bytes[2] = hb;
-            ex.launches += 1;
-            ex.t_begin(KC_MISC, 0.0, 1, "dup3", (long long)hb, 0, 0, 1);
-            if (!ex.dry && ex.status == LD_OK) ex.note(dup_halves_launch(da, ex.stream));
-            ex.t_end("dup_halves_kernel");
-            pair_pending = false;
-            n = n_alloc;
-            M = n * L;
-        }
-        {
-            const int Tp = u->ctx_tpad;
-            AttnParams a;
-            a.Q = q2; a.ldq = C; a.sQ = (long long)L * C;
-            a.K = u->ctx_k[s.ctx_slot]; a.ldk = C; a.sK = (long long)Tp * C;
-            a.Vt = u->ctx_vt[s.ctx_slot]; a.ldvt = Tp; a.sV = (long long)C * Tp;
-            a.O = ao; a.ldo = C; a.sO = (long long)L * C;
-            a.B = n; a.H = heads; a.Lq = L; a.Lk = u->ctx_tok; a.d = d;
-            a.scale = 1.0f / sqrtf((float)d);
-            ex.attention(a);
-        }
-        producer(ao, C, s.o2_w, s.o2_b, t, C);
+        if (fold && u->xf_live && heads * 80 <= 3 * C && xattn_fold_gate(C, L)) {
+            const int HN = heads * 80, stat_rows = M, zmod = split_here ? n : 0;
+            if (split_here) {
+                const size_t hb = (size_t)M * C * sizeof(half_t);
+                DupArgs da;
+                da.count = 2;
+                da.base[0] = reinterpret_cast<char*>(t); da.base[1] = reinterpret_cast<char*>(const_cast<half_t*>(x));
+                da.bytes[0] = da.bytes[1] = hb;
+                ex.launches += 1;
+                ex.t_begin(KC_MISC, 0.0, 1, "dup2", (long long)hb, 0, 0, 1);
+                if (!ex.dry && ex.status == LD_OK) ex.note(dup_halves_launch(da, ex.stream));
+                ex.t_end("dup_halves_kernel");
+                pair_pending = false;
+                n = n_alloc;
+                M = n * L;
+            }
+            half_t* pr = qkv;
+            {
+                GemmParams p;
+                p.A = t; p.lda = C; p.sA = (long long)L * C;
+                p.W = u->xf_g[s.ctx_slot]; p.ldw = C; p.sW = (long long)HN * C;
+                p.M = L; p.N = HN; p.K = C; p.batch = n;
+                p.bias_n = u->xf_gb[s.ctx_slot]; p.sBias = HN;
+                p.act = 4;
+                p.C = pr; p.ldc = HN; p.sC = (long long)L * HN;
+                p.ln_stat = stat; p.ln_parts = parts; p.ln_rows = stat_rows; p.ln_zmod = zmod;
+                p.ln_inv_c = 1.0f / (float)C; p.ln_eps = 1e-5f;
+                p.ln_wsum = u->xf_gs[s.ctx_slot]; p.sWsum = HN;
+                ex.gemm(p);
+            }
+            {
+                GemmParams p;
+                p.A = pr; p.lda = HN; p.sA = (long long)L * HN;
+                p.W = u->xf_z[s.ctx_slot]; p.ldw = HN; p.sW = (long long)C * HN;
+                p.M = L; p.N = C; p.K = HN; p.batch = n;
+                p.bias_n = P(s.o2_b);
+                p.R = t; p.ldr = C; p.sR = (long long)L * C;
+                p.C = t; p.ldc = C; p.sC = (long long)L * C;
+                p.stat_out = stat;
+                p.stat_parts_out = &parts;
+                ex.gemm(p);
+            }
+        } else {
+            if (!fold) ex.layernorm(t, P(s.ln2_g), P(s.ln2_b), nrm, M, C);
+            half_t* q2 = qkv;
+            {
+                GemmParams p;
+                p.A = fold ? t : nrm; p.lda = C;
+                p.W = fold ? reinterpret_cast<const half_t*>(fb + s.f_q2_w) : P(s.q2_w); p.ldw = C;
+                p.M = M; p.N = C; p.K = C;
+                p.C = q2; p.ldc = C;
+                if (fold) {
+                    p.bias_n = reinterpret_cast<const half_t*>(fb + s.f_q2_b);
+                    ln_args(p, s.f_q2_s);
+                }
+                ex.gemm(p);
+            }
+            if (split_here) {
+                const size_t hb = (size_t)M * C * sizeof(half_t);
+                DupArgs da;
+                da.count = 3;
+                da.base[0] = reinterpret_cast<char*>(t); da.base[1] = reinterpret_cast<char*>(q2); da.base[2] = reinterpret_cast<char*>(const_cast<half_t*>(x));
+                da.bytes[0] = da.bytes[1] = da.bytes[2] = hb;
+                ex.launches += 1;
+                ex.t_begin(KC_MISC, 0.0, 1, "dup3", (long long)hb, 0, 0, 1);
+                if (!ex.dry && ex.status == LD_OK) ex.note(dup_halves_launch(da, ex.stream));
+                ex.t_end("dup_halves_kernel");
+                pair_pending = false;
+                n = n_alloc;
+                M = n * L;
+            }
+            {
+                const int Tp = u->ctx_tpad;
+                AttnParams a;
+                a.Q = q2; a.ldq = C; a.sQ = (long long)L * C;
+                a.K = u->ctx_k[s.ctx_slot]; a.ldk = C; a.sK = (long long)Tp * C;
+                a.Vt = u->ctx_vt[s.ctx_slot]; a.ldvt = Tp; a.sV = (long long)C * Tp;
+                a.O = ao; a.ldo = C; a.sO = (long long)L * C;
+                a.B = n; a.H = heads; a.Lq = L; a.Lk = u->ctx_tok; a.d = d;
+                a.scale = 1.0f / sqrtf((float)d);
+                ex.attention(a);
+            }
+            producer(ao, C, s.o2_w, s.o2_b, t, C);
+        }
         if (!fold) ex.layernorm(t, P(s.ln3_g), P(s.ln3_b), nrm, M, C);
         ff = ar.halfs(Ma * 4 * C);
         {
@@ -526,6 +580,7 @@
         int st = ln_fold_launch(P_q1, 3 * C, C, u->pt.ptr(s.ln1_g), u->pt.ptr(s.ln1_b), nullptr, H(s.f_qk_w), H(s.f_qk_b), F(s.f_qk_s), stream);
         if (st == LD_OK) st = ln_fold_launch(u->pt.ptr(s.q2_w), C, C, u->pt.ptr(s.ln2_g), u->pt.ptr(s.ln2_b), nullptr, H(s.f_q2_w), H(s.f_q2_b), F(s.f_q2_s), stream);
         if (st == LD_OK) st = ln_fold_launch(u->pt.ptr(s.ff1_w), 8 * C, C, u->pt.ptr(s.ln3_g), u->pt.ptr(s.ln3_b), u->pt.ptr(s.ff1_b), H(s.f_ff1_w), H(s.f_ff1_b), F(s.f_ff1_s), stream);
+        if (st == LD_OK) st = transpose_half_launch(H(s.f_q2_w), C, C, H(s.f_q2_wt), stream);
         if (st == LD_OK) st = mlp_out_fold_launch(u->pt.ptr(s.pout_w), u->pt.ptr(s.ff2_w), u->pt.ptr(s.ff2_b), u->pt.ptr(s.pout_b), C, H(s.f_mo_w), H(s.f_mo_b), stream);
         if (st != LD_OK) return st;
     }
@@ -547,18 +602,41 @@
     return LD_OK;
 }
 
+int derive_weights(ld_unet* u, hipStream_t stream) {
+    if (u->w8_base != nullptr) {
+        const int st = derive_conv8_weights(u, stream);
+        if (st != LD_OK) return st;
+    }
+    if (u->ln_fold) {
+        const int st = fold_layernorms(u, stream);
+        if (st != LD_OK) return st;
+    }
+    u->fold_dirty = false;
+    return LD_OK;
+}
+
+int xattn_fold_all(ld_unet* u, hipStream_t stream) {
+    for (size_t i = 0; i < u->st.size(); ++i) {
+        const StW& s = u->st[i];
+        XattnFoldArgs a;
+        a.K2 = u->ctx_k[i]; a.V2 = u->ctx_v[i];
+        a.WqT = reinterpret_cast<const half_t*>(u->fold_base + s.f_q2_wt);
+        a.bq = reinterpret_cast<const half_t*>(u->fold_base + s.f_q2_b);
+        a.Wo = u->pt.ptr(s.o2_w);
+        a.n = u->ctx_n; a.heads = u->cfg.num_heads; a.C = s.c; a.Tp = u->ctx_tpad; a.tokens = u->ctx_tok;
+        a.G = u->xf_g[i]; a.gbias = u->xf_gb[i]; a.gwsum = u->xf_gs[i]; a.Z = u->xf_z[i];
+        const int st = xattn_fold_launch(a, stream);
+        if (st != LD_OK) return st;
+    }
+    return LD_OK;
+}
+
 int run_forward(ld_unet* u, bool dry, const float* x, const float* sigma, float* out, int n, int h, int w, int eps_only, hipStream_t stream,
                 size_t* dry_peak = nullptr, bool pair = false) {
     if (!dry && u->fold_dirty) {
-        if (u->w8_base != nullptr) {
-            const int st = derive_conv8_weights(u, stream);
-            if (st != LD_OK) return st;
-        }
-        if (u->ln_fold) {
-            const int st = fold_layernorms(u, stream);
-            if (st != LD_OK) return st;
-        }
-        u->fold_dirty = false;
+        int st = derive_weights(u, stream);
+        if (st == LD_OK && u->xf_live) st = xattn_fold_all(u, stream);
+        if (st != LD_OK) return st;
     }
     if (pair && (n & 1)) return LD_ERR_SHAPE;
     Run R;
@@ -786,6 +864,15 @@
     u->ctx_tpad = (max_tok + 7) & ~7;
     u->ctx_k.assign(u->st.size(), nullptr);
     u->ctx_vt.assign(u->st.size(), nullptr);
+    u->ctx_v.assign(u->st.size(), nullptr);
+    u->xf_g.assign(u->st.size(), nullptr);
+    u->xf_z.assign(u->st.size(), nullptr);
+    u->xf_gb.assign(u->st.size(), nullptr);
+    u->xf_gs.assign(u->st.size(), nullptr);
+    u->xf_live = false;
+    u->xf_reserved = u->ln_fold && max_tok <= 80 && !(u->cfg.num_heads & 1);
+    for (const StW& s : u->st)
+        if (s.c % u->cfg.num_heads || ((s.c / u->cfg.num_heads) & 7)) u->xf_reserved = false;
     size_t peak = 0;
     int st = run_forward(u, true, nullptr, nullptr, nullptr, max_n, max_h, max_w, 0, nullptr, &peak);
     if (st != LD_OK) return st;
@@ -799,6 +886,12 @@
     const size_t tpad = (size_t)u->ctx_tpad;
     size_t ctxb = ((size_t)max_n * tpad * u->cfg.context_dim * sizeof(half_t) + 255) / 256 * 256;
     for (const StW& s : u->st) ctxb += 2 * (((size_t)max_n * tpad * s.c * sizeof(half_t) + 255) / 256 * 256);
+    const size_t HN = (size_t)u->cfg.num_heads * 80;
+    auto r256 = [](size_t b) { return (b + 255) / 256 * 256; };
+    if (u->xf_reserved)
+        for (const StW& s : u->st)
+            ctxb += r256((size_t)max_n * tpad * s.c * sizeof(half_t)) + 2 * r256((size_t)max_n * HN * s.c * sizeof(half_t)) + r256((size_t)max_n * HN * sizeof(half_t)) +
+                    r256((size_t)max_n * HN * sizeof(float));
     u->splitk_bytes = (size_t)96 << 20;
     u->ws_bytes = act + ctxb + u->splitk_bytes + 4096;
     if (hipMalloc((void**)&u->ws_base, u->ws_bytes) != hipSuccess) {
@@ -820,6 +913,18 @@
         p += b;
         u->ctx_vt[i] = reinterpret_cast<half_t*>(p);
         p += b;
+        if (u->xf_reserved) {
+            u->ctx_v[i] = reinterpret_cast<half_t*>(p);
+            p += b;
+            u->xf_g[i] = reinterpret_cast<half_t*>(p);
+            p += r256((size_t)max_n * HN * u->st[i].c * sizeof(half_t));
+            u->xf_z[i] = reinterpret_cast<half_t*>(p);
+            p += r256((size_t)max_n * HN * u->st[i].c * sizeof(half_t));
+            u->xf_gb[i] = reinterpret_cast<half_t*>(p);
+            p += r256((size_t)max_n * HN * sizeof(half_t));
+            u->xf_gs[i] = reinterpret_cast<float*>(p);
+            p += r256((size_t)max_n * HN * sizeof(float));
+        }
     }
     if (getenv("LD_PROFILE_DUMP") != nullptr)
         fprintf(stderr, "[ld_reserve] workspace %p (%zu MiB)  weights %p  folds %p  conv8 weights %p\n", (void*)u->ws_base, u->ws_bytes >> 20, (void*)u->pt.base,
@@ -840,6 +945,7 @@
     const int D = u->cfg.context_dim, Tp = (tokens + 7) & ~7;
     int st = ctx_pad_launch(ctx, dtype == LD_F32, n, tokens, Tp, D, u->ctx16, stream);
     if (st != LD_OK) return st;
+    const bool xf = u->xf_reserved && tokens <= 80;
     for (size_t i = 0; i < u->st.size(); ++i) {
         const StW& s = u->st[i];
         GemmParams k;
@@ -856,10 +962,24 @@
         v.C = u->ctx_vt[i]; v.ldc = Tp; v.sC = (long long)s.c * Tp;
         st = gemm_launch(v, stream);
         if (st != LD_OK) return st;
+        if (xf) {
+            GemmParams r = k;
+            r.W = u->pt.ptr(s.v2_w);
+            r.C = u->ctx_v[i];
+            st = gemm_launch(r, stream);
+            if (st != LD_OK) return st;
+        }
     }
     u->ctx_n = n;
     u->ctx_tok = tokens;
     u->ctx_tpad = Tp;
+    u->xf_live = false;
+    if (xf) {
+        if (u->fold_dirty) st = derive_weights(u, stream);
+        if (st == LD_OK) st = xattn_fold_all(u, stream);
+        if (st != LD_OK) return st;
+        u->xf_live = true;
+    }
     return LD_OK;
 }
 
diff --git a/lightdiffusion_amd/ops.py b/lightdiffusion_amd/ops.py
--- a/lightdiffusion_amd/ops.py
+++ b/lightdiffusion_amd/ops.py
@@ -42,7 +42,7 @@
 
 def linear(x: torch.Tensor, weight: torch.Tensor, bias: Optional[torch.Tensor] = None, residual: Optional[torch.Tensor] = None,
            act: str = "none", alpha: float = 1.0) -> torch.Tensor:
-    code = {"none": 0, "silu": 1, "geglu": 2, "quick_gelu": 3}[act]
+    code = {"none": 0, "silu": 1, "geglu": 2, "quick_gelu": 3, "softmax80": 4}[act]
     K = x.shape[-1]
     N = weight.shape[0]
     M = x.numel() // K
```

Measured after the change: 59.85 steps/s. Within noise of the previous version (-0.5%).
